# vLAR-group/OGC

Measured on AMD Instinct MI355X. Metric: point-clouds/sec (8192 pts) segnet fwd+bwd, higher is better.
Workload: dtype f32; 1 GPU; C4 KITTI-SF train_seg unsup: segnet_kitti fwd + OGC loss (dynamic+smooth+invariance) + bwd + Adam, 4 samples x 4 views x 8192 pts per GPU; n_point=8192, n_slot=10, parallelism=dp1, optimizer_stepped=True

## Files before the change

include/ogc_ops.h:

```cpp
#ifndef OGC_OPS_H
#define OGC_OPS_H

#ifdef __cplusplus
extern "C" {
#endif

typedef void *ogc_stream_t;
typedef unsigned short ogc_bf16_t;

enum {
    OGC_OK = 0,
    OGC_ERR_INVALID_ARG = -1,
    OGC_ERR_LAUNCH = -2,
    OGC_ERR_UNSUPPORTED = -3
};

#define OGC_VERSION 208
int ogc_version(void);
int ogc_distance_contracted(void);
int ogc_set_deterministic(int on);
int ogc_get_deterministic(void);
const char *ogc_last_error(void);

int ogc_furthest_point_sampling(int b, int n, int m, const float *xyz, float *temp,
// ... 63 lines not shown
                 ogc_stream_t stream);

int ogc_seg_eval_ignore(int B, int n, int k, const int *segm, const float *mask, const int *ignore, int ignore_npoint_thresh,
                        int *hard, int *counts, int *ignored, double *pred_iou, double *confidence, int *valid, int *n_gt,
                        float *score, int *rows, double *ri, int *status, ogc_stream_t stream);

int ogc_flow_eval(int B, int N, const float *gt_flow, const float *flow_pred, double epe_norm_thresh, double eps,
                  double *epe_sum, int *counts, ogc_stream_t stream);

#define OGC_SUP_LOSS_MAX_K 32
#define OGC_SUP_LOSS_TILE 64
long long ogc_sup_loss_ws_doubles(int B, int n, int k);
int ogc_sup_match_cost(int B, int n, int k, const float *mask, const float *gt_mask, const float *valid, int use_focal,
                       double alpha, double gamma, double *ws, float *cost_ce, float *cost_dice, ogc_stream_t stream);
int ogc_sup_mask_loss_fwd(int B, int n, int k, const float *mask, const float *gt_mask, const float *valid, const int *col4row,
                          int use_focal, double alpha, double gamma, double *ws, double *sums, float *terms,
                          ogc_stream_t stream);
int ogc_sup_mask_loss_bwd(int B, int n, int k, const float *mask, const float *gt_mask, const float *valid, const int *col4row,
                          int use_focal, double alpha, double gamma, const double *sums, double w_ce, double w_dice,
                          const float *grad_out, float *grad_mask, ogc_stream_t stream);

int ogc_group_concat(int b, int c, int n, int npoints, int nsample, const float *xyz, const float *new_xyz,
                     const float *points, const int *idx, float *out, ogc_stream_t stream);

int ogc_group_concat_grad(int b, int c, int n, int npoints, int nsample, const float *grad_out, const int *idx,
                          float *grad_points, ogc_stream_t stream);

int ogc_group_linear_fwd(int b, int m, int n, int npoints, int nsample, int groups, const float *P, const int *idx,
                         const float *rel, const float *wx, float *y, double *stats, ogc_stream_t stream);
int ogc_group_linear_fwd_direct(int b, int m, int cf, int n, int npoints, int nsample, int groups, const float *feats,
                                const int *idx, const float *rel, const float *w, float *y, double *stats, ogc_stream_t stream);
int ogc_group_linear_fwd_direct_h(int b, int m, int cf, int n, int npoints, int nsample, int groups, const float *feats,
                                  const int *idx, const float *rel, const float *w, ogc_bf16_t *y, double *stats, ogc_stream_t stream);
int ogc_group_linear_bwd(int b, int m, int n, int npoints, int nsample, const float *grad_y, const int *idx,
                         const float *rel, float *grad_p, float *dwx, ogc_stream_t stream);

int ogc_group_reverse_chunk(int n, int npoints, int nsample);
int ogc_group_reverse(int b, int n, int npoints, int nsample, const int *idx, int *rev_start, unsigned short *rev_pos,
                      unsigned short *heads, ogc_stream_t stream);
int ogc_group_points_grad_rev(int b, int c, int n, int npoints, int nsample, const float *grad_out, const int *rev_start,
                              const unsigned short *rev_pos, const unsigned short *heads, float *grad_points,
                              ogc_stream_t stream);

int ogc_group_points_grad_rev_dwx(int b, int c, int n, int npoints, int nsample, const float *grad_out, const int *rev_start,
                                  const unsigned short *rev_pos, const unsigned short *heads, const float *rel,
                                  float *grad_points, float *dwx, ogc_stream_t stream);
int ogc_three_interpolate_grad_rev(int b, int c, int n, int m, const float *grad_out, const float *weight,
                                   const int *rev_start, const unsigned short *rev_pos, const unsigned short *heads,
                                   float *grad_points, ogc_stream_t stream);
int ogc_three_interpolate_grad_rev_bs(int b, int c, int n, int m, const float *grad_out, long long grad_out_bstride,
                                      const float *weight, const int *rev_start, const unsigned short *rev_pos,
                                      const unsigned short *heads, float *grad_points, ogc_stream_t stream);

int ogc_view_means(int parts, const float *const *src, const int *rows, const long long *len, float *out, ogc_stream_t stream);
int ogc_view_means_grad(int parts, float *const *grad, const int *rows, const long long *len, const float *weight,
                        const float *g_loss, ogc_stream_t stream);
int ogc_sum_ranges(int parts, const float *const *src, const long long *first, const long long *count, long long total,
                   float *out, ogc_stream_t stream);

int ogc_rigid_moments(int vb, int n, int k, const float *pc, const float *pc2, const float *mask, double *mom, float *S,
                      float *means, ogc_stream_t stream);
int ogc_rigid_translation(int total, const float *means, const int *valid, float *R, float *t, ogc_stream_t stream);
int ogc_rigid_blend(int vb, int n, int k, int p, int backward, const float *pc, const float *pc2, const float *mask,
                    const float *R, const float *t, const float *grad_out, float *out, ogc_stream_t stream);

int ogc_mask_iou(int pb, int n, int k, const float *mask1, const float *mask2, int *counts, float *iou,
                 ogc_stream_t stream);
int ogc_matched_distance(int pb, int n, int k, int p, int backward, const float *mask1, const float *mask2,
                         const int *col12, const int *col21, const float *grad12, const float *grad21, float *out1,
                         float *out2, ogc_stream_t stream);

int ogc_lsap_maximize(int np, int k, const float *score, int *col4row, ogc_stream_t stream);

int ogc_sym_eigvals(int nb, int k, const double *A, double *w, ogc_stream_t stream);

int ogc_neighbour_consistency_fwd(int b, int n, int c, int k, int p, const float *mask, const int *idx, float *out,
                                  ogc_stream_t stream);

int ogc_reverse_neighbours(int b, int n, int k, const int *idx, int *rev_start, int *rev_src, int *rev_mult, int *ws,
                           ogc_stream_t stream);

int ogc_neighbour_consistency_bwd(int b, int n, int c, int k, int p, const float *mask, const int *idx,
                                  const int *rev_start, const int *rev_src, const int *rev_mult, const float *grad_out,
                                  float *grad_mask, ogc_stream_t stream);

int ogc_soft_nn_target(int b, int n1, int n2, int k, float temperature, const float *p1, const float *p2,
                       const float *mask1, const float *mask2, float *target, ogc_stream_t stream);

int ogc_soft_carry(int b, int n1, int n2, int c, float temperature, const float *p1, const float *p2, const float *x,
                   float *out, ogc_stream_t stream);

#define OGC_SCAN_CROP_TILE 1024
#define OGC_SCAN_CROP_CAMERA_DOUBLES 36
int ogc_scan_crop_camera(int n, int stride, const float *scan, const double *cam, float clip_distance, float depth_thresh,
                         float *out_pc, int *keep_idx, int *count, ogc_stream_t stream);
int ogc_scan_crop_front(int n, int stride, const float *scan, float *out_pc, int *keep_idx, int *count, ogc_stream_t stream);
int ogc_scan_crop_tile(void);

#define OGC_BOX_SEGM_CHUNK 128
#define OGC_BOX_SEGM_BOX_DOUBLES 18
int ogc_box_segm(int n, int k, const float *pc, int sign_x, int sign_y, int sign_z, const double *boxes, const int *ids,
                 int *segm, int *semantic_segm, ogc_stream_t stream);
int ogc_box_segm_chunk(void);

int ogc_kittisf_unproject(int height, int width, const unsigned short *disp1, const unsigned short *disp2,
                          const unsigned short *flow, const unsigned short *inst, float fb, float f, float p02, float p03,
                          float p12, float p13, float p23, float depth_thresh, const int *select_semantics, int n_select,
                          float *pc1, float *pc2, int *segm, int *keep_idx, int *count, ogc_stream_t stream);

int ogc_png_unfilter(const unsigned char *in, unsigned char *out, int height, int row_bytes, int bpp);

int ogc_attention_fwd(int b, int lq, int lk, int h, int d, float scale, const float *q, int ldq, const float *k,
                      int ldk, const float *v, int ldv, float *out, float *prob, ogc_stream_t stream);
int ogc_attention_bwd(int b, int lq, int lk, int h, int d, float scale, const float *q, int ldq, const float *k,
                      int ldk, const float *v, int ldv, const float *out, const float *prob, const float *dout,
                      float *dq, int lddq, float *dk, int lddk, float *dv, int lddv, ogc_stream_t stream);

int ogc_small_linear_fwd(int rows, int n_in, int n_out, const float *x, const float *weight, const float *bias,
                         float *y, ogc_stream_t stream);
int ogc_small_linear_bwd(int rows, int n_in, int n_out, const float *x, const float *weight, const float *grad_y,
                         float *grad_x, float *grad_weight, float *grad_bias, ogc_stream_t stream);

int ogc_conv1x1_wgrad_moments(int b, int cin, int cout, int hw, int relu, const float *y_prev, const float *pa,
                              const float *pb, const float *grad_y, float *moments, ogc_stream_t stream);
int ogc_gn_moments_combine(int b, int cin, int cout, int hw, int groups, const float *moments, const float *w,
                           const float *pa, const float *pb, const float *mean, const float *rstd, const float *gamma,
                           float *grad_w, float *coef, float *grad_gamma, float *grad_beta, ogc_stream_t stream);
int ogc_conv1x1_dgrad_adjoint(int b, int cin, int cout, int hw, int relu, const float *w, const float *grad_y,
                              const float *y_prev, const float *pa, const float *pb, const float *coef, float *grad_prev,
                              ogc_stream_t stream);

int ogc_first_conv_stats(int b, int c1, int c0, int hw, int groups, const float *x0, const float *w1, double *stats,
                         ogc_stream_t stream);
int ogc_conv1x1_gemm_affine_first(int b, int M, int K, int hw, int relu, int groups, int c0, const float *w, const float *x0,
                                  const float *w1, const float *pa, const float *pb, float *out, double *stats,
                                  ogc_stream_t stream);
int ogc_conv1x1_wgrad_moments_first(int b, int cin, int cout, int hw, int relu, int c0, const float *x0, const float *w1,
                                    const float *pa, const float *pb, const float *grad_y, float *moments,
                                    ogc_stream_t stream);
int ogc_conv1x1_dgrad_adjoint_first(int b, int cin, int cout, int hw, int relu, int c0, const float *w, const float *grad_y,
                                    const float *x0, const float *w1, const float *pa, const float *pb, const float *coef,
                                    float *grad_w1, ogc_stream_t stream);

int ogc_group_norm_maxpool_bwd_sparse(int b, int c, int p, int s, int groups, int relu, const float *x,
                                      const float *x_at_argmax, const float *gamma, const float *mean, const float *rstd, const float *out, const int *argmax,
                                      const float *grad_out, float *coef2, float *inj, float *grad_gamma,
                                      float *grad_beta, double *ws, ogc_stream_t stream);
int ogc_conv1x1_wgrad_moments_pooled(int b, int cin, int cout, int hw, int relu, int nsample, const float *y_prev,
                                     const float *pa, const float *pb, const float *y, const float *coef2,
                                     const float *inj, float *moments, ogc_stream_t stream);
int ogc_conv1x1_dgrad_adjoint_pooled(int b, int cin, int cout, int hw, int relu, int nsample, const float *w, const float *y,
                                     const float *coef2, const float *inj, const float *y_prev, const float *pa,
                                     const float *pb, const float *coef, float *grad_prev, ogc_stream_t stream);

int ogc_mlp_chain_pool_supported(int c0, int c1, int c2, int c3, int nsample);
int ogc_mlp_chain_pool(int b, int c0, int c1, int c2, int c3, int p, int nsample, const float *x, const float *wt1,
                       const float *b1, const float *wt2, const float *b2, const float *wt3, const float *b3, float *out,
                       ogc_stream_t stream);

int ogc_corr_layer_pool_supported(int cf, int c1, int c2, int c3, int nsample);
int ogc_corr_layer_pool(int b, int cf, int c1, int c2, int c3, int n1, int n2, int nsample, const float *pos1,
                        const float *pos2, const float *feat1, const float *feat2, const int *idx, const float *wt1,
                        const float *b1, const float *wt2, const float *b2, const float *wt3, const float *b3, float *out,
                        ogc_stream_t stream);

long long ogc_slot_masks_ws_floats(int b, int d, int n, int k);
int ogc_slot_masks_fwd(int b, int d, int n, int k, float temperature, const float *feats, const float *slots,
                       float *mask, ogc_stream_t stream);
int ogc_slot_masks_bwd(int b, int d, int n, int k, float temperature, const float *feats, const float *slots,
                       const float *mask, const float *grad_mask, float *grad_feats, float *grad_slots, float *ws,
                       ogc_stream_t stream);

int ogc_group_norm_stats_slots(void);
int ogc_group_norm_bwd_slots(void);
int ogc_group_norm_fwd(int b, int c, int hw, int groups, float eps, int relu, const float *x,
                       const float *gamma, const float *beta, float *y, float *mean, float *rstd,
                       double *ws, ogc_stream_t stream);
int ogc_group_norm_bwd(int b, int c, int hw, int groups, int relu, const float *x, const float *gamma,
                       const float *beta, const float *mean, const float *rstd, const float *grad_y,
                       float *grad_x, float *grad_gamma, float *grad_beta, double *ws, ogc_stream_t stream);

int ogc_group_norm_maxpool_fwd(int b, int c, int p, int s, int groups, float eps, int relu, const float *x,
                               const float *gamma, const float *beta, float *out, int *argmax, float *mean,
                               float *rstd, double *ws, ogc_stream_t stream);
int ogc_group_norm_maxpool_bwd(int b, int c, int p, int s, int groups, int relu, const float *x,
                               const float *gamma, const float *mean, const float *rstd, const float *out,
                               const int *argmax, const float *grad_out, float *grad_x, float *grad_gamma,
                               float *grad_beta, double *ws, ogc_stream_t stream);
int ogc_group_norm_maxpool_bwd_ext(int b, int c, int p, int s, int groups, int relu, const float *x,
                                   const float *x_at_argmax, const float *gamma, const float *mean, const float *rstd,
                                   const float *out, const int *argmax, const float *grad_out, float *grad_x,
                                   float *grad_gamma, float *grad_beta, double *ws, ogc_stream_t stream);

int ogc_batch_norm_fwd(int b, int c, int hw, float eps, int relu, int training, float momentum, const float *x,
                       const float *gamma, const float *beta, float *running_mean, float *running_var, float *y,
                       float *mean, float *rstd, double *ws, const double *stats, int slots, ogc_stream_t stream);
int ogc_batch_norm_bwd(int b, int c, int hw, int relu, int training, const float *x, const float *gamma,
                       const float *beta, const float *mean, const float *rstd, const float *grad_y, float *grad_x,
                       float *grad_gamma, float *grad_beta, double *ws, ogc_stream_t stream);
int ogc_batch_norm_maxpool_fwd(int b, int c, int p, int s, float eps, int relu, int training, float momentum,
                               const float *x, const float *gamma, const float *beta, float *running_mean,
                               float *running_var, float *out, int *argmax, float *mean, float *rstd, double *ws,
                               const double *stats, int slots, ogc_stream_t stream);
int ogc_batch_norm_maxpool_bwd(int b, int c, int p, int s, int relu, int training, const float *x, const float *gamma,
                               const float *mean, const float *rstd, const float *out, const int *argmax,
                               const float *grad_out, float *grad_x, float *grad_gamma, float *grad_beta, double *ws,
                               ogc_stream_t stream);

int ogc_conv1x1_wgrad(int b, int cin, int cout, int hw, const float *x, const float *dy, float *dw,
                      ogc_stream_t stream);

int ogc_conv1x1_gemm(int b, int M, int K, int hw, int transpose_a, const float *w, const float *in,
                     float *out, ogc_stream_t stream);

int ogc_conv1x1_gn_slots(void);
int ogc_conv1x1_gemm_stats_supported(int b, int M, int K, int hw, int affine);
int ogc_conv1x1_gemm_stream_supported(int b, int M, int K, int hw);
int ogc_conv1x1_gemm_any(int b, int M, int K, int hw, int transpose_a, const float *w, const float *in, float *out,
                         ogc_stream_t stream);

int ogc_set_matmul_precision(int bf16);
int ogc_conv1x1_gemm_gnstats(int b, int M, int K, int hw, int groups, const float *w, const float *in, float *out,
                             double *stats, ogc_stream_t stream);

int ogc_group_norm_coeffs(int b, int c, int hw, int groups, float eps, const float *x, const float *gamma,
                          const float *beta, const double *stats, int slots, double *ws, float *mean, float *rstd,
                          float *a, float *bb, ogc_stream_t stream);
int ogc_conv1x1_gemm_affine(int b, int M, int K, int hw, int relu, int groups, const float *w, const float *in,
                            const float *pa, const float *pb, float *out, double *stats, ogc_stream_t stream);
int ogc_conv1x1_wgrad_affine(int b, int cin, int cout, int hw, int relu, const float *x, const float *pa,
                             const float *pb, const float *dy, float *dw, ogc_stream_t stream);
int ogc_conv1x1_wgrad_affine_pooled(int b, int cin, int cout, int hw, int relu, int nsample, const float *x, const float *pa,
                                    const float *pb, const float *y, const float *coef2, const float *inj, float *dw,
                                    ogc_stream_t stream);
int ogc_conv1x1_dgrad_pooled(int b, int cin, int cout, int hw, int nsample, const float *w, const float *y, const float *coef2,
                             const float *inj, float *grad_z, ogc_stream_t stream);

int ogc_group_norm_fwd_stats(int b, int c, int hw, int groups, float eps, int relu, const float *x,
                             const float *gamma, const float *beta, float *y, float *mean, float *rstd,
                             const double *stats, int slots, ogc_stream_t stream);
int ogc_group_norm_maxpool_fwd_stats(int b, int c, int p, int s, int groups, float eps, int relu, const float *x,
                                     const float *gamma, const float *beta, float *out, int *argmax, float *mean,
                                     float *rstd, const double *stats, int slots, ogc_stream_t stream);

int ogc_conv1x1_gemm_affine_pool(int b, int M, int K, int hw, int relu, int groups, int nsample, const float *w,
                                 const float *in, const float *pa, const float *pb, const float *next_gamma,
                                 float *out, double *stats, float *yext, int *aext, ogc_stream_t stream);
int ogc_group_norm_pool_extremes(int b, int c, int p, int s, int groups, float eps, int relu, const float *yext,
                                 const int *aext, const float *gamma, const float *beta, float *out, int *argmax,
                                 float *mean, float *rstd, const double *stats, int slots, ogc_stream_t stream);

int ogc_chamfer_terms(int b, int n1, int n2, int p, const float *p1, const float *pc2, const int *idx12, const int *idx21,
                      float *dist1, float *dist2, ogc_stream_t stream);
int ogc_chamfer_terms_grad(int b, int n1, int n2, int p, const float *p1, const float *pc2, const int *idx12, const int *idx21,
                           const float *g1, const float *g2, float *grad_p1, ogc_stream_t stream);

int ogc_gather_xyz_pair(int b, int n, int m, const float *xyz, const int *idx, float *out, float *out_t, ogc_stream_t stream);
int ogc_flow_advance(int b, int n, float scale, const float *cur, const float *delta, const float *ref, float *out_delta,
                     float *out_new, float *out_new_t, float *out_flow, ogc_stream_t stream);
int ogc_linear_cn(int b, int cin, int cout, int n, const float *x, const float *weight, const float *bias, float *y,
                  ogc_stream_t stream);
int ogc_three_nn_weights(int b, int n, int mode, const float *dist2, float *weight, ogc_stream_t stream);
int ogc_soft_corr_flow(int b, int n1, int n2, int c, float support, const float *epsilon, const float *pc1, const float *pc2,
                       const float *f1, const float *f2, float *flow, ogc_stream_t stream);
int ogc_gru_reset(int b, int c, int cx, int n, int s, const float *rc, long long rc_batch_stride, const float *hx, float *out,
                  ogc_stream_t stream);
int ogc_gru_blend(int b, int c, int n, int s, const float *zc, long long zc_batch_stride, const float *qc,
                  long long qc_batch_stride, const float *h, long long h_batch_stride, float *out, ogc_stream_t stream);

int ogc_zero_arena_begin(void *base, int bytes, ogc_stream_t stream);
int ogc_zero_arena_end(void);

int ogc_group_linear_fwd_h(int b, int m, int n, int npoints, int nsample, int groups, const float *P, const int *idx,
                           const float *rel, const float *wx, ogc_bf16_t *y, double *stats, ogc_stream_t stream);
int ogc_group_linear_fwd_pt_h(int b, int m, int n, int npoints, int nsample, int groups, const float *Pt, const int *idx,
                              const float *rel, const float *wx, ogc_bf16_t *y, double *stats, ogc_stream_t stream);
int ogc_group_points_grad_rev_h(int b, int c, int n, int npoints, int nsample, const ogc_bf16_t *grad_out, const int *rev_start,
                                const unsigned short *rev_pos, const unsigned short *heads, float *grad_points,
                                ogc_stream_t stream);
int ogc_group_points_grad_rev_dwx_h(int b, int c, int n, int npoints, int nsample, const ogc_bf16_t *grad_out, const int *rev_start,
                                    const unsigned short *rev_pos, const unsigned short *heads, const float *rel,
                                    float *grad_points, float *dwx, ogc_stream_t stream);
int ogc_conv1x1_gemm_h(int b, int M, int K, int hw, int transpose_a, const float *w, const ogc_bf16_t *in, ogc_bf16_t *out,
                       ogc_stream_t stream);
int ogc_conv1x1_gemm_affine_h(int b, int M, int K, int hw, int relu, int groups, const float *w, const ogc_bf16_t *in,
                              const float *pa, const float *pb, ogc_bf16_t *out, double *stats, ogc_stream_t stream);
int ogc_conv1x1_gemm_affine_pool_h(int b, int M, int K, int hw, int relu, int groups, int nsample, const float *w,
                                   const ogc_bf16_t *in, const float *pa, const float *pb, const float *next_gamma,
                                   ogc_bf16_t *out, double *stats, float *yext, int *aext, ogc_stream_t stream);
int ogc_conv1x1_wgrad_xf_h(int b, int cin, int cout, int hw, const float *x, const ogc_bf16_t *dy, float *dw,
                           ogc_stream_t stream);
int ogc_conv1x1_wgrad_affine_h(int b, int cin, int cout, int hw, int relu, const ogc_bf16_t *x, const float *pa,
                               const float *pb, const ogc_bf16_t *dy, float *dw, ogc_stream_t stream);
int ogc_conv1x1_wgrad_affine_pooled_h(int b, int cin, int cout, int hw, int relu, int nsample, const ogc_bf16_t *x,
                                      const float *pa, const float *pb, const ogc_bf16_t *y, const float *coef2,
                                      const float *inj, float *dw, ogc_stream_t stream);
int ogc_conv1x1_dgrad_pooled_h(int b, int cin, int cout, int hw, int nsample, const float *w, const ogc_bf16_t *y,
                               const float *coef2, const float *inj, ogc_bf16_t *grad_z, ogc_stream_t stream);
int ogc_conv1x1_wgrad_moments_h(int b, int cin, int cout, int hw, int relu, const ogc_bf16_t *y_prev, const float *pa,
                                const float *pb, const ogc_bf16_t *grad_y, float *moments, ogc_stream_t stream);
int ogc_conv1x1_wgrad_moments_pooled_h(int b, int cin, int cout, int hw, int relu, int nsample, const ogc_bf16_t *y_prev,
                                       const float *pa, const float *pb, const ogc_bf16_t *y, const float *coef2,
                                       const float *inj, float *moments, ogc_stream_t stream);
int ogc_conv1x1_dgrad_adjoint_h(int b, int cin, int cout, int hw, int relu, const float *w, const ogc_bf16_t *grad_y,
                                const ogc_bf16_t *y_prev, const float *pa, const float *pb, const float *coef,
                                ogc_bf16_t *grad_prev, ogc_stream_t stream);
// ... 17 lines not shown
```

ogc_amd/_lib.py:

```python
import ctypes
import os

_HERE = os.path.dirname(os.path.abspath(__file__))
FMAD = os.environ.get("OGC_FMAD", "0") == "1"
DETERMINISTIC = os.environ.get("OGC_DETERMINISTIC", "0") == "1"
LIB_PATH = os.path.join(_HERE, "csrc", "libogc_ops_fmad.so" if FMAD else "libogc_ops.so")

_vp = ctypes.c_void_p
_int = ctypes.c_int
_flt = ctypes.c_float
_dbl = ctypes.c_double
_ll = ctypes.c_longlong

SIGNATURES = {
    "ogc_set_deterministic": [_int],
    "ogc_group_linear_fwd_direct": [_int, _int, _int, _int, _int, _int, _int, _vp, _vp, _vp, _vp, _vp, _vp, _vp],
    "ogc_get_deterministic": [],
    "ogc_furthest_point_sampling": [_int, _int, _int, _vp, _vp, _vp, _vp],
    "ogc_furthest_point_sampling_chain": [_int, _int, _int, _vp, _vp, _vp, _vp, _vp, _vp],
    "ogc_gather_points": [_int, _int, _int, _int, _vp, _vp, _vp, _vp],
    "ogc_gather_points_grad": [_int, _int, _int, _int, _vp, _vp, _vp, _vp],
    "ogc_knn": [_int, _int, _int, _int, _vp, _vp, _vp, _vp, _vp],
    "ogc_three_nn": [_int, _int, _int, _vp, _vp, _vp, _vp, _vp],
    "ogc_three_interpolate": [_int, _int, _int, _int, _vp, _vp, _vp, _vp, _vp],
    "ogc_three_interpolate_grad": [_int, _int, _int, _int, _vp, _vp, _vp, _vp, _vp],
    "ogc_group_points": [_int, _int, _int, _int, _int, _vp, _vp, _vp, _vp],
    "ogc_group_points_grad": [_int, _int, _int, _int, _int, _vp, _vp, _vp, _vp],
    "ogc_group_reverse_chunk": [_int, _int, _int],
    "ogc_group_reverse": [_int, _int, _int, _int, _vp, _vp, _vp, _vp, _vp],
    "ogc_three_interpolate_grad_rev": [_int, _int, _int, _int, _vp, _vp, _vp, _vp, _vp, _vp, _vp],
    "ogc_view_means": [_int, _vp, _vp, _vp, _vp, _vp],
    "ogc_view_means_grad": [_int, _vp, _vp, _vp, _vp, _vp, _vp],
    "ogc_sum_ranges": [_int, _vp, _vp, _vp, _ll, _vp, _vp],
    "ogc_three_interpolate_grad_rev_bs": [_int, _int, _int, _int, _vp, _ll, _vp, _vp, _vp, _vp, _vp, _vp],
    "ogc_group_points_grad_rev": [_int, _int, _int, _int, _int, _vp, _vp, _vp, _vp, _vp, _vp],
    "ogc_group_points_grad_rev_dwx": [_int, _int, _int, _int, _int, _vp, _vp, _vp, _vp, _vp, _vp, _vp, _vp],
    "ogc_ball_query": [_int, _int, _int, _flt, _int, _vp, _vp, _vp, _vp],
    "ogc_knn_clamped": [_int, _int, _int, _int, _flt, _vp, _vp, _vp, _vp, _vp],
    "ogc_cell_grid_bytes": [_int, _int],
    "ogc_cell_grid_build": [_int, _int, _flt, _vp, _vp, _vp],
    "ogc_ball_query_cells": [_int, _int, _flt, _int, _vp, _vp, _flt, _vp, _vp],
    "ogc_knn_clamped_cells": [_int, _int, _int, _flt, _vp, _vp, _flt, _vp, _vp, _vp],
    "ogc_chamfer_terms": [_int, _int, _int, _int, _vp, _vp, _vp, _vp, _vp, _vp, _vp],
    "ogc_chamfer_terms_grad": [_int, _int, _int, _int, _vp, _vp, _vp, _vp, _vp, _vp, _vp, _vp],
    "ogc_gather_xyz_pair": [_int, _int, _int, _vp, _vp, _vp, _vp, _vp],
    "ogc_flow_advance": [_int, _int, _flt, _vp, _vp, _vp, _vp, _vp, _vp, _vp, _vp],
    "ogc_linear_cn": [_int, _int, _int, _int, _vp, _vp, _vp, _vp, _vp],
    "ogc_three_nn_weights": [_int, _int, _int, _vp, _vp, _vp],
    "ogc_soft_corr_flow": [_int, _int, _int, _int, _flt, _vp, _vp, _vp, _vp, _vp, _vp, _vp],
    "ogc_gru_reset": [_int, _int, _int, _int, _int, _vp, _ll, _vp, _vp, _vp],
    "ogc_gru_blend": [_int, _int, _int, _int, _vp, _ll, _vp, _ll, _vp, _ll, _vp, _vp],
    "ogc_zero_arena_begin": [_vp, _int, _vp],
    "ogc_zero_arena_end": [],
    "ogc_adam_max_tensors": [],
    "ogc_adam_chunk": [],
    "ogc_adam_step": [_int, _int, _vp, _vp, _vp, _vp, _vp, _dbl, _dbl, _dbl, _dbl, _dbl, _vp],
    "ogc_kabsch_rotation": [_int, _vp, _vp, _vp, _vp],
    "ogc_rigid_icp": [_int, _int, _vp, _vp, _vp, _int, _dbl, _vp, _vp, _vp, _vp],
    "ogc_ground_plane_fit": [_int, _int, _vp, _int, _int, _dbl, _dbl, _int, _vp, _vp, _vp, _vp],
    "ogc_seg_eval": [_int, _int, _int, _vp, _vp, _int, _vp, _vp, _vp, _vp, _vp, _vp, _vp, _vp, _vp, _vp, _vp],
    "ogc_seg_eval_ignore": [_int, _int, _int, _vp, _vp, _vp, _int, _vp, _vp, _vp, _vp, _vp, _vp, _vp, _vp, _vp, _vp, _vp, _vp],
    "ogc_flow_eval": [_int, _int, _vp, _vp, _dbl, _dbl, _vp, _vp, _vp],
    "ogc_lsap_maximize": [_int, _int, _vp, _vp, _vp],
    "ogc_sup_loss_ws_doubles": [_int, _int, _int],
    "ogc_sup_match_cost": [_int, _int, _int, _vp, _vp, _vp, _int, _dbl, _dbl, _vp, _vp, _vp, _vp],
    "ogc_sup_mask_loss_fwd": [_int, _int, _int, _vp, _vp, _vp, _vp, _int, _dbl, _dbl, _vp, _vp, _vp, _vp],
    "ogc_sup_mask_loss_bwd": [_int, _int, _int, _vp, _vp, _vp, _vp, _int, _dbl, _dbl, _vp, _dbl, _dbl, _vp, _vp, _vp],
    "ogc_rigid_moments": [_int, _int, _int, _vp, _vp, _vp, _vp, _vp, _vp, _vp],
    "ogc_rigid_translation": [_int, _vp, _vp, _vp, _vp, _vp],
    "ogc_rigid_blend": [_int, _int, _int, _int, _int, _vp, _vp, _vp, _vp, _vp, _vp, _vp, _vp],
    "ogc_mask_iou": [_int, _int, _int, _vp, _vp, _vp, _vp, _vp],
    "ogc_matched_distance": [_int, _int, _int, _int, _int, _vp, _vp, _vp, _vp, _vp, _vp, _vp, _vp, _vp],
    "ogc_soft_nn_target": [_int, _int, _int, _int, _flt, _vp, _vp, _vp, _vp, _vp, _vp],
    "ogc_soft_carry": [_int, _int, _int, _int, _flt, _vp, _vp, _vp, _vp, _vp],
    "ogc_scan_crop_camera": [_int, _int, _vp, _vp, _flt, _flt, _vp, _vp, _vp, _vp],
    "ogc_scan_crop_front": [_int, _int, _vp, _vp, _vp, _vp, _vp],
    "ogc_scan_crop_tile": [],
    "ogc_box_segm": [_int, _int, _vp, _int, _int, _int, _vp, _vp, _vp, _vp, _vp],
    "ogc_box_segm_chunk": [],
    "ogc_kittisf_unproject": [_int, _int, _vp, _vp, _vp, _vp, _flt, _flt, _flt, _flt, _flt, _flt, _flt, _flt, _vp, _int,
                              _vp, _vp, _vp, _vp, _vp, _vp],
    "ogc_png_unfilter": [_vp, _vp, _int, _int, _int],
    "ogc_group_concat": [_int, _int, _int, _int, _int, _vp, _vp, _vp, _vp, _vp, _vp],
    "ogc_group_linear_fwd": [_int, _int, _int, _int, _int, _int, _vp, _vp, _vp, _vp, _vp, _vp, _vp],
    "ogc_group_linear_bwd": [_int, _int, _int, _int, _int, _vp, _vp, _vp, _vp, _vp, _vp],
    "ogc_group_concat_grad": [_int, _int, _int, _int, _int, _vp, _vp, _vp, _vp],
    "ogc_neighbour_consistency_fwd": [_int, _int, _int, _int, _int, _vp, _vp, _vp, _vp],
    "ogc_reverse_neighbours": [_int, _int, _int, _vp, _vp, _vp, _vp, _vp, _vp],
    "ogc_neighbour_consistency_bwd": [_int, _int, _int, _int, _int, _vp, _vp, _vp, _vp, _vp, _vp, _vp, _vp],
    "ogc_sym_eigvals": [_int, _int, _vp, _vp, _vp],
    "ogc_group_norm_fwd": [_int, _int, _int, _int, _flt, _int, _vp, _vp, _vp, _vp, _vp, _vp, _vp, _vp],
    "ogc_group_norm_bwd": [_int, _int, _int, _int, _int, _vp, _vp, _vp, _vp, _vp, _vp, _vp, _vp, _vp, _vp, _vp],
    "ogc_group_norm_maxpool_fwd": [_int, _int, _int, _int, _int, _flt, _int, _vp, _vp, _vp, _vp, _vp, _vp, _vp, _vp, _vp],
    "ogc_conv1x1_gemm": [_int, _int, _int, _int, _int, _vp, _vp, _vp, _vp],
    "ogc_attention_fwd": [_int, _int, _int, _int, _int, _flt, _vp, _int, _vp, _int, _vp, _int, _vp, _vp, _vp],
    "ogc_attention_bwd": [_int, _int, _int, _int, _int, _flt, _vp, _int, _vp, _int, _vp, _int, _vp, _vp, _vp, _vp, _int,
                          _vp, _int, _vp, _int, _vp],
    "ogc_conv1x1_gemm_affine_pool": [_int, _int, _int, _int, _int, _int, _int, _vp, _vp, _vp, _vp, _vp, _vp, _vp, _vp, _vp,
                                     _vp],
    "ogc_group_norm_pool_extremes": [_int, _int, _int, _int, _int, _flt, _int, _vp, _vp, _vp, _vp, _vp, _vp, _vp, _vp, _vp,
                                     _int, _vp],
    "ogc_small_linear_fwd": [_int, _int, _int, _vp, _vp, _vp, _vp, _vp],
    "ogc_small_linear_bwd": [_int, _int, _int, _vp, _vp, _vp, _vp, _vp, _vp, _vp],
    "ogc_conv1x1_wgrad_moments": [_int, _int, _int, _int, _int, _vp, _vp, _vp, _vp, _vp, _vp],
    "ogc_gn_moments_combine": [_int, _int, _int, _int, _int, _vp, _vp, _vp, _vp, _vp, _vp, _vp, _vp, _vp, _vp, _vp, _vp],
    "ogc_conv1x1_dgrad_adjoint": [_int, _int, _int, _int, _int, _vp, _vp, _vp, _vp, _vp, _vp, _vp, _vp],
    "ogc_first_conv_stats": [_int, _int, _int, _int, _int, _vp, _vp, _vp, _vp],
    "ogc_conv1x1_gemm_affine_first": [_int, _int, _int, _int, _int, _int, _int, _vp, _vp, _vp, _vp, _vp, _vp, _vp, _vp],
    "ogc_conv1x1_wgrad_moments_first": [_int, _int, _int, _int, _int, _int, _vp, _vp, _vp, _vp, _vp, _vp, _vp],
    "ogc_conv1x1_dgrad_adjoint_first": [_int, _int, _int, _int, _int, _int, _vp, _vp, _vp, _vp, _vp, _vp, _vp, _vp, _vp],
    "ogc_group_norm_maxpool_bwd_sparse": [_int, _int, _int, _int, _int, _int, _vp, _vp, _vp, _vp, _vp, _vp, _vp, _vp, _vp, _vp,
                                          _vp, _vp, _vp, _vp],
    "ogc_group_norm_maxpool_bwd_ext": [_int, _int, _int, _int, _int, _int, _vp, _vp, _vp, _vp, _vp, _vp, _vp, _vp, _vp, _vp,
                                       _vp, _vp, _vp],
    "ogc_conv1x1_wgrad_moments_pooled": [_int, _int, _int, _int, _int, _int, _vp, _vp, _vp, _vp, _vp, _vp, _vp, _vp],
    "ogc_conv1x1_dgrad_adjoint_pooled": [_int, _int, _int, _int, _int, _int, _vp, _vp, _vp, _vp, _vp, _vp, _vp, _vp, _vp, _vp],
    "ogc_mlp_chain_pool_supported": [_int, _int, _int, _int, _int],
    "ogc_mlp_chain_pool": [_int, _int, _int, _int, _int, _int, _int, _vp, _vp, _vp, _vp, _vp, _vp, _vp, _vp, _vp],
    "ogc_corr_layer_pool_supported": [_int, _int, _int, _int, _int],
    "ogc_corr_layer_pool": [_int, _int, _int, _int, _int, _int, _int, _int, _vp, _vp, _vp, _vp, _vp, _vp, _vp, _vp, _vp, _vp,
                            _vp, _vp, _vp],
    "ogc_slot_masks_ws_floats": [_int, _int, _int, _int],
    "ogc_slot_masks_fwd": [_int, _int, _int, _int, _flt, _vp, _vp, _vp, _vp],
    "ogc_slot_masks_bwd": [_int, _int, _int, _int, _flt, _vp, _vp, _vp, _vp, _vp, _vp, _vp, _vp],
    "ogc_conv1x1_gn_slots": [],
    "ogc_conv1x1_gemm_stats_supported": [_int, _int, _int, _int, _int],
    "ogc_conv1x1_gemm_stream_supported": [_int, _int, _int, _int],
    "ogc_conv1x1_gemm_any": [_int, _int, _int, _int, _int, _vp, _vp, _vp, _vp],
    "ogc_set_matmul_precision": [_int],
    "ogc_group_norm_stats_slots": [],
    "ogc_group_norm_bwd_slots": [],
    "ogc_group_norm_coeffs": [_int, _int, _int, _int, _flt, _vp, _vp, _vp, _vp, _int, _vp, _vp, _vp, _vp, _vp, _vp],
    "ogc_conv1x1_gemm_affine": [_int, _int, _int, _int, _int, _int, _vp, _vp, _vp, _vp, _vp, _vp, _vp],
    "ogc_conv1x1_wgrad_affine": [_int, _int, _int, _int, _int, _vp, _vp, _vp, _vp, _vp, _vp],
    "ogc_conv1x1_wgrad_affine_pooled": [_int, _int, _int, _int, _int, _int, _vp, _vp, _vp, _vp, _vp, _vp, _vp, _vp],
    "ogc_conv1x1_dgrad_pooled": [_int, _int, _int, _int, _int, _vp, _vp, _vp, _vp, _vp, _vp],
    "ogc_batch_norm_fwd": [_int, _int, _int, _flt, _int, _int, _flt, _vp, _vp, _vp, _vp, _vp, _vp, _vp, _vp, _vp, _vp,
                           _int, _vp],
    "ogc_batch_norm_bwd": [_int, _int, _int, _int, _int, _vp, _vp, _vp, _vp, _vp, _vp, _vp, _vp, _vp, _vp, _vp],
    "ogc_batch_norm_maxpool_fwd": [_int, _int, _int, _int, _flt, _int, _int, _flt, _vp, _vp, _vp, _vp, _vp, _vp, _vp,
                                   _vp, _vp, _vp, _vp, _int, _vp],
    "ogc_batch_norm_maxpool_bwd": [_int, _int, _int, _int, _int, _int, _vp, _vp, _vp, _vp, _vp, _vp, _vp, _vp, _vp,
                                   _vp, _vp, _vp],
    "ogc_conv1x1_gemm_gnstats": [_int, _int, _int, _int, _int, _vp, _vp, _vp, _vp, _vp],
    "ogc_group_norm_fwd_stats": [_int, _int, _int, _int, _flt, _int, _vp, _vp, _vp, _vp, _vp, _vp, _vp, _int, _vp],
    "ogc_group_norm_maxpool_fwd_stats": [_int, _int, _int, _int, _int, _flt, _int, _vp, _vp, _vp, _vp, _vp, _vp, _vp,
                                         _vp, _int, _vp],
    "ogc_conv1x1_wgrad": [_int, _int, _int, _int, _vp, _vp, _vp, _vp],
    "ogc_group_norm_maxpool_bwd": [_int, _int, _int, _int, _int, _int, _vp, _vp, _vp, _vp, _vp, _vp, _vp, _vp, _vp, _vp,
                                   _vp, _vp],
}

for _n in ("ogc_group_linear_fwd", "ogc_group_points_grad_rev", "ogc_conv1x1_gemm", "ogc_conv1x1_gemm_affine",
           "ogc_conv1x1_gemm_affine_pool", "ogc_conv1x1_wgrad_affine", "ogc_conv1x1_wgrad_affine_pooled",
           "ogc_conv1x1_dgrad_pooled", "ogc_conv1x1_wgrad_moments", "ogc_conv1x1_wgrad_moments_pooled",
           "ogc_conv1x1_dgrad_adjoint", "ogc_conv1x1_dgrad_adjoint_pooled", "ogc_group_norm_bwd",
           "ogc_group_norm_maxpool_bwd_sparse", "ogc_group_points_grad_rev_dwx"):
    SIGNATURES[_n + "_h"] = SIGNATURES[_n]
SIGNATURES["ogc_group_linear_fwd_direct_h"] = SIGNATURES["ogc_group_linear_fwd_direct"]
SIGNATURES["ogc_conv1x1_wgrad_xf_h"] = SIGNATURES["ogc_conv1x1_wgrad"]
SIGNATURES["ogc_group_linear_fwd_pt_h"] = SIGNATURES["ogc_group_linear_fwd"]

HEADER_VERSION = 208
_lib = None
_fns = {}


class OgcOpsError(RuntimeError):
    pass


def load():
    global _lib
    if _lib is None:
        if not os.path.exists(LIB_PATH):
            raise OgcOpsError(
                "libogc_ops.so not found at %s — build it with `python ogc_amd/csrc/build.py` "
                "(there is no CPU fallback)" % LIB_PATH)
        L = ctypes.CDLL(LIB_PATH)
        for name, argtypes in SIGNATURES.items():
            fn = getattr(L, name)
            fn.argtypes = argtypes
            fn.restype = _int
        L.ogc_version.restype = _int
        if L.ogc_version() != HEADER_VERSION:
            raise OgcOpsError("libogc_ops.so at %s is version %d, this package binds version %d of include/ogc_ops.h — rebuild it "
                              "with `python ogc_amd/csrc/build.py --force`" % (LIB_PATH, L.ogc_version(), HEADER_VERSION))
        L.ogc_distance_contracted.restype = _int
        if bool(L.ogc_distance_contracted()) != FMAD:
            raise OgcOpsError("%s evaluates distances %s, OGC_FMAD asked for the other form" %
                              (LIB_PATH, "contracted (fma)" if L.ogc_distance_contracted() else "un-contracted"))
        L.ogc_slot_masks_ws_floats.restype = ctypes.c_longlong
        L.ogc_cell_grid_bytes.restype = ctypes.c_longlong
        L.ogc_sup_loss_ws_doubles.restype = ctypes.c_longlong
        L.ogc_last_error.restype = ctypes.c_char_p
        L.ogc_set_deterministic(1 if DETERMINISTIC else 0)
        _lib = L
    return _lib


def set_deterministic(on):
    global DETERMINISTIC
    DETERMINISTIC = bool(on)
    load().ogc_set_deterministic(1 if on else 0)


CALL_COUNTS = None

ROCTX_NAMES = {
    "ogc_furthest_point_sampling": "K1 furthest_point_sampling", "ogc_furthest_point_sampling_chain": "K1 furthest_point_sampling (chain)",
    "ogc_gather_points": "K2 gather_points", "ogc_gather_points_grad": "K3 gather_points_grad",
    "ogc_knn": "K4 knn", "ogc_knn_clamped": "K4 knn (+ sqrt + radius clamp)", "ogc_knn_clamped_cells": "K4 knn (shared cell grid)",
    "ogc_three_nn": "K5 three_nn", "ogc_three_interpolate": "K6 three_interpolate",
    "ogc_three_interpolate_grad": "K7 three_interpolate_grad", "ogc_three_interpolate_grad_rev": "K7 three_interpolate_grad (gather form)",
    "ogc_three_interpolate_grad_rev_bs": "K7 three_interpolate_grad (gather form)",
    "ogc_group_points": "K8 group_points", "ogc_group_points_grad": "K9 group_points_grad",
    "ogc_group_points_grad_rev": "K9 group_points_grad (gather form)",
    "ogc_ball_query": "K10 ball_query", "ogc_ball_query_cells": "K10 ball_query (shared cell grid)",
}
_roctx = None


def _roctx_lib():
    global _roctx
    if _roctx is None:
        _roctx = False
        if os.environ.get("OGC_ROCTX", "0") == "1":
            for name in ("librocprofiler-sdk-roctx.so", "libroctx64.so"):
                try:
                    lib = ctypes.CDLL(os.path.join(os.environ.get("ROCM_PATH", "/opt/rocm"), "lib", name))
                    lib.roctxRangePushA.argtypes = [ctypes.c_char_p]
                    lib.roctxRangePushA.restype = ctypes.c_int
                    lib.roctxRangePop.restype = ctypes.c_int
                    _roctx = lib
                    break
                except (OSError, AttributeError):
                    continue
    return _roctx


def call(name, *args):
    if CALL_COUNTS is not None:
        CALL_COUNTS[name] += 1
    fn = _fns.get(name)
    if fn is None:
        fn = _fns[name] = getattr(load(), name)
    tx = _roctx_lib()
    if tx:
        tx.roctxRangePushA(ROCTX_NAMES.get(name, name).encode())
        try:
            rc = fn(*args)
        finally:
            tx.roctxRangePop()
    else:
        rc = fn(*args)
    if rc != 0:
        msg = load().ogc_last_error().decode("utf-8", "replace")
        raise OgcOpsError("%s failed (status %d): %s" % (name, rc, msg))
    return rc
```

ogc_amd/csrc/gn_fused_bwd.hip:

```cpp
#include "conv1x1_shared.h"
#include "act_io.h"
#include "first_conv.h"

namespace {

template <int COB, int CIB, bool POOLED, typename AT = float, int FIRST = 0>
__global__ __launch_bounds__(WG_WAVES *OGC_WAVE) void wgrad_moments_kernel(int cin, int cout, int hw, int chunks,
                                                                           int steps_per_wave, int relu,
                                                                           const AT *__restrict__ x,
                                                                           const AT *__restrict__ dy,
                                                                           const float *__restrict__ aff_a,
                                                                           const float *__restrict__ aff_b,
                                                                           const float2 *__restrict__ coef2,
                                                                           const float2 *__restrict__ inj,
                                                                           int s_shift,
                                                                           float *__restrict__ hm,
                                                                           FirstIn first = FirstIn()) {
    constexpr int XN = FIRST ? FIRST : CIB;
    __shared__ float red[WG_WAVES][COB * CIB * 256];
    const int lane = threadIdx.x & 63, wave = __builtin_amdgcn_readfirstlane(threadIdx.x >> 6);
    const int i = lane & 15, k = lane >> 4;
    const int img = blockIdx.x / chunks, chunk = blockIdx.x - img * chunks;
    const int co0 = blockIdx.y * (16 * COB), ci0 = blockIdx.z * (16 * CIB);
    const int steps_per_img = hw >> 4;
    const int first_step = (chunk * WG_WAVES + wave) * steps_per_wave;
    const int mine = max(0, min(steps_per_wave, steps_per_img - first_step));

    v4f acc1[COB][CIB], acc2[COB][CIB];
#pragma unroll
    for (int a = 0; a < COB; ++a)
#pragma unroll
        for (int c = 0; c < CIB; ++c) {
            acc1[a][c] = (v4f){0.f, 0.f, 0.f, 0.f};
            acc2[a][c] = (v4f){0.f, 0.f, 0.f, 0.f};
        }
    int yrow[COB], xrow[XN], jrow[COB];
    float ca[CIB], cb[CIB], pc2[COB], pc3[COB];
    float w1r[FIRST ? CIB : 1][FIRST ? FIRST : 1];
    const int centres = hw >> s_shift, smask = (1 << s_shift) - 1;
#pragma unroll
    for (int a = 0; a < COB; ++a) {
        const int row = min(co0 + a * 16 + i, cout - 1);
        yrow[a] = row * hw;
        if (POOLED) {
            const float2 cc = coef2[(size_t)img * cout + row];
            pc2[a] = cc.x;
            pc3[a] = cc.y;
            jrow[a] = row * centres;
        }
    }
    const float2 *jb_ = POOLED ? inj + (size_t)img * cout * centres : nullptr;
#pragma unroll
    for (int c = 0; c < CIB; ++c) {
        const int ch = min(ci0 + c * 16 + i, cin - 1);
        if constexpr (FIRST == 0) xrow[c] = ch * hw;
        ca[c] = aff_a[(size_t)img * cin + ch];
        cb[c] = aff_b[(size_t)img * cin + ch];
        if constexpr (FIRST > 0) {
#pragma unroll
            for (int e = 0; e < FIRST; ++e) w1r[c][e] = e < first.c0 ? first.w1[ch * first.c0 + min(e, first.c0 - 1)] : 0.f;
        }
    }
    if constexpr (FIRST > 0) {
#pragma unroll
        for (int e = 0; e < FIRST; ++e) xrow[e] = min(e, first.c0 - 1) * hw;
    }
    const AT *yb_ = dy + (size_t)img * cout * hw + 4 * k;
    const AT *xb_ = FIRST ? reinterpret_cast<const AT *>(first.x0) + (size_t)img * first.c0 * hw + 4 * k
                          : x + (size_t)img * cin * hw + 4 * k;
    int cur = min(first_step, steps_per_img - 1);
    const int stop = min(first_step + mine, steps_per_img) - 1;
    auto load = [&](float4(&yv)[COB], float4(&xv)[XN], float2(&jv)[COB], int &jpos) {
        const int pb = cur * 16;
#pragma unroll
        for (int a = 0; a < COB; ++a) yv[a] = ogc_ld4(yb_ + yrow[a] + pb);
#pragma unroll
        for (int c = 0; c < XN; ++c) xv[c] = ogc_ld4(xb_ + xrow[c] + pb);
        if (POOLED) {
#pragma unroll
            for (int a = 0; a < COB; ++a) jv[a] = jb_[jrow[a] + (pb >> s_shift)];
            jpos = (pb & smask) + 4 * k;
        }
        cur = min(cur + 1, max(stop, 0));
    };
    auto fma16 = [&](float4(&yv)[COB], const float4(&xraw)[XN], const float2(&jv)[COB], int jpos) {
        if (POOLED) {
#pragma unroll
            for (int a = 0; a < COB; ++a) ogc_pooled_grad(yv[a], pc2[a], pc3[a], jv[a], jpos);
        }
        float4 x0v[FIRST ? FIRST : 1];
        if constexpr (FIRST > 0) {
#pragma unroll
            for (int e = 0; e < FIRST; ++e) x0v[e] = xraw[e];
            ogc_first_mask<FIRST>(x0v, first.c0, true);
        }
        float4 m1[CIB], m2[CIB];
#pragma unroll
        for (int c = 0; c < CIB; ++c) {
            float4 v;
            if constexpr (FIRST > 0) v = ogc_first_row<FIRST>(x0v, w1r[c]);
            else v = xraw[c];
            const bool bx = relu ? fmaf(ca[c], v.x, cb[c]) > 0.f : true;
            const bool by = relu ? fmaf(ca[c], v.y, cb[c]) > 0.f : true;
            const bool bz = relu ? fmaf(ca[c], v.z, cb[c]) > 0.f : true;
            const bool bw = relu ? fmaf(ca[c], v.w, cb[c]) > 0.f : true;
            m1[c] = make_float4(bx ? 1.f : 0.f, by ? 1.f : 0.f, bz ? 1.f : 0.f, bw ? 1.f : 0.f);
            m2[c] = make_float4(bx ? v.x : 0.f, by ? v.y : 0.f, bz ? v.z : 0.f, bw ? v.w : 0.f);
        }
#pragma unroll
        for (int a = 0; a < COB; ++a)
#pragma unroll
            for (int c = 0; c < CIB; ++c) {
                acc1[a][c] = __builtin_amdgcn_mfma_f32_16x16x4f32(yv[a].x, m1[c].x, acc1[a][c], 0, 0, 0);
                acc2[a][c] = __builtin_amdgcn_mfma_f32_16x16x4f32(yv[a].x, m2[c].x, acc2[a][c], 0, 0, 0);
                acc1[a][c] = __builtin_amdgcn_mfma_f32_16x16x4f32(yv[a].y, m1[c].y, acc1[a][c], 0, 0, 0);
                acc2[a][c] = __builtin_amdgcn_mfma_f32_16x16x4f32(yv[a].y, m2[c].y, acc2[a][c], 0, 0, 0);
                acc1[a][c] = __builtin_amdgcn_mfma_f32_16x16x4f32(yv[a].z, m1[c].z, acc1[a][c], 0, 0, 0);
                acc2[a][c] = __builtin_amdgcn_mfma_f32_16x16x4f32(yv[a].z, m2[c].z, acc2[a][c], 0, 0, 0);
                acc1[a][c] = __builtin_amdgcn_mfma_f32_16x16x4f32(yv[a].w, m1[c].w, acc1[a][c], 0, 0, 0);
                acc2[a][c] = __builtin_amdgcn_mfma_f32_16x16x4f32(yv[a].w, m2[c].w, acc2[a][c], 0, 0, 0);
            }
    };

    float4 ya[COB], xa[XN], yb[COB], xb[XN];
    float2 ja[COB], jb[COB];
    int pa_ = 0, pb_ = 0;
    load(ya, xa, ja, pa_);
    int s = 0;
    for (; s + 1 < mine; s += 2) {
        load(yb, xb, jb, pb_);
        fma16(ya, xa, ja, pa_);
        load(ya, xa, ja, pa_);
        fma16(yb, xb, jb, pb_);
    }
    if (s < mine) fma16(ya, xa, ja, pa_);

    float *dst = hm + (size_t)img * 2 * cout * cin;
#pragma unroll
    for (int which = 0; which < 2; ++which) {
        if (which) __syncthreads();
#pragma unroll
        for (int a = 0; a < COB; ++a)
#pragma unroll
            for (int c = 0; c < CIB; ++c)
#pragma unroll
                for (int r = 0; r < 4; ++r)
                    red[wave][(a * CIB + c) * 256 + (k * 4 + r) * 16 + i] = which ? acc2[a][c][r] : acc1[a][c][r];
        __syncthreads();
        for (int t = threadIdx.x; t < COB * CIB * 256; t += WG_WAVES * OGC_WAVE) {
            const int blk = t >> 8, a = blk / CIB, c = blk % CIB;
            const int row = co0 + a * 16 + ((t & 255) >> 4), col = ci0 + c * 16 + (t & 15);
            const float v = (red[0][t] + red[1][t]) + (red[2][t] + red[3][t]);
            if (row < cout && col < cin && v != 0.0f) unsafeAtomicAdd(dst + ((size_t)which * cout + row) * cin + col, v);
        }
    }
}

typedef short v4s16 __attribute__((ext_vector_type(4)));

template <int COB, int CIB, bool POOLED>
__global__ __launch_bounds__(WG_WAVES *OGC_WAVE) void wgrad_moments16_kernel(int cin, int cout, int hw, int chunks,
                                                                             int steps_per_wave, int relu,
                                                                             const ogc_bf16 *__restrict__ x,
                                                                             const ogc_bf16 *__restrict__ dy,
                                                                             const float *__restrict__ aff_a,
                                                                             const float *__restrict__ aff_b,
                                                                             const float2 *__restrict__ coef2,
                                                                             const float2 *__restrict__ inj,
                                                                             int s_shift,
                                                                             float *__restrict__ hm) {
    __shared__ float red[WG_WAVES][COB * CIB * 256];
    const int lane = threadIdx.x & 63, wave = __builtin_amdgcn_readfirstlane(threadIdx.x >> 6);
    const int i = lane & 15, k = lane >> 4;
    const int img = blockIdx.x / chunks, chunk = blockIdx.x - img * chunks;
    const int co0 = blockIdx.y * (16 * COB), ci0 = blockIdx.z * (16 * CIB);
    const int steps_per_img = hw >> 5;
    const int first = (chunk * WG_WAVES + wave) * steps_per_wave;
    const int mine = max(0, min(steps_per_wave, steps_per_img - first));

    v4f acc1[COB][CIB], acc2[COB][CIB];
#pragma unroll
    for (int a = 0; a < COB; ++a)
#pragma unroll
        for (int c = 0; c < CIB; ++c) {
            acc1[a][c] = (v4f){0.f, 0.f, 0.f, 0.f};
            acc2[a][c] = (v4f){0.f, 0.f, 0.f, 0.f};
        }
    int yrow[COB], xrow[CIB], jrow[COB];
    float ca[CIB], cb[CIB], pc2[COB], pc3[COB];
    const int centres = hw >> s_shift, smask = (1 << s_shift) - 1;
#pragma unroll
    for (int a = 0; a < COB; ++a) {
        const int row = min(co0 + a * 16 + i, cout - 1);
        yrow[a] = row * hw;
        if (POOLED) {
            const float2 cc = coef2[(size_t)img * cout + row];
            pc2[a] = cc.x;
            pc3[a] = cc.y;
            jrow[a] = row * centres;
        }
    }
    const float2 *jb_ = POOLED ? inj + (size_t)img * cout * centres : nullptr;
#pragma unroll
    for (int c = 0; c < CIB; ++c) {
        const int ch = min(ci0 + c * 16 + i, cin - 1);
        xrow[c] = ch * hw;
        ca[c] = aff_a[(size_t)img * cin + ch];
        cb[c] = aff_b[(size_t)img * cin + ch];
    }
    const ogc_bf16 *yb_ = dy + (size_t)img * cout * hw + 8 * k;
    const ogc_bf16 *xb_ = x + (size_t)img * cin * hw + 8 * k;
    int cur = min(first, steps_per_img - 1);
    const int stop = min(first + mine, steps_per_img) - 1;
    auto load = [&](uint4(&yv)[COB], uint4(&xv)[CIB], float2(&jv)[COB], int &jpos) {
        const int pb = cur * 32;
#pragma unroll
        for (int a = 0; a < COB; ++a) yv[a] = *reinterpret_cast<const uint4 *>(yb_ + yrow[a] + pb);
#pragma unroll
        for (int c = 0; c < CIB; ++c) xv[c] = *reinterpret_cast<const uint4 *>(xb_ + xrow[c] + pb);
        if (POOLED) {
#pragma unroll
            for (int a = 0; a < COB; ++a) jv[a] = jb_[jrow[a] + ((pb + 8 * k) >> s_shift)];
            jpos = (pb + 8 * k) & smask;
        }
        cur = min(cur + 1, max(stop, 0));
    };
    auto fma32 = [&](const uint4(&yraw)[COB], const uint4(&xraw)[CIB], const float2(&jv)[COB], int jpos) {
        v4s16 y0[COB], y1[COB];
#pragma unroll
        for (int a = 0; a < COB; ++a) {
            if (POOLED) {
                float f[8];
                ogc_unpack8(yraw[a], f);
                ogc_pooled_grad(f, pc2[a], pc3[a], jv[a], jpos);
                y0[a] = ogc_pack_bf16_rr(f[0], f[1], f[2], f[3]);
                y1[a] = ogc_pack_bf16_rr(f[4], f[5], f[6], f[7]);
            } else {
                y0[a] = __builtin_bit_cast(v4s16, make_uint2(yraw[a].x, yraw[a].y));
                y1[a] = __builtin_bit_cast(v4s16, make_uint2(yraw[a].z, yraw[a].w));
            }
        }
        v4s16 m1a[CIB], m1b[CIB], m2a[CIB], m2b[CIB];
#pragma unroll
        for (int c = 0; c < CIB; ++c) {
            float f[8];
            ogc_unpack8(xraw[c], f);
            unsigned keep[4];
#pragma unroll
            for (int e = 0; e < 4; ++e) {
                const bool lo = relu ? fmaf(ca[c], f[2 * e], cb[c]) > 0.f : true;
                const bool hi = relu ? fmaf(ca[c], f[2 * e + 1], cb[c]) > 0.f : true;
                keep[e] = (lo ? 0x0000FFFFu : 0u) | (hi ? 0xFFFF0000u : 0u);
            }
            const unsigned xs[4] = {xraw[c].x, xraw[c].y, xraw[c].z, xraw[c].w};
            m1a[c] = __builtin_bit_cast(v4s16, make_uint2(keep[0] & 0x3F803F80u, keep[1] & 0x3F803F80u));
            m1b[c] = __builtin_bit_cast(v4s16, make_uint2(keep[2] & 0x3F803F80u, keep[3] & 0x3F803F80u));
            m2a[c] = __builtin_bit_cast(v4s16, make_uint2(keep[0] & xs[0], keep[1] & xs[1]));
            m2b[c] = __builtin_bit_cast(v4s16, make_uint2(keep[2] & xs[2], keep[3] & xs[3]));
        }
#pragma unroll
        for (int a = 0; a < COB; ++a)
#pragma unroll
            for (int c = 0; c < CIB; ++c) {
                acc1[a][c] = ogc_mfma_bf16_k32(y0[a], y1[a], m1a[c], m1b[c], acc1[a][c]);
                acc2[a][c] = ogc_mfma_bf16_k32(y0[a], y1[a], m2a[c], m2b[c], acc2[a][c]);
            }
    };

    uint4 ya[COB], xa[CIB], yb[COB], xb[CIB];
    float2 ja[COB], jb[COB];
    int pa_ = 0, pb_ = 0;
    load(ya, xa, ja, pa_);
    int s = 0;
    for (; s + 1 < mine; s += 2) {
        load(yb, xb, jb, pb_);
        fma32(ya, xa, ja, pa_);
        load(ya, xa, ja, pa_);
        fma32(yb, xb, jb, pb_);
    }
    if (s < mine) fma32(ya, xa, ja, pa_);

    float *dst = hm + (size_t)img * 2 * cout * cin;
#pragma unroll
    for (int which = 0; which < 2; ++which) {
        if (which) __syncthreads();
#pragma unroll
        for (int a = 0; a < COB; ++a)
#pragma unroll
            for (int c = 0; c < CIB; ++c)
#pragma unroll
                for (int r = 0; r < 4; ++r)
                    red[wave][(a * CIB + c) * 256 + (k * 4 + r) * 16 + i] = which ? acc2[a][c][r] : acc1[a][c][r];
        __syncthreads();
        for (int t = threadIdx.x; t < COB * CIB * 256; t += WG_WAVES * OGC_WAVE) {
            const int blk = t >> 8, a = blk / CIB, c = blk % CIB;
            const int row = co0 + a * 16 + ((t & 255) >> 4), col = ci0 + c * 16 + (t & 15);
            const float v = (red[0][t] + red[1][t]) + (red[2][t] + red[3][t]);
            if (row < cout && col < cin && v != 0.0f) unsafeAtomicAdd(dst + ((size_t)which * cout + row) * cin + col, v);
        }
    }
}


template <int COB, int CIB, typename AT, int FIRST = 0>
void moments_launch(int b, int cin, int cout, int hw, int relu, const AT *x, const AT *dy, const float *pa,
                    const float *pb, const float *coef2, const float *inj, int s_shift, float *hm, hipStream_t s,
                    FirstIn first = FirstIn()) {
    const int steps_per_img = sizeof(AT) == 2 ? hw >> 5 : hw >> 4;
    const int tiles = ogc_divup(cout, 16 * COB) * ogc_divup(cin, 16 * CIB);
    long long waves = (2048 / tiles) / b;
    if (waves < 4) waves = 4;
    int spw = (int)((steps_per_img + waves - 1) / waves);
    if (spw < 8) spw = 8;
    spw = (spw + 1) / 2 * 2;
    const int chunks = ogc_divup(steps_per_img, spw * WG_WAVES);
    dim3 grid(b * chunks, ogc_divup(cout, 16 * COB), ogc_divup(cin, 16 * CIB));
    const float2 *c2 = reinterpret_cast<const float2 *>(coef2), *ij = reinterpret_cast<const float2 *>(inj);
    if constexpr (sizeof(AT) == 2) {
        if (inj)
            hipLaunchKernelGGL((wgrad_moments16_kernel<COB, CIB, true>), grid, dim3(WG_WAVES * OGC_WAVE), 0, s, cin, cout, hw,
                               chunks, spw, relu, x, dy, pa, pb, c2, ij, s_shift, hm);
        else
            hipLaunchKernelGGL((wgrad_moments16_kernel<COB, CIB, false>), grid, dim3(WG_WAVES * OGC_WAVE), 0, s, cin, cout, hw,
                               chunks, spw, relu, x, dy, pa, pb, c2, ij, 0, hm);
    } else if constexpr (FIRST > 0) {
        hipLaunchKernelGGL((wgrad_moments_kernel<COB, CIB, false, AT, FIRST>), grid, dim3(WG_WAVES * OGC_WAVE), 0, s, cin, cout, hw,
                           chunks, spw, relu, x, dy, pa, pb, c2, ij, 0, hm, first);
    } else {
        if (inj)
            hipLaunchKernelGGL((wgrad_moments_kernel<COB, CIB, true, AT>), grid, dim3(WG_WAVES * OGC_WAVE), 0, s, cin, cout, hw, chunks,
                               spw, relu, x, dy, pa, pb, c2, ij, s_shift, hm);
        else
            hipLaunchKernelGGL((wgrad_moments_kernel<COB, CIB, false, AT>), grid, dim3(WG_WAVES * OGC_WAVE), 0, s, cin, cout, hw, chunks,
                               spw, relu, x, dy, pa, pb, c2, ij, 0, hm);
    }
}

__global__ __launch_bounds__(256) void moments_combine_kernel(int b, int cin, int cout, int hw, int groups,
                                                              const float *__restrict__ hm, const float *__restrict__ w,
                                                              const float *__restrict__ pa, const float *__restrict__ pb,
                                                              const float *__restrict__ mean, const float *__restrict__ rstd,
                                                              const float *__restrict__ gamma, float *__restrict__ dw,
                                                              float *__restrict__ coef,
                                                              float *__restrict__ dgamma, float *__restrict__ dbeta) {
    __shared__ double s1[32], s2[32];
    const int cpg = cin / groups;
    if ((int)blockIdx.x < b) {
        const int img = blockIdx.x;
        __shared__ double tt1[512], tt2[512];
        for (int t = threadIdx.x; t < 512; t += blockDim.x) { tt1[t] = 0.0; tt2[t] = 0.0; }
        if (threadIdx.x < 32) { s1[threadIdx.x] = 0.0; s2[threadIdx.x] = 0.0; }
        __syncthreads();
        const float *h1 = hm + (size_t)img * 2 * cout * cin, *h2 = h1 + (size_t)cout * cin;
        for (int it = threadIdx.x; it < cin * 8; it += blockDim.x) {
            const int ml = it / cin, k = it - ml * cin;
            double t1 = 0.0, t2 = 0.0;
            for (int m = ml; m < cout; m += 8) {
                const double wv = w[(size_t)m * cin + k];
                t1 += wv * h1[(size_t)m * cin + k];
                t2 += wv * h2[(size_t)m * cin + k];
            }
            atomicAdd(&tt1[k], t1);
            atomicAdd(&tt2[k], t2);
        }
        __syncthreads();
        for (int k = threadIdx.x; k < cin; k += blockDim.x) {
            const int g = k / cpg;
            const double mu = mean[img * groups + g], r = rstd[img * groups + g], gm = gamma[k];
            atomicAdd(&s1[g], gm * tt1[k]);
            atomicAdd(&s2[g], gm * (tt2[k] - mu * tt1[k]) * r);
        }
        __syncthreads();
        const double n = (double)cpg * (double)hw;
        for (int k = threadIdx.x; k < cin; k += blockDim.x) {
            const int g = k / cpg;
            const double mu = mean[img * groups + g], r = rstd[img * groups + g];
            const double c2 = -r * r * s2[g] / n;
            const double c3 = -r * s1[g] / n - c2 * mu;
            float *o = coef + ((size_t)img * cin + k) * 3;
            o[0] = (float)((double)gamma[k] * r);
            o[1] = (float)c2;
            o[2] = (float)c3;
        }
        for (int k = threadIdx.x; k < cin; k += blockDim.x) {
            const int g = k / cpg;
            const double mu = mean[img * groups + g], r = rstd[img * groups + g];
            unsafeAtomicAdd(dgamma + k, (float)((tt2[k] - mu * tt1[k]) * r));
            unsafeAtomicAdd(dbeta + k, (float)tt1[k]);
        }
    } else {
        const long long e = ((long long)blockIdx.x - b) * blockDim.x + threadIdx.x;
        if (e < (long long)cout * cin) {
            const int k = (int)(e % cin);
            float acc = 0.f;
            for (int img = 0; img < b; ++img) {
                const float *h1 = hm + (size_t)img * 2 * cout * cin, *h2 = h1 + (size_t)cout * cin;
                acc += pa[(size_t)img * cin + k] * h2[e] + pb[(size_t)img * cin + k] * h1[e];
            }
            dw[e] = acc;
        }
    }
}

template <int KQ, bool POOLED, typename AT = float, bool BF = false, int FIRST = 0>
__global__ __launch_bounds__(WG_WAVES *OGC_WAVE) void dgrad_adjoint_kernel(int M, int K, int hw, int relu,
                                                                           const float *__restrict__ w,
                                                                           const AT *__restrict__ gy,
                                                                           const AT *__restrict__ yprev,
                                                                           const float *__restrict__ pa,
                                                                           const float *__restrict__ pb,
                                                                           const float *__restrict__ coef,
                                                                           const float2 *__restrict__ coef2,
                                                                           const float2 *__restrict__ inj,
                                                                           int s_shift,
                                                                           AT *__restrict__ out,
                                                                           FirstIn first = FirstIn()) {
    extern __shared__ __attribute__((aligned(16))) float a_lds[];
    __shared__ __attribute__((aligned(16))) float s_w1[FIRST ? FC_MAX_ROWS * FC_MAX_C0 : 4];
    __shared__ float s_dw[FIRST ? FC_MAX_ROWS * FC_MAX_C0 : 4];
    const int lane = threadIdx.x & 63, wave = threadIdx.x >> 6;
    const int j = lane & 15, kk = lane >> 4;
    const int b = blockIdx.y;
    const int Kq = (K + 3) >> 2;
    const AT *inb = gy + (size_t)b * K * hw;
    AT *outb = out + (size_t)b * M * hw;
    const AT *yb = yprev + (size_t)b * M * hw;
    const int a_ld = ogc_a_ld(Kq);
    float *cf = a_lds + (size_t)64 * a_ld;
    if constexpr (FIRST > 0) {
        static_assert(!POOLED && !BF && sizeof(AT) == 4, "first-layer form: dense, fp32");
        ogc_first_stage_w1<WG_WAVES * OGC_WAVE>(s_w1, first.w1, M, first.c0);
        for (int t = threadIdx.x; t < FC_MAX_ROWS * FC_MAX_C0; t += WG_WAVES * OGC_WAVE) s_dw[t] = 0.f;
    }
    const int run = FIRST ? first.run : 1;
    for (int it = 0; it < run; ++it) {
    const int p0 = ((blockIdx.x * run + it) * WG_WAVES + wave) * 64;
    const bool live = p0 < hw;
    float4 x0v[FIRST ? FIRST : 1];
    if constexpr (FIRST > 0) {
        ogc_first_load_raw<FIRST>(x0v, first.x0 + (size_t)b * first.c0 * hw + (live ? p0 + 4 * j : 0), first.c0, hw);
        ogc_first_mask<FIRST>(x0v, first.c0, live);
    }

    float4 xin[KQ];
#pragma unroll
    for (int q = 0; q < KQ; ++q) {
        const int row = q * 4 + kk;
        xin[q] = (live && q < Kq && row < K) ? ogc_ld4(inb + (size_t)row * hw + p0 + 4 * j) : make_float4(0.f, 0.f, 0.f, 0.f);
    }
    if (POOLED) {
        const int centres = hw >> s_shift, cpw = 64 >> s_shift;
        float4 *tab = reinterpret_cast<float4 *>(cf + 64 * 5) + (size_t)wave * K * cpw;
        for (int e = lane; e < K * cpw; e += OGC_WAVE) {
            const int row = e / cpw, centre = (p0 >> s_shift) + (e - row * cpw);
            const float2 cc = coef2[(size_t)b * K + row];
            const float2 jj = (live && centre < centres) ? inj[((size_t)b * K + row) * centres + centre]
                                                         : make_float2(0.f, __int_as_float(-1));
            tab[e] = make_float4(cc.x, cc.y, jj.x, jj.y);
        }
        __syncthreads();
        const int mine = (4 * j) >> s_shift, jpos = (p0 + 4 * j) & ((1 << s_shift) - 1);
#pragma unroll
        for (int q = 0; q < KQ; ++q) {
            const int row = q * 4 + kk;
            if (q < Kq && row < K) {
                const float4 t = tab[row * cpw + mine];
                const int rel = __float_as_int(t.w) - jpos;
                xin[q].x = fmaf(t.x, xin[q].x, t.y) + (rel == 0 ? t.z : 0.f);
                xin[q].y = fmaf(t.x, xin[q].y, t.y) + (rel == 1 ? t.z : 0.f);
                xin[q].z = fmaf(t.x, xin[q].z, t.y) + (rel == 2 ? t.z : 0.f);
                xin[q].w = fmaf(t.x, xin[q].w, t.y) + (rel == 3 ? t.z : 0.f);
            }
        }
    }
    typedef short v4s __attribute__((ext_vector_type(4)));
    constexpr int GQ = (KQ + 3) / 4;
    v4s xb[BF ? GQ : 1][4];
    if constexpr (BF) {
#pragma unroll
        for (int g = 0; g < GQ; ++g) {
            float4 r[4];
#pragma unroll
            for (int i = 0; i < 4; ++i) r[i] = 4 * g + i < KQ ? xin[4 * g + i] : make_float4(0.f, 0.f, 0.f, 0.f);
            xb[g][0] = ogc_pack_bf16_rr(r[0].x, r[1].x, r[2].x, r[3].x);
            xb[g][1] = ogc_pack_bf16_rr(r[0].y, r[1].y, r[2].y, r[3].y);
            xb[g][2] = ogc_pack_bf16_rr(r[0].z, r[1].z, r[2].z, r[3].z);
            xb[g][3] = ogc_pack_bf16_rr(r[0].w, r[1].w, r[2].w, r[3].w);
        }
    }
    for (int m0 = 0; m0 < M; m0 += 64) {
        if (FIRST == 0 || it == 0) {
        __syncthreads();
        if constexpr (BF) {
            ogc_stage_weight_tile_bf16<true, WG_WAVES, GQ>(a_lds, w, m0, M, K, Kq);
        } else {
            ogc_stage_weight_tile<true, WG_WAVES>(a_lds, w, m0, M, K, Kq);
        }
        for (int t = threadIdx.x; t < 64; t += WG_WAVES * OGC_WAVE) {
            const int m = m0 + t;
            const bool in = m < M;
            cf[t * 5 + 0] = in ? pa[(size_t)b * M + m] : 0.f;
            cf[t * 5 + 1] = in ? pb[(size_t)b * M + m] : 0.f;
            cf[t * 5 + 2] = in ? coef[((size_t)b * M + m) * 3] : 0.f;
            cf[t * 5 + 3] = in ? coef[((size_t)b * M + m) * 3 + 1] : 0.f;
            cf[t * 5 + 4] = in ? coef[((size_t)b * M + m) * 3 + 2] : 0.f;
        }
        __syncthreads();
        }
        const int nblk = min(4, (M - m0 + 15) >> 4);
#pragma unroll
        for (int a = 0; a < 4; ++a) {
            if (a < nblk) {
                float4 yv[4];
#pragma unroll
                for (int r = 0; r < 4; ++r) {
                    const int m = m0 + a * 16 + kk * 4 + r;
                    if constexpr (FIRST > 0) {
                        float w1r[FIRST];
                        ogc_first_w1_row<FIRST>(w1r, s_w1, m);
                        yv[r] = ogc_first_row<FIRST>(x0v, w1r);
                    } else {
                        yv[r] = (live && m < M) ? ogc_ld4(yb + (size_t)m * hw + p0 + 4 * j) : make_float4(0.f, 0.f, 0.f, 0.f);
                    }
                }
                v4f acc[4];
#pragma unroll
                for (int c = 0; c < 4; ++c) acc[c] = (v4f){0.f, 0.f, 0.f, 0.f};
                if constexpr (BF) {
                    const v4s *a_bf = reinterpret_cast<const v4s *>(a_lds);
#pragma unroll
                    for (int g = 0; g + 1 < GQ; g += 2) {
                        if (4 * (g + 1) < Kq) {
                            const v4s av0 = a_bf[(g * 64 + a * 16 + j) * 4 + kk], av1 = a_bf[((g + 1) * 64 + a * 16 + j) * 4 + kk];
#pragma unroll
                            for (int c = 0; c < 4; ++c) acc[c] = ogc_mfma_bf16_k32(av0, av1, xb[g][c], xb[g + 1][c], acc[c]);
                        } else if (4 * g < Kq) {
                            const v4s av = a_bf[(g * 64 + a * 16 + j) * 4 + kk];
#pragma unroll
                            for (int c = 0; c < 4; ++c) acc[c] = __builtin_amdgcn_mfma_f32_16x16x16bf16_1k(av, xb[g][c], acc[c], 0, 0, 0);
                        }
                    }
                    if constexpr (GQ % 2 == 1) {
                        constexpr int g = GQ - 1;
                        if (4 * g < Kq) {
                            const v4s av = a_bf[(g * 64 + a * 16 + j) * 4 + kk];
#pragma unroll
                            for (int c = 0; c < 4; ++c) acc[c] = __builtin_amdgcn_mfma_f32_16x16x16bf16_1k(av, xb[g][c], acc[c], 0, 0, 0);
                        }
                    }
                } else {
#pragma unroll
                for (int q = 0; q < KQ; ++q) {
                    if (q < Kq) {
                        const float av = a_lds[(a * 16 + j) * a_ld + q * 4 + kk];
                        acc[0] = __builtin_amdgcn_mfma_f32_16x16x4f32(av, xin[q].x, acc[0], 0, 0, 0);
                        acc[1] = __builtin_amdgcn_mfma_f32_16x16x4f32(av, xin[q].y, acc[1], 0, 0, 0);
                        acc[2] = __builtin_amdgcn_mfma_f32_16x16x4f32(av, xin[q].z, acc[2], 0, 0, 0);
                        acc[3] = __builtin_amdgcn_mfma_f32_16x16x4f32(av, xin[q].w, acc[3], 0, 0, 0);
                    }
                }
                }
                if (live) {
#pragma unroll
                    for (int r = 0; r < 4; ++r) {
                        const int mi = a * 16 + kk * 4 + r, m = m0 + mi;
                        if (m < M) {
                            const float fa = cf[mi * 5], fb = cf[mi * 5 + 1], al = cf[mi * 5 + 2], c2 = cf[mi * 5 + 3], c3 = cf[mi * 5 + 4];
                            const float4 y = yv[r];
                            float4 g = make_float4(acc[0][r], acc[1][r], acc[2][r], acc[3][r]);
                            if (relu) {
                                g.x = fmaf(fa, y.x, fb) > 0.f ? g.x : 0.f; g.y = fmaf(fa, y.y, fb) > 0.f ? g.y : 0.f;
                                g.z = fmaf(fa, y.z, fb) > 0.f ? g.z : 0.f; g.w = fmaf(fa, y.w, fb) > 0.f ? g.w : 0.f;
                            }
                            float4 o;
                            o.x = fmaf(al, g.x, fmaf(c2, y.x, c3)); o.y = fmaf(al, g.y, fmaf(c2, y.y, c3));
                            o.z = fmaf(al, g.z, fmaf(c2, y.z, c3)); o.w = fmaf(al, g.w, fmaf(c2, y.w, c3));
                            if constexpr (FIRST > 0) {
                                float mine = 0.f;
#pragma unroll
                                for (int c = 0; c < FIRST; ++c) {
                                    float d = fmaf(o.w, x0v[c].w, fmaf(o.z, x0v[c].z, fmaf(o.y, x0v[c].y, o.x * x0v[c].x)));
                                    d += ogc_dpp_f32<0xB1>(d);
                                    d += ogc_dpp_f32<0x4E>(d);
                                    d += ogc_dpp_f32<0x141>(d);
                                    d += ogc_dpp_f32<0x140>(d);
                                    mine = j == c ? d : mine;
                                }
                                if (j < first.c0) atomicAdd(&s_dw[m * FC_MAX_C0 + j], mine);
                            } else {
                                ogc_st4(outb + (size_t)m * hw + p0 + 4 * j, o);
                            }
                        }
                    }
                }
            }
        }
    }
    }
    if constexpr (FIRST > 0) {
        __syncthreads();
        for (int t = threadIdx.x; t < M * first.c0; t += WG_WAVES * OGC_WAVE) {
            const float v = s_dw[(t / first.c0) * FC_MAX_C0 + t % first.c0];
            if (v != 0.0f) unsafeAtomicAdd(first.dw1 + t, v);
        }
    }
}

}

namespace {
int nsample_shift(int nsample) { return nsample == 16 ? 4 : nsample == 32 ? 5 : nsample == 64 ? 6 : -1; }

template <typename AT>
int wgrad_moments_impl(const char *name, int b, int cin, int cout, int hw, int relu, const AT *y_prev, const float *pa,
                       const float *pb, const AT *grad_y, const float *coef2, const float *inj, int s_shift,
                       float *moments, ogc_stream_t stream) {
    OGC_REQUIRE(b >= 0 && cin >= 1 && cout >= 1 && hw >= 1, "%s: bad shape", name);
    OGC_REQUIRE(y_prev && pa && pb && grad_y && moments, "%s: null pointer", name);
    if ((hw & (sizeof(AT) == 2 ? 31 : 15)) != 0 || (((uintptr_t)y_prev | (uintptr_t)grad_y) & 15) != 0) {
        ogc_set_error("%s: hw=%d must be a multiple of 16 (32 for 16-bit tensors) and the tensors 16-byte aligned", name, hw);
        return OGC_ERR_UNSUPPORTED;
    }
    if (sizeof(AT) == 2 && !ogc_g_matmul_bf16) {
        ogc_set_error("%s: 16-bit activations need ogc_set_matmul_precision(1)", name);
        return OGC_ERR_UNSUPPORTED;
    }
    OGC_REQUIRE((long long)cin * hw < (1ll << 31) && (long long)cout * hw < (1ll << 31) && b <= 32768,
                "%s: one sample exceeds 32-bit indexing", name);
    hipStream_t s = (hipStream_t)stream;
    if (b == 0) return OGC_OK;
    if (ogc_zero_async(moments, sizeof(float) * 2 * (size_t)b * cin * cout, s) != hipSuccess) {
        ogc_set_error("%s: memset failed", name);
        return OGC_ERR_LAUNCH;
    }
#define OGC_ML(A, C) moments_launch<A, C, AT>(b, cin, cout, hw, relu, y_prev, grad_y, pa, pb, coef2, inj, s_shift, moments, s)
    if (cout <= 16 && cin <= 16) OGC_ML(1, 1);
    else if (cout <= 32 && cin <= 16) OGC_ML(2, 1);
    else if (cout <= 32 && cin <= 32) OGC_ML(2, 2);
    else if (cin <= 16) OGC_ML(4, 1);
    else if (cin <= 32) OGC_ML(4, 2);
    else if (cout <= 32) OGC_ML(2, 4);
    else if (inj && sizeof(AT) == 4) OGC_ML(4, 2);
    else OGC_ML(4, 4);
#undef OGC_ML
    OGC_CHECK_LAUNCH(name);
    return OGC_OK;
}
}

extern "C" int ogc_conv1x1_wgrad_moments(int b, int cin, int cout, int hw, int relu, const float *y_prev, const float *pa,
                                         const float *pb, const float *grad_y, float *moments, ogc_stream_t stream) {
    return wgrad_moments_impl<float>("ogc_conv1x1_wgrad_moments", b, cin, cout, hw, relu, y_prev, pa, pb, grad_y, nullptr, nullptr, 0,
                                     moments, stream);
}

extern "C" int ogc_conv1x1_wgrad_moments_h(int b, int cin, int cout, int hw, int relu, const ogc_bf16_t *y_prev, const float *pa,
                                           const float *pb, const ogc_bf16_t *grad_y, float *moments, ogc_stream_t stream) {
    return wgrad_moments_impl<ogc_bf16>("ogc_conv1x1_wgrad_moments_h", b, cin, cout, hw, relu, y_prev, pa, pb, grad_y, nullptr,
                                        nullptr, 0, moments, stream);
}

namespace {
template <typename AT>
int wgrad_moments_pooled_impl(const char *name, int b, int cin, int cout, int hw, int relu, int nsample, const AT *y_prev,
                              const float *pa, const float *pb, const AT *y, const float *coef2, const float *inj,
                              float *moments, ogc_stream_t stream) {
    const int sh = nsample_shift(nsample);
    if (sh < 0 || hw % nsample != 0 || (((uintptr_t)coef2 | (uintptr_t)inj) & 7) != 0) {
        ogc_set_error("%s: nsample=%d must be 16, 32 or 64 and divide hw=%d", name, nsample, hw);
        return OGC_ERR_UNSUPPORTED;
    }
    OGC_REQUIRE(b == 0 || (coef2 && inj), "%s: null pointer", name);
    return wgrad_moments_impl<AT>(name, b, cin, cout, hw, relu, y_prev, pa, pb, y, coef2, inj, sh, moments, stream);
}
}

extern "C" int ogc_conv1x1_wgrad_moments_pooled(int b, int cin, int cout, int hw, int relu, int nsample, const float *y_prev,
                                                const float *pa, const float *pb, const float *y, const float *coef2,
                                                const float *inj, float *moments, ogc_stream_t stream) {
    return wgrad_moments_pooled_impl<float>("ogc_conv1x1_wgrad_moments_pooled", b, cin, cout, hw, relu, nsample, y_prev, pa, pb, y,
                                            coef2, inj, moments, stream);
}

extern "C" int ogc_conv1x1_wgrad_moments_pooled_h(int b, int cin, int cout, int hw, int relu, int nsample,
                                                  const ogc_bf16_t *y_prev, const float *pa, const float *pb, const ogc_bf16_t *y,
                                                  const float *coef2, const float *inj, float *moments, ogc_stream_t stream) {
    return wgrad_moments_pooled_impl<ogc_bf16>("ogc_conv1x1_wgrad_moments_pooled_h", b, cin, cout, hw, relu, nsample, y_prev, pa,
                                               pb, y, coef2, inj, moments, stream);
}

extern "C" int ogc_gn_moments_combine(int b, int cin, int cout, int hw, int groups, const float *moments, const float *w,
                                      const float *pa, const float *pb, const float *mean, const float *rstd,
                                      const float *gamma, float *grad_w, float *coef, float *grad_gamma,
                                      float *grad_beta, ogc_stream_t stream) {
    OGC_REQUIRE(b >= 1 && cin >= 1 && cin <= 512 && cout >= 1 && hw >= 1 && groups >= 1 && groups <= 32 && cin % groups == 0,
                "ogc_gn_moments_combine: bad shape (cin <= 512, groups <= 32 dividing cin)");
    OGC_REQUIRE(moments && w && pa && pb && mean && rstd && gamma && grad_w && coef && grad_gamma && grad_beta,
                "ogc_gn_moments_combine: null pointer");
    OGC_REQUIRE(grad_beta == grad_gamma + cin, "ogc_gn_moments_combine: grad_beta must follow grad_gamma (one 2 x cin buffer)");
    if (ogc_zero_async(grad_gamma, sizeof(float) * 2 * (size_t)cin, (hipStream_t)stream) != hipSuccess) {
        ogc_set_error("ogc_gn_moments_combine: memset failed");
        return OGC_ERR_LAUNCH;
    }
    hipLaunchKernelGGL(moments_combine_kernel, dim3(b + ogc_divup((long long)cout * cin, 256)), dim3(256), 0,
                       (hipStream_t)stream, b, cin, cout, hw, groups, moments, w, pa, pb, mean, rstd, gamma, grad_w, coef,
                       grad_gamma, grad_beta);
    OGC_CHECK_LAUNCH("ogc_gn_moments_combine");
    return OGC_OK;
}

namespace {
template <typename AT>
int dgrad_adjoint_impl(const char *name, int b, int cin, int cout, int hw, int relu, const float *w, const AT *grad_y,
                       const AT *y_prev, const float *pa, const float *pb, const float *coef, const float *coef2,
                       const float *inj, int s_shift, AT *grad_prev, ogc_stream_t stream) {
    OGC_REQUIRE(b >= 0 && cin >= 1 && cout >= 1 && hw >= 1, "%s: bad shape", name);
    OGC_REQUIRE(w && grad_y && y_prev && pa && pb && coef && grad_prev, "%s: null pointer", name);
    if ((hw & 63) != 0 || cout > 160 || (((uintptr_t)grad_y | (uintptr_t)y_prev | (uintptr_t)grad_prev) & ogc_act_mask<AT>()) != 0) {
        ogc_set_error("%s: needs hw %% 64 == 0, cout <= 160 and 16-byte aligned tensors (hw=%d, cout=%d)", name, hw, cout);
        return OGC_ERR_UNSUPPORTED;
    }
    OGC_REQUIRE((long long)cin * hw < (1ll << 31) && (long long)cout * hw < (1ll << 31) && b <= 65535,
                "%s: one sample exceeds 32-bit indexing", name);
    if (b == 0) return OGC_OK;
    const int M = cin, K = cout, Kq = (K + 3) / 4;
    const size_t lds = ((size_t)64 * ogc_a_ld(Kq) + 64 * 5) * sizeof(float) +
                       (inj ? (size_t)WG_WAVES * K * (64 >> s_shift) * sizeof(float4) : 0);
    if (sizeof(AT) == 2 && !ogc_g_matmul_bf16) {
        ogc_set_error("%s: 16-bit activations need ogc_set_matmul_precision(1)", name);
        return OGC_ERR_UNSUPPORTED;
    }
    if (lds > 64 * 1024) {
        ogc_set_error("%s: the weight tile and the pooled table need %zu bytes of LDS (> 64 KiB) at cout=%d, nsample=%d", name,
                      lds, cout, 64 >> (6 - s_shift));
        return OGC_ERR_UNSUPPORTED;
    }
    dim3 grid(ogc_divup(hw, 64 * WG_WAVES), b);
    hipStream_t s = (hipStream_t)stream;
    if constexpr (sizeof(AT) == 2) {
        if (!inj && ogc_gemm16_adjoint_launch(b, M, K, hw, relu, w, grad_y, y_prev, pa, pb, coef, grad_prev, s)) {
            OGC_CHECK_LAUNCH(name);
            return OGC_OK;
        }
    }
    const float2 *c2 = reinterpret_cast<const float2 *>(coef2), *ij = reinterpret_cast<const float2 *>(inj);
#define OGC_DGA(KQV)                                                                                                        \
    do {                                                                                                                    \
        if (inj)                                                                                                            \
            hipLaunchKernelGGL((dgrad_adjoint_kernel<KQV, true, AT, sizeof(AT) == 2>), grid, dim3(WG_WAVES * OGC_WAVE), lds, s, M, K, hw, relu, w,  \
                               grad_y, y_prev, pa, pb, coef, c2, ij, s_shift, grad_prev);                                  \
        else                                                                                                                \
            hipLaunchKernelGGL((dgrad_adjoint_kernel<KQV, false, AT, sizeof(AT) == 2>), grid, dim3(WG_WAVES * OGC_WAVE), lds, s, M, K, hw, relu, w, \
                               grad_y, y_prev, pa, pb, coef, c2, ij, 0, grad_prev);                                        \
    } while (0)
    if (Kq <= 8) OGC_DGA(8);
    else if (Kq <= 16) OGC_DGA(16);
    else if (Kq <= 25) OGC_DGA(25);
    else if (Kq <= 33) OGC_DGA(33);
    else OGC_DGA(40);
#undef OGC_DGA
    OGC_CHECK_LAUNCH(name);
    return OGC_OK;
}
}

extern "C" int ogc_conv1x1_dgrad_adjoint(int b, int cin, int cout, int hw, int relu, const float *w, const float *grad_y,
                                         const float *y_prev, const float *pa, const float *pb, const float *coef,
                                         float *grad_prev, ogc_stream_t stream) {
    return dgrad_adjoint_impl<float>("ogc_conv1x1_dgrad_adjoint", b, cin, cout, hw, relu, w, grad_y, y_prev, pa, pb, coef, nullptr,
                                     nullptr, 0, grad_prev, stream);
}

extern "C" int ogc_conv1x1_dgrad_adjoint_h(int b, int cin, int cout, int hw, int relu, const float *w, const ogc_bf16_t *grad_y,
                                           const ogc_bf16_t *y_prev, const float *pa, const float *pb, const float *coef,
                                           ogc_bf16_t *grad_prev, ogc_stream_t stream) {
    return dgrad_adjoint_impl<ogc_bf16>("ogc_conv1x1_dgrad_adjoint_h", b, cin, cout, hw, relu, w, grad_y, y_prev, pa, pb, coef,
                                        nullptr, nullptr, 0, grad_prev, stream);
}

namespace {
template <typename AT>
int dgrad_adjoint_pooled_impl(const char *name, int b, int cin, int cout, int hw, int relu, int nsample, const float *w,
                              const AT *y, const float *coef2, const float *inj, const AT *y_prev, const float *pa,
                              const float *pb, const float *coef, AT *grad_prev, ogc_stream_t stream) {
    const int sh = nsample_shift(nsample);
    if (sh < 0 || hw % nsample != 0 || (((uintptr_t)coef2 | (uintptr_t)inj) & 7) != 0) {
        ogc_set_error("%s: nsample=%d must be 16, 32 or 64 and divide hw=%d", name, nsample, hw);
        return OGC_ERR_UNSUPPORTED;
    }
    OGC_REQUIRE(b == 0 || (coef2 && inj), "%s: null pointer", name);
    return dgrad_adjoint_impl<AT>(name, b, cin, cout, hw, relu, w, y, y_prev, pa, pb, coef, coef2, inj, sh, grad_prev, stream);
}
}

extern "C" int ogc_conv1x1_dgrad_adjoint_pooled(int b, int cin, int cout, int hw, int relu, int nsample, const float *w,
                                                const float *y, const float *coef2, const float *inj, const float *y_prev,
                                                const float *pa, const float *pb, const float *coef, float *grad_prev,
                                                ogc_stream_t stream) {
    return dgrad_adjoint_pooled_impl<float>("ogc_conv1x1_dgrad_adjoint_pooled", b, cin, cout, hw, relu, nsample, w, y, coef2, inj,
                                            y_prev, pa, pb, coef, grad_prev, stream);
}

extern "C" int ogc_conv1x1_dgrad_adjoint_pooled_h(int b, int cin, int cout, int hw, int relu, int nsample, const float *w,
                                                  const ogc_bf16_t *y, const float *coef2, const float *inj,
                                                  const ogc_bf16_t *y_prev, const float *pa, const float *pb, const float *coef,
                                                  ogc_bf16_t *grad_prev, ogc_stream_t stream) {
    return dgrad_adjoint_pooled_impl<ogc_bf16>("ogc_conv1x1_dgrad_adjoint_pooled_h", b, cin, cout, hw, relu, nsample, w, y, coef2,
                                               inj, y_prev, pa, pb, coef, grad_prev, stream);
}

extern "C" int ogc_conv1x1_wgrad_moments_first(int b, int cin, int cout, int hw, int relu, int c0, const float *x0, const float *w1,
                                               const float *pa, const float *pb, const float *grad_y, float *moments,
                                               ogc_stream_t stream) {
    const char *name = "ogc_conv1x1_wgrad_moments_first";
    const int rc = ogc_first_check(name, b, cin, c0, hw, x0, w1);
    if (rc != OGC_OK) return rc;
    OGC_REQUIRE(cout >= 1 && pa && pb && grad_y && moments, "%s: bad shape or null pointer", name);
    if (((uintptr_t)grad_y & 15) != 0) {
        ogc_set_error("%s: grad_y must be 16-byte aligned", name);
        return OGC_ERR_UNSUPPORTED;
    }
    OGC_REQUIRE((long long)cout * hw < (1ll << 31), "%s: one sample exceeds 32-bit indexing", name);
    hipStream_t s = (hipStream_t)stream;
    if (b == 0) return OGC_OK;
    if (ogc_zero_async(moments, sizeof(float) * 2 * (size_t)b * cin * cout, s) != hipSuccess) {
        ogc_set_error("%s: memset failed", name);
        return OGC_ERR_LAUNCH;
    }
    FirstIn first;
    first.x0 = x0; first.w1 = w1; first.c0 = c0;
    const int cp = ogc_first_cp(c0);
#define OGC_MLF(A, C)                                                                                                                    \
    do {                                                                                                                                 \
        if (cp == 3) moments_launch<A, C, float, 3>(b, cin, cout, hw, relu, nullptr, grad_y, pa, pb, nullptr, nullptr, 0, moments, s, first); \
        else if (cp == 6) moments_launch<A, C, float, 6>(b, cin, cout, hw, relu, nullptr, grad_y, pa, pb, nullptr, nullptr, 0, moments, s, first); \
        else moments_launch<A, C, float, 8>(b, cin, cout, hw, relu, nullptr, grad_y, pa, pb, nullptr, nullptr, 0, moments, s, first); \
    } while (0)
    if (cout <= 16 && cin <= 16) OGC_MLF(1, 1);
    else if (cout <= 32 && cin <= 16) OGC_MLF(2, 1);
    else if (cout <= 32) OGC_MLF(2, 2);
    else if (cin <= 16) OGC_MLF(4, 1);
    else OGC_MLF(4, 2);
#undef OGC_MLF
    OGC_CHECK_LAUNCH(name);
    return OGC_OK;
}

extern "C" int ogc_conv1x1_dgrad_adjoint_first(int b, int cin, int cout, int hw, int relu, int c0, const float *w,
                                               const float *grad_y, const float *x0, const float *w1, const float *pa,
                                               const float *pb, const float *coef, float *grad_w1, ogc_stream_t stream) {
    const char *name = "ogc_conv1x1_dgrad_adjoint_first";
    const int rc = ogc_first_check(name, b, cin, c0, hw, x0, w1);
    if (rc != OGC_OK) return rc;
    OGC_REQUIRE(cout >= 1 && w && grad_y && pa && pb && coef && grad_w1, "%s: bad shape or null pointer", name);
    if (cout > 64 || ((uintptr_t)grad_y & 15) != 0) {
        ogc_set_error("%s: needs cout <= 64 and a 16-byte aligned grad_y (cout=%d)", name, cout);
        return OGC_ERR_UNSUPPORTED;
    }
    OGC_REQUIRE((long long)cout * hw < (1ll << 31) && b <= 65535, "%s: one sample exceeds 32-bit indexing", name);
    hipStream_t s = (hipStream_t)stream;
    if (ogc_zero_async(grad_w1, sizeof(float) * (size_t)cin * c0, s) != hipSuccess) {
        ogc_set_error("%s: memset failed", name);
        return OGC_ERR_LAUNCH;
    }
    if (b == 0) return OGC_OK;
    const int M = cin, K = cout, Kq = (K + 3) / 4;
    const size_t lds = ((size_t)64 * ogc_a_ld(Kq) + 64 * 5) * sizeof(float);
    const int tiles = ogc_divup(hw, 64 * WG_WAVES);
    int chunks = 768 / b;
    if (chunks < 1) chunks = 1;
    if (chunks > tiles) chunks = tiles;
    FirstIn first;
    first.x0 = x0; first.w1 = w1; first.c0 = c0; first.dw1 = grad_w1;
    first.run = ogc_divup(tiles, chunks);
    dim3 grid(ogc_divup(tiles, first.run), b);
    const int cp = ogc_first_cp(c0);
#define OGC_DGAF(KQV, CPV)                                                                                                  \
    hipLaunchKernelGGL((dgrad_adjoint_kernel<KQV, false, float, false, CPV>), grid, dim3(WG_WAVES * OGC_WAVE), lds, s, M, K, hw, \
                       relu, w, grad_y, (const float *)nullptr, pa, pb, coef, (const float2 *)nullptr, (const float2 *)nullptr, 0, \
                       (float *)nullptr, first)
    if (Kq <= 8) {
        if (cp == 3) OGC_DGAF(8, 3); else if (cp == 6) OGC_DGAF(8, 6); else OGC_DGAF(8, 8);
    } else {
        if (cp == 3) OGC_DGAF(16, 3); else if (cp == 6) OGC_DGAF(16, 6); else OGC_DGAF(16, 8);
    }
#undef OGC_DGAF
    OGC_CHECK_LAUNCH(name);
    return OGC_OK;
}
```

ogc_amd/fused.py:

```python
import weakref

import torch
import torch.nn.functional as F
from torch.autograd import Function

from .pointnet2 import pointnet2 as _api



import collections as _collections
import functools as _functools

from .utils.zero_arena import zeroed_empty

GATE_MISSES = _collections.Counter()


def deterministic():
    from . import _lib
    return _lib.DETERMINISTIC

ACT16 = __import__("os").environ.get("OGC_ACT16", "1") != "0"


# ... 626 lines not shown
    with torch.no_grad():
        counts = zeroed_empty(PB * K * K, torch.int32, dev)
        iou = torch.empty(PB, K, K, dtype=torch.float32, device=dev)
        nat.mask_iou_wrapper(PB, N, K, mask1.detach(), mask2.detach(), counts, iou)
        both = torch.stack([iou, iou.transpose(1, 2)]).contiguous()
        cols = torch.empty(2 * PB, K, dtype=torch.int32, device=dev)
        nat.lsap_maximize_wrapper(2 * PB, K, both, cols)
    return _MatchedDistance.apply(mask1, mask2, cols[:PB], cols[PB:], int(loss_norm))


FUSED_GN_BACKWARD_MAX_WIDTH = 64
FUSED_GN_BACKWARD = True
ACT16_MOMENT_WIDTH = int(__import__("os").environ.get("OGC_ACT16_MOMENT_WIDTH", "64"))


def _moment_width(t):
    return ACT16_MOMENT_WIDTH if t.dtype is torch.bfloat16 else FUSED_GN_BACKWARD_MAX_WIDTH


def _pool_moment_cout(t):
    return ACT16_MOMENT_WIDTH if t.dtype is torch.bfloat16 else max(FUSED_GN_BACKWARD_MAX_WIDTH, SPARSE_POOL_MAX_COUT)


def _norm_act_conv_forward(y_prev, stats_prev, gn_weight, gn_bias, conv_weight, gn_groups, eps, relu, next_groups, pool,
                           next_gamma):
    nat = _api._native
    B, cin = y_prev.shape[0], y_prev.shape[1]
    cout = conv_weight.shape[0]
    hw = y_prev.numel() // (B * cin)
    dev = y_prev.device
    mean = torch.empty(B * gn_groups, dtype=torch.float32, device=dev)
    rstd = torch.empty_like(mean)
    a = torch.empty(B * cin, dtype=torch.float32, device=dev)
    bb = torch.empty_like(a)
    gamma, beta = gn_weight.contiguous(), gn_bias.contiguous()
    if stats_prev is not None:
        nat.group_norm_coeffs_wrapper(B, cin, hw, gn_groups, eps, None, gamma, beta, stats_prev,
                                      stats_prev.numel() // (2 * B * gn_groups), None, mean, rstd, a, bb)
    else:
        ws = nat.group_norm_ws(B, cin, gn_groups, False, dev)
        nat.group_norm_coeffs_wrapper(B, cin, hw, gn_groups, eps, y_prev, gamma, beta, None, 0, ws, mean, rstd, a, bb)
    y = torch.empty((B, cout) + tuple(y_prev.shape[2:]), dtype=y_prev.dtype, device=dev)
    w = conv_weight.contiguous()
    stats = extremes = None
    if (next_groups > 0 and next_groups <= 32 and cout % next_groups == 0 and (cout // next_groups) % 4 == 0
            and (cin <= 100 or _stats_ok(nat, B, cout, cin, hw, True))):
        stats = zeroed_empty(nat.conv1x1_gn_slots() * B * next_groups * 2, torch.float64, dev)
        if (pool and next_gamma is not None and (cin <= 100 or POOL_EXTREMES_WIDE)
                and getattr(nat, "conv1x1_gemm_affine_pool_wrapper", None) is not None):
            centres = hw // pool
            yext = torch.empty(B, cout, centres, dtype=torch.float32, device=dev)
            aext = torch.empty(B, cout, centres, dtype=torch.int32, device=dev)
            nat.conv1x1_gemm_affine_pool_wrapper(B, cout, cin, hw, relu, next_groups, pool, w, y_prev, a, bb,
                                                 next_gamma.contiguous(), y, stats, yext, aext)
            extremes = (yext, aext)
        else:
            nat.conv1x1_gemm_affine_wrapper(B, cout, cin, hw, relu, next_groups, w, y_prev, a, bb, y, stats)
    else:
        nat.conv1x1_gemm_affine_wrapper(B, cout, cin, hw, relu, 0, w, y_prev, a, bb, y, None)
    return y, stats, extremes, mean, rstd, a, bb


class _NormActConv(Function):

    @staticmethod
    def forward(ctx, y_prev, stats_prev, gn_weight, gn_bias, conv_weight, gn_groups, eps, relu, next_groups, pool=0,
                next_gamma=None):
        ctx.set_materialize_grads(False)
        y_prev = y_prev.contiguous()
        y, stats, extremes, mean, rstd, a, bb = _norm_act_conv_forward(y_prev, stats_prev, gn_weight, gn_bias, conv_weight,
                                                                       gn_groups, eps, relu, next_groups, pool, next_gamma)
        hw = y_prev.numel() // (y_prev.shape[0] * y_prev.shape[1])
        ctx.save_for_backward(y_prev, gn_weight, gn_bias, conv_weight, mean, rstd, a, bb)
        ctx.cfg = (gn_groups, relu, hw)
        if extremes is not None:
            ctx.mark_non_differentiable(stats, *extremes)
            return (y, stats) + extremes
        if stats is not None:
            ctx.mark_non_differentiable(stats)
        return y, stats

    @staticmethod
    def backward(ctx, grad_y, _grad_stats=None, *_grad_extremes):
        if grad_y is None:
            return (None,) * 11
        nat = _api._native
        y_prev, gn_weight, gn_bias, conv_weight, mean, rstd, a, bb = ctx.saved_tensors
        gn_groups, relu, hw = ctx.cfg
        B, cin = y_prev.shape[0], y_prev.shape[1]
        cout = conv_weight.shape[0]
        grad_y = grad_y.contiguous()
        w = conv_weight.contiguous()
        grad_w = zeroed_empty((cout, cin), torch.float32, y_prev.device)
        if (FUSED_GN_BACKWARD and getattr(nat, "conv1x1_dgrad_adjoint_wrapper", None) is not None and hw % 64 == 0
                and cout <= _moment_width(y_prev) and cin <= _moment_width(y_prev) and gn_groups <= 32
                and cin % gn_groups == 0):
            dev = y_prev.device
            moments = zeroed_empty((B, 2, cout, cin), torch.float32, dev)
            nat.conv1x1_wgrad_moments_wrapper(B, cin, cout, hw, relu, y_prev, a, bb, grad_y, moments)
            coef = torch.empty(B, cin, 3, dtype=torch.float32, device=dev)
            ggb = zeroed_empty((2, cin), torch.float32, dev)
            gw, gb = ggb[0], ggb[1]
            nat.gn_moments_combine_wrapper(B, cin, cout, hw, gn_groups, moments, w.view(cout, cin), a, bb, mean, rstd,
                                           gn_weight.contiguous(), grad_w, coef, gw, gb)
            grad_prev = torch.empty_like(y_prev)
            nat.conv1x1_dgrad_adjoint_wrapper(B, cin, cout, hw, relu, w.view(cout, cin), grad_y, y_prev, a, bb, coef, grad_prev)
            return grad_prev, None, gw, gb, grad_w.view_as(conv_weight), None, None, None, None, None, None
        nat.conv1x1_wgrad_affine_wrapper(B, cin, cout, hw, relu, y_prev, a, bb, grad_y, grad_w)
        if y_prev.dtype is torch.bfloat16 or (_gemm_ok(cout, hw) and _plain_gemm_mine(cout, (B, cin, hw))):
            grad_z = torch.empty_like(y_prev)
            nat.conv1x1_gemm_wrapper(B, cin, cout, hw, 1, w, grad_y, grad_z)
        else:
            grad_z = _product(w.view(cout, cin), grad_y.reshape(B, cout, hw), True).view_as(y_prev)
        grad_prev = torch.empty_like(y_prev)
        gw, gb = torch.empty_like(gn_weight), torch.empty_like(gn_bias)
        ws = nat.group_norm_ws(B, cin, gn_groups, True, y_prev.device)
        nat.group_norm_bwd_wrapper(B, cin, hw, gn_groups, relu, y_prev, gn_weight.contiguous(),
                                   gn_bias.contiguous(), mean, rstd, grad_z, grad_prev, gw, gb, ws)
        return grad_prev, None, gw, gb, grad_w.view_as(conv_weight), None, None, None, None, None, None


@_gate
def norm_act_conv_available(y_prev, gn, conv):
    if deterministic():
        return False
    if not (y_prev.is_cuda and _is_act(y_prev) and gn.affine and conv.bias is None and conv.groups == 1
            and all(k == 1 for k in conv.kernel_size) and all(v == 1 for v in conv.stride)
            and all(v == 0 for v in conv.padding)
            and getattr(_api._native, "conv1x1_gemm_affine_wrapper", None) is not None):
        return False
    hw = y_prev.numel() // max(y_prev.shape[0] * y_prev.shape[1], 1)
    if y_prev.dtype is torch.bfloat16 and _api._native.get_matmul_precision() != "bf16":
        return False
    return _gemm_ok(y_prev.shape[1], hw)


def act16_middle_ok(y_prev, gn, conv):
    return norm_act_conv_available(y_prev, gn, conv) and conv.weight.shape[0] <= 160


def norm_act_conv(y_prev, stats_prev, gn, relu, conv, next_gn=None, pool=0):
    next_groups = next_gn.num_groups if (next_gn is not None and next_gn.affine) else 0
    res = _NormActConv.apply(y_prev, stats_prev, gn.weight, gn.bias, conv.weight, gn.num_groups, gn.eps, bool(relu),
                             next_groups, int(pool) if (pool in (16, 32, 64) and next_groups) else 0,
                             next_gn.weight if next_groups else None)
    if pool:
        return res[0], res[1], (tuple(res[2:]) if len(res) > 2 else None)
    return res[0], res[1]


FIRST_PAIR_FUSED = True
FIRST_PAIR_MAX_C0 = 8


class _FirstPairConv(Function):

    @staticmethod
    def forward(ctx, x0, w1, gn_weight, gn_bias, w2, gn_groups, eps, relu, next_groups):
        ctx.set_materialize_grads(False)
        nat = _api._native
        B, c0 = x0.shape[0], x0.shape[1]
        c1, c2 = w1.shape[0], w2.shape[0]
        hw = x0.numel() // (B * c0)
        dev = x0.device
        slots = nat.conv1x1_gn_slots()
        w1c, w2c = w1.contiguous(), w2.contiguous()
        stats1 = zeroed_empty(slots * B * gn_groups * 2, torch.float64, dev)
        nat.first_conv_stats_wrapper(B, c1, c0, hw, gn_groups, x0, w1c, stats1)
        mean = torch.empty(B * gn_groups, dtype=torch.float32, device=dev)
        rstd = torch.empty_like(mean)
        a = torch.empty(B * c1, dtype=torch.float32, device=dev)
        bb = torch.empty_like(a)
        nat.group_norm_coeffs_wrapper(B, c1, hw, gn_groups, eps, None, gn_weight.contiguous(), gn_bias.contiguous(), stats1,
                                      slots, None, mean, rstd, a, bb)
        y2 = torch.empty((B, c2) + tuple(x0.shape[2:]), dtype=torch.float32, device=dev)
        stats2 = zeroed_empty(slots * B * next_groups * 2, torch.float64, dev)
        nat.conv1x1_gemm_affine_first_wrapper(B, c2, c1, hw, relu, next_groups, c0, w2c, x0, w1c, a, bb, y2, stats2)
        ctx.save_for_backward(x0, w1, gn_weight, w2, mean, rstd, a, bb)
        ctx.cfg = (gn_groups, relu, hw)
        ctx.mark_non_differentiable(stats2)
        return y2, stats2

    @staticmethod
    def backward(ctx, grad_y, _grad_stats=None):
        if grad_y is None:
            return (None,) * 9
        nat = _api._native
        x0, w1, gn_weight, w2, mean, rstd, a, bb = ctx.saved_tensors
        gn_groups, relu, hw = ctx.cfg
        B, c0 = x0.shape[0], x0.shape[1]
        c1, c2 = w1.shape[0], w2.shape[0]
        dev = x0.device
        grad_y = grad_y.contiguous()
        w1c, w2c = w1.contiguous().view(c1, c0), w2.contiguous().view(c2, c1)
        moments = zeroed_empty((B, 2, c2, c1), torch.float32, dev)
        nat.conv1x1_wgrad_moments_first_wrapper(B, c1, c2, hw, relu, c0, x0, w1c, a, bb, grad_y, moments)
        grad_w2 = zeroed_empty((c2, c1), torch.float32, dev)
        coef = torch.empty(B, c1, 3, dtype=torch.float32, device=dev)
        ggb = zeroed_empty((2, c1), torch.float32, dev)
        nat.gn_moments_combine_wrapper(B, c1, c2, hw, gn_groups, moments, w2c, a, bb, mean, rstd, gn_weight.contiguous(),
                                       grad_w2, coef, ggb[0], ggb[1])
        grad_w1 = zeroed_empty((c1, c0), torch.float32, dev)
        nat.conv1x1_dgrad_adjoint_first_wrapper(B, c1, c2, hw, relu, c0, w2c, grad_y, x0, w1c, a, bb, coef, grad_w1)
        return None, grad_w1.view_as(w1), ggb[0], ggb[1], grad_w2.view_as(w2), None, None, None, None


def _plain_conv(conv):
    return (conv.bias is None and conv.groups == 1 and all(k == 1 for k in conv.kernel_size)
            and all(v == 1 for v in conv.stride) and all(v == 0 for v in conv.padding))


def first_pair_available(x, conv, gn, conv2, gn2):
    if not FIRST_PAIR_FUSED or deterministic():
        return False
    nat = _api._native
    if (getattr(nat, "conv1x1_dgrad_adjoint_first_wrapper", None) is None or not FUSED_GN_BACKWARD
            or nat.get_matmul_precision() != "fp32"):
        return False
    if not (x is not None and x.is_cuda and x.dtype == torch.float32 and x.is_contiguous() and x.dim() >= 3
            and not x.requires_grad and 1 <= x.shape[1] <= FIRST_PAIR_MAX_C0 and x.shape[0] >= 1):
        return False
    if not (_plain_conv(conv) and _plain_conv(conv2) and gn.affine and gn2.affine):
        return False
    c0, c1, c2 = x.shape[1], conv.weight.shape[0], conv2.weight.shape[0]
    hw = x.numel() // (x.shape[0] * c0)
    g1, g2 = gn.num_groups, gn2.num_groups
    return (conv.weight.shape[1] == c0 and conv2.weight.shape[1] == c1 and hw % 64 == 0
            and c1 <= FUSED_GN_BACKWARD_MAX_WIDTH and c2 <= FUSED_GN_BACKWARD_MAX_WIDTH
            and g1 <= 32 and c1 % g1 == 0 and (c1 // g1) % 4 == 0 and g2 <= 32 and c2 % g2 == 0 and (c2 // g2) % 4 == 0
            and max(c1, c2) * hw < 2 ** 31 and x.shape[0] <= 32768)


def first_pair_conv(x, conv, gn, relu, conv2, gn2):
    return _FirstPairConv.apply(x, conv.weight, gn.weight, gn.bias, conv2.weight, gn.num_groups, gn.eps, bool(relu),
                                gn2.num_groups)


SPARSE_POOL_BACKWARD = True
SPARSE_POOL_MAX_COUT = 64
WIDE_POOL_BACKWARD = _os.environ.get("OGC_WIDE_POOL", "1") != "0"

class _NormActConvPool(Function):

    @staticmethod
    def forward(ctx, y_prev, stats_prev, gn_weight, gn_bias, conv_weight, gn_groups, eps, relu, gn2_weight, gn2_bias,
                groups2, eps2, relu2):
        nat = _api._native
        y_prev = y_prev.contiguous()
        B, cin, P, S = y_prev.shape
        cout = conv_weight.shape[0]
        y, stats, extremes, mean, rstd, a, bb = _norm_act_conv_forward(y_prev, stats_prev, gn_weight, gn_bias, conv_weight,
                                                                       gn_groups, eps, relu, groups2, S, gn2_weight)
        dev = y_prev.device
        out = torch.empty(B, cout, P, dtype=torch.float32, device=dev)
        arg = torch.empty(B, cout, P, dtype=torch.int32, device=dev)
        mean2 = torch.empty(B * groups2, dtype=torch.float32, device=dev)
        rstd2 = torch.empty_like(mean2)
        g2, b2 = gn2_weight.contiguous(), gn2_bias.contiguous()
        nat.group_norm_pool_extremes_wrapper(B, cout, P, S, groups2, eps2, relu2, extremes[0], extremes[1], g2, b2, out, arg,
                                             mean2, rstd2, stats, stats.numel() // (2 * B * groups2))
        ctx.save_for_backward(y_prev, gn_weight, gn_bias, conv_weight, mean, rstd, a, bb, y, gn2_weight, mean2, rstd2, out, arg,
                              extremes[0])
        ctx.cfg = (gn_groups, relu, groups2, relu2)
        return out

    @staticmethod
    def backward(ctx, grad_out):
        nat = _api._native
        (y_prev, gn_weight, gn_bias, conv_weight, mean, rstd, a, bb, y, gn2_weight, mean2, rstd2, out, arg,
         yext) = ctx.saved_tensors
        gn_groups, relu, groups2, relu2 = ctx.cfg
        B, cin, P, S = y_prev.shape
        cout, hw, dev = conv_weight.shape[0], P * S, y_prev.device
        coef2 = torch.empty(B, cout, 2, dtype=torch.float32, device=dev)
        inj = torch.empty(B, cout, P, 2, dtype=torch.float32, device=dev)
        gw2, gb2 = torch.empty_like(gn2_weight), torch.empty_like(gn2_weight)
        ws = nat.group_norm_ws(B, cout, groups2, True, dev)
        nat.group_norm_maxpool_bwd_sparse_wrapper(B, cout, P, S, groups2, relu2, y, gn2_weight.contiguous(), mean2,
                                                  rstd2, out, arg, grad_out.contiguous(), coef2, inj, gw2, gb2, ws,
                                                  yext if POOL_SUMS_FROM_EXTREMES else None)
        w = conv_weight.contiguous().view(cout, cin)
        if cin > _moment_width(y_prev) or cout > _pool_moment_cout(y_prev):
            grad_w = zeroed_empty((cout, cin), torch.float32, dev)
            nat.conv1x1_wgrad_affine_pooled_wrapper(B, cin, cout, hw, relu, S, y_prev, a, bb, y, coef2, inj, grad_w)
            grad_z = torch.empty_like(y_prev)
            nat.conv1x1_dgrad_pooled_wrapper(B, cin, cout, hw, S, w, y, coef2, inj, grad_z)
            grad_prev = torch.empty_like(y_prev)
            gw, gb = torch.empty_like(gn_weight), torch.empty_like(gn_bias)
            ws = nat.group_norm_ws(B, cin, gn_groups, True, dev)
            nat.group_norm_bwd_wrapper(B, cin, hw, gn_groups, relu, y_prev, gn_weight.contiguous(), gn_bias.contiguous(), mean,
                                       rstd, grad_z, grad_prev, gw, gb, ws)
            return (grad_prev, None, gw, gb, grad_w.view_as(conv_weight), None, None, None, gw2, gb2, None, None, None)
        moments = zeroed_empty((B, 2, cout, cin), torch.float32, dev)
        nat.conv1x1_wgrad_moments_pooled_wrapper(B, cin, cout, hw, relu, S, y_prev, a, bb, y, coef2, inj, moments)
        coef = torch.empty(B, cin, 3, dtype=torch.float32, device=dev)
        ggb = zeroed_empty((2, cin), torch.float32, dev)
        gw, gb = ggb[0], ggb[1]
        grad_w = torch.empty(cout, cin, dtype=torch.float32, device=dev)
        nat.gn_moments_combine_wrapper(B, cin, cout, hw, gn_groups, moments, w, a, bb, mean, rstd,
                                       gn_weight.contiguous(), grad_w, coef, gw, gb)
        grad_prev = torch.empty_like(y_prev)
        nat.conv1x1_dgrad_adjoint_pooled_wrapper(B, cin, cout, hw, relu, S, w, y, coef2, inj, y_prev, a, bb, coef, grad_prev)
        return (grad_prev, None, gw, gb, grad_w.view_as(conv_weight), None, None, None, gw2, gb2, None, None, None)


@_gate
def norm_act_conv_pool_available(y_prev, gn, conv, next_gn):
    nat = _api._native
    if not (SPARSE_POOL_BACKWARD and FUSED_GN_BACKWARD and y_prev.dim() == 4 and y_prev.shape[-1] in (16, 32, 64)
            and next_gn is not None and next_gn.affine and norm_act_conv_available(y_prev, gn, conv)
            and getattr(nat, "conv1x1_dgrad_adjoint_pooled_wrapper", None) is not None
            and getattr(nat, "conv1x1_gemm_affine_pool_wrapper", None) is not None):
        return False
    cin, cout, g, g2 = y_prev.shape[1], conv.weight.shape[0], gn.num_groups, next_gn.num_groups
    if cin > _moment_width(y_prev) or cout > _pool_moment_cout(y_prev):
        B, hw = y_prev.shape[0], y_prev.shape[2] * y_prev.shape[3]
        return (WIDE_POOL_BACKWARD and getattr(nat, "conv1x1_dgrad_pooled_wrapper", None) is not None
                and hw % 64 == 0 and B * (hw // 64) >= 1024 and B <= 65535
                and g <= 32 and cin % g == 0 and g2 <= 32 and cout % g2 == 0 and (cout // g2) % 4 == 0
                and (cin <= 100 or (POOL_EXTREMES_WIDE and _stats_ok(nat, B, cout, cin, hw, True))))
    kq = (cout + 3) // 4
    lds = (64 * 4 * (kq | 1) + 320) * 4 + 4 * cout * (64 // y_prev.shape[-1]) * 16
    return (lds <= 65536 and (y_prev.shape[2] * y_prev.shape[3]) % 64 == 0 and cin <= _moment_width(y_prev)
            and cout <= _pool_moment_cout(y_prev) and g <= 32 and cin % g == 0
            and g2 <= 32 and cout % g2 == 0 and (cout // g2) % 4 == 0)


def norm_act_conv_pool(y_prev, stats_prev, gn, relu, conv, next_gn, next_relu):
    return _NormActConvPool.apply(y_prev, stats_prev, gn.weight, gn.bias, conv.weight, gn.num_groups, gn.eps, bool(relu),
                                  next_gn.weight, next_gn.bias, next_gn.num_groups, next_gn.eps, bool(next_relu))


class _SelfAttentionCore(Function):

    @staticmethod
    def forward(ctx, qkv, n_head):
        nat = _api._native
        qkv = qkv.contiguous()
        B, L, E3 = qkv.shape
        E = E3 // 3
        out = torch.empty(B, L, E, dtype=torch.float32, device=qkv.device)
        prob = torch.empty(B, n_head, L, L, dtype=torch.float32, device=qkv.device)
        scale = (E // n_head) ** -0.5
        nat.attention_fwd_wrapper(n_head, scale, qkv[:, :, :E], qkv[:, :, E:2 * E], qkv[:, :, 2 * E:], out, prob)
        ctx.save_for_backward(qkv, out, prob)
        ctx.cfg = (n_head, scale)
        return out

    @staticmethod
    def backward(ctx, grad_out):
        qkv, out, prob = ctx.saved_tensors
        n_head, scale = ctx.cfg
        E = qkv.shape[2] // 3
        grad = torch.empty_like(qkv)
        _api._native.attention_bwd_wrapper(n_head, scale, qkv[:, :, :E], qkv[:, :, E:2 * E], qkv[:, :, 2 * E:], out, prob,
                                           grad_out.contiguous(), grad[:, :, :E], grad[:, :, E:2 * E], grad[:, :, 2 * E:])
        return grad, None


class _CrossAttentionCore(Function):

    @staticmethod
    def forward(ctx, q, kv, n_head):
        nat = _api._native
        q, kv = q.contiguous(), kv.contiguous()
        B, Lq, E = q.shape
        Lk = kv.shape[1]
        out = torch.empty(B, Lq, E, dtype=torch.float32, device=q.device)
        prob = torch.empty(B, n_head, Lq, Lk, dtype=torch.float32, device=q.device)
        scale = (E // n_head) ** -0.5
        nat.attention_fwd_wrapper(n_head, scale, q, kv[:, :, :E], kv[:, :, E:], out, prob)
        ctx.save_for_backward(q, kv, out, prob)
        ctx.cfg = (n_head, scale)
        return out

    @staticmethod
    def backward(ctx, grad_out):
        q, kv, out, prob = ctx.saved_tensors
        n_head, scale = ctx.cfg
        E = q.shape[2]
        gq, gkv = torch.empty_like(q), torch.empty_like(kv)
        _api._native.attention_bwd_wrapper(n_head, scale, q, kv[:, :, :E], kv[:, :, E:], out, prob, grad_out.contiguous(),
                                           gq, gkv[:, :, :E], gkv[:, :, E:])
        return gq, gkv, None


class _SlotMasks(Function):

    @staticmethod
    def forward(ctx, feats, slots, temperature):
        feats, slots = feats.contiguous(), slots.contiguous()
        B, D, N = feats.shape
        mask = torch.empty(B, N, slots.shape[2], dtype=torch.float32, device=feats.device)
        _api._native.slot_masks_fwd_wrapper(temperature, feats, slots, mask)
        ctx.save_for_backward(feats, slots, mask)
        ctx.temperature = temperature
        return mask

    @staticmethod
    def backward(ctx, grad_mask):
        feats, slots, mask = ctx.saved_tensors
        gf, gs = torch.empty_like(feats), torch.empty_like(slots)
        _api._native.slot_masks_bwd_wrapper(ctx.temperature, feats, slots, mask, grad_mask.contiguous(), gf, gs)
        return gf, gs, None


@_gate
def slot_masks_available(feats, slots):
    return (getattr(_api._native, "slot_masks_fwd_wrapper", None) is not None and feats.dim() == 3 and slots.dim() == 3
            and feats.shape[1] == slots.shape[1] <= 256 and 0 < slots.shape[2] <= 32 and feats.shape[2] > 0
            and all(t.is_cuda and t.dtype == torch.float32 for t in (feats, slots)))


def slot_masks(feats, slots, temperature=0.05):
    return _SlotMasks.apply(feats, slots, float(temperature))


@_gate
def attention_core_available(embed_dim, n_head, lq, lk, *tensors):
    nat = _api._native
    return (getattr(nat, "attention_fwd_wrapper", None) is not None and embed_dim % n_head == 0
            and embed_dim // n_head in (16, 32) and 4 * (lq * lk + 2 * lq * (embed_dim // n_head) + lq + 4) <= 64 * 1024
            and all(t.is_cuda and t.dtype == torch.float32 for t in tensors))


class _SmallLinear(Function):

    @staticmethod
    def forward(ctx, x, weight, bias):
        x2 = x.reshape(-1, x.shape[-1]).contiguous()
        weight = weight.contiguous()
        y = torch.empty(x2.shape[0], weight.shape[0], dtype=torch.float32, device=x.device)
        _api._native.small_linear_fwd_wrapper(x2, weight, None if bias is None else bias.contiguous(), y)
        ctx.save_for_backward(x2, weight)
        ctx.shape = x.shape
        ctx.has_bias = bias is not None
        return y.view(*x.shape[:-1], weight.shape[0])

    @staticmethod
    def backward(ctx, gy):
        x2, weight = ctx.saved_tensors
        gy2 = gy.reshape(-1, gy.shape[-1]).contiguous()
        gx = torch.empty_like(x2) if ctx.needs_input_grad[0] else None
        gw = torch.empty_like(weight) if ctx.needs_input_grad[1] else None
        gb = torch.empty(weight.shape[0], dtype=torch.float32, device=gy.device) \
            if (ctx.has_bias and ctx.needs_input_grad[2]) else None
        if gx is not None or gw is not None or gb is not None:
            _api._native.small_linear_bwd_wrapper(x2, weight, gy2, gx, gw, gb)
        return (None if gx is None else gx.view(ctx.shape)), gw, gb


_SMALL_LINEAR_ROWS = 1024


def small_linear(x, weight, bias=None):
    if (x.is_cuda and x.dtype == torch.float32 and weight.dtype == torch.float32 and x.dim() >= 2
            and 0 < x.numel() // x.shape[-1] <= _SMALL_LINEAR_ROWS
            and getattr(_api._native, "small_linear_fwd_wrapper", None) is not None):
        return _SmallLinear.apply(x, weight, bias)
    return F.linear(x, weight, bias)


class _ManyRowsLinear(Function):

    @staticmethod
    def forward(ctx, x, weight, bias):
        ctx.save_for_backward(x, weight)
        return F.linear(x, weight, bias)

    @staticmethod
    def backward(ctx, gy):
        x, weight = ctx.saved_tensors
        gx = gw = gb = None
        if ctx.needs_input_grad[0]:
            gx = gy.matmul(weight)
        if ctx.needs_input_grad[1]:
            gw = torch.bmm(gy.transpose(1, 2), x).sum(0)
        if ctx.needs_input_grad[2]:
            gb = gy.sum(1).sum(0)
        return gx, gw, gb


def many_rows_linear(x, weight, bias):
# ... 159 lines not shown
```

ogc_amd/pointnet2_cuda.py:

```python
import torch

from . import _lib


def _check(t, dtype, name):
    try:
        if t.is_cuda and t.dtype is dtype and t.is_contiguous():
            return t.data_ptr()
    except AttributeError:
        pass
    if not isinstance(t, torch.Tensor):
        raise TypeError("%s must be a torch.Tensor" % name)
    if t.device.type != "cuda":
        raise RuntimeError("%s must be a CUDA tensor (HIP device); ogc_amd has no CPU path" % name)
    if not t.is_contiguous():
        raise RuntimeError("%s must be contiguous" % name)
    if t.dtype != dtype:
        raise RuntimeError("%s must be %s, got %s" % (name, dtype, t.dtype))
    return t.data_ptr()


def _f(t, name):
    return _check(t, torch.float32, name)

# ... 524 lines not shown

def _opt(t, dtype, name):
    return 0 if t is None else _check(t, dtype, name)


def batch_norm_fwd_wrapper(b, c, hw, eps, relu, training, momentum, x, gamma, beta, running_mean, running_var, y, mean,
                           rstd, ws, stats, slots):
    _run("ogc_batch_norm_fwd", x, b, c, hw, float(eps), int(relu), int(training), float(momentum), _f(x, "x"),
         _f(gamma, "gamma"), _f(beta, "beta"), _opt(running_mean, torch.float32, "running_mean"),
         _opt(running_var, torch.float32, "running_var"), _f(y, "y"), _opt(mean, torch.float32, "mean"),
         _opt(rstd, torch.float32, "rstd"), _opt(ws, torch.float64, "ws"), _opt(stats, torch.float64, "stats"), int(slots))


def batch_norm_bwd_wrapper(b, c, hw, relu, training, x, gamma, beta, mean, rstd, grad_y, grad_x, grad_gamma, grad_beta,
                           ws):
    _run("ogc_batch_norm_bwd", x, b, c, hw, int(relu), int(training), _f(x, "x"), _f(gamma, "gamma"), _f(beta, "beta"),
         _f(mean, "mean"), _f(rstd, "rstd"), _f(grad_y, "grad_y"), _f(grad_x, "grad_x"), _f(grad_gamma, "grad_gamma"),
         _f(grad_beta, "grad_beta"), _check(ws, torch.float64, "ws"))


def batch_norm_maxpool_fwd_wrapper(b, c, p, s, eps, relu, training, momentum, x, gamma, beta, running_mean, running_var,
                                   out, argmax, mean, rstd, ws, stats, slots):
    _run("ogc_batch_norm_maxpool_fwd", x, b, c, p, s, float(eps), int(relu), int(training), float(momentum), _f(x, "x"),
         _f(gamma, "gamma"), _f(beta, "beta"), _opt(running_mean, torch.float32, "running_mean"),
         _opt(running_var, torch.float32, "running_var"), _f(out, "out"), _i(argmax, "argmax"),
         _opt(mean, torch.float32, "mean"), _opt(rstd, torch.float32, "rstd"), _opt(ws, torch.float64, "ws"),
         _opt(stats, torch.float64, "stats"), int(slots))


def batch_norm_maxpool_bwd_wrapper(b, c, p, s, relu, training, x, gamma, mean, rstd, out, argmax, grad_out, grad_x,
                                   grad_gamma, grad_beta, ws):
    _run("ogc_batch_norm_maxpool_bwd", x, b, c, p, s, int(relu), int(training), _f(x, "x"), _f(gamma, "gamma"),
         _f(mean, "mean"), _f(rstd, "rstd"), _f(out, "out"), _i(argmax, "argmax"), _f(grad_out, "grad_out"),
         _f(grad_x, "grad_x"), _f(grad_gamma, "grad_gamma"), _f(grad_beta, "grad_beta"), _check(ws, torch.float64, "ws"))


def group_norm_coeffs_wrapper(b, c, hw, groups, eps, x, gamma, beta, stats, slots, ws, mean, rstd, a, bb):
    _run("ogc_group_norm_coeffs", gamma, b, c, hw, groups, float(eps), _opt(x, torch.float32, "x"), _f(gamma, "gamma"),
         _f(beta, "beta"), _opt(stats, torch.float64, "stats"), int(slots), _opt(ws, torch.float64, "ws"),
         _f(mean, "mean"), _f(rstd, "rstd"), _f(a, "a"), _f(bb, "bb"))


def conv1x1_gemm_affine_wrapper(b, M, K, hw, relu, groups, w, inp, pa, pb, out, stats):
    h, (ip, op) = _acts((inp, out), ("in", "out"))
    _run("ogc_conv1x1_gemm_affine" + h, inp, b, M, K, hw, int(relu), int(groups), _f(w, "w"), ip, _f(pa, "pa"),
         _f(pb, "pb"), op, _opt(stats, torch.float64, "stats"))


def conv1x1_gemm_affine_pool_wrapper(b, M, K, hw, relu, groups, nsample, w, inp, pa, pb, next_gamma, out, stats, yext,
                                     aext):
    h, (ip, op) = _acts((inp, out), ("in", "out"))
    _run("ogc_conv1x1_gemm_affine_pool" + h, inp, b, M, K, hw, int(relu), int(groups), int(nsample), _f(w, "w"),
         ip, _f(pa, "pa"), _f(pb, "pb"), _f(next_gamma, "next_gamma"), op,
         _check(stats, torch.float64, "stats"), _f(yext, "yext"), _i(aext, "aext"))


def group_norm_pool_extremes_wrapper(b, c, p, s, groups, eps, relu, yext, aext, gamma, beta, out, argmax, mean, rstd,
                                     stats, slots):
    _run("ogc_group_norm_pool_extremes", yext, b, c, p, s, groups, float(eps), int(relu), _f(yext, "yext"),
         _i(aext, "aext"), _f(gamma, "gamma"), _f(beta, "beta"), _f(out, "out"), _i(argmax, "argmax"), _f(mean, "mean"),
         _f(rstd, "rstd"), _check(stats, torch.float64, "stats"), int(slots))


def conv1x1_wgrad_affine_wrapper(b, cin, cout, hw, relu, x, pa, pb, dy, dw):
    h, (xp, dyp) = _acts((x, dy), ("x", "dy"))
    _run("ogc_conv1x1_wgrad_affine" + h, x, b, cin, cout, hw, int(relu), xp, _f(pa, "pa"), _f(pb, "pb"), dyp, _f(dw, "dw"))


def _rows(t, name):
    if not isinstance(t, torch.Tensor) or t.device.type != "cuda" or t.dtype != torch.float32 or t.dim() != 3:
        raise RuntimeError("%s must be a 3-D float32 CUDA tensor" % name)
    ld = t.stride(1)
    if t.stride(2) != 1 or ld < t.shape[2] or (t.shape[0] > 1 and t.stride(0) != t.shape[1] * ld):
        raise RuntimeError("%s must be a column slice of a contiguous (b, l, W) tensor" % name)
    return t.data_ptr(), ld


def attention_fwd_wrapper(h, scale, q, k, v, out, prob):
    b, lq, e = q.shape
    lk = k.shape[1]
    (qp, ldq), (kp, ldk), (vp, ldv) = _rows(q, "q"), _rows(k, "k"), _rows(v, "v")
    _run("ogc_attention_fwd", q, b, lq, lk, h, e // h, float(scale), qp, ldq, kp, ldk, vp, ldv, _f(out, "out"),
         _f(prob, "prob"))


def attention_bwd_wrapper(h, scale, q, k, v, out, prob, dout, dq, dk, dv):
    b, lq, e = q.shape
    lk = k.shape[1]
    (qp, ldq), (kp, ldk), (vp, ldv) = _rows(q, "q"), _rows(k, "k"), _rows(v, "v")
    (dqp, lddq), (dkp, lddk), (dvp, lddv) = _rows(dq, "dq"), _rows(dk, "dk"), _rows(dv, "dv")
    _run("ogc_attention_bwd", q, b, lq, lk, h, e // h, float(scale), qp, ldq, kp, ldk, vp, ldv, _f(out, "out"),
         _f(prob, "prob"), _f(dout, "dout"), dqp, lddq, dkp, lddk, dvp, lddv)


def conv1x1_wgrad_moments_wrapper(b, cin, cout, hw, relu, y_prev, pa, pb, grad_y, moments):
    h, (yp, gp) = _acts((y_prev, grad_y), ("y_prev", "grad_y"))
    _run("ogc_conv1x1_wgrad_moments" + h, y_prev, b, cin, cout, hw, int(relu), yp, _f(pa, "pa"), _f(pb, "pb"), gp,
         _f(moments, "moments"))


def gn_moments_combine_wrapper(b, cin, cout, hw, groups, moments, w, pa, pb, mean, rstd, gamma, grad_w, coef, gw, gb):
    _run("ogc_gn_moments_combine", moments, b, cin, cout, hw, groups, _f(moments, "moments"), _f(w, "w"), _f(pa, "pa"),
         _f(pb, "pb"), _f(mean, "mean"), _f(rstd, "rstd"), _f(gamma, "gamma"), _f(grad_w, "grad_w"), _f(coef, "coef"),
         _f(gw, "grad_gamma"), _f(gb, "grad_beta"))


def conv1x1_dgrad_adjoint_wrapper(b, cin, cout, hw, relu, w, grad_y, y_prev, pa, pb, coef, grad_prev):
    h, (gp, yp, op) = _acts((grad_y, y_prev, grad_prev), ("grad_y", "y_prev", "grad_prev"))
    _run("ogc_conv1x1_dgrad_adjoint" + h, grad_y, b, cin, cout, hw, int(relu), _f(w, "w"), gp, yp, _f(pa, "pa"), _f(pb, "pb"),
         _f(coef, "coef"), op)


def first_conv_stats_wrapper(b, c1, c0, hw, groups, x0, w1, stats):
    _run("ogc_first_conv_stats", x0, b, c1, c0, hw, groups, _f(x0, "x0"), _f(w1, "w1"), _check(stats, torch.float64, "stats"))


def conv1x1_gemm_affine_first_wrapper(b, M, K, hw, relu, groups, c0, w, x0, w1, pa, pb, out, stats):
    _run("ogc_conv1x1_gemm_affine_first", x0, b, M, K, hw, int(relu), groups, c0, _f(w, "w"), _f(x0, "x0"), _f(w1, "w1"),
         _f(pa, "pa"), _f(pb, "pb"), _f(out, "out"), _check(stats, torch.float64, "stats"))


def conv1x1_wgrad_moments_first_wrapper(b, cin, cout, hw, relu, c0, x0, w1, pa, pb, grad_y, moments):
    _run("ogc_conv1x1_wgrad_moments_first", x0, b, cin, cout, hw, int(relu), c0, _f(x0, "x0"), _f(w1, "w1"), _f(pa, "pa"),
         _f(pb, "pb"), _f(grad_y, "grad_y"), _f(moments, "moments"))


def conv1x1_dgrad_adjoint_first_wrapper(b, cin, cout, hw, relu, c0, w, grad_y, x0, w1, pa, pb, coef, grad_w1):
    _run("ogc_conv1x1_dgrad_adjoint_first", x0, b, cin, cout, hw, int(relu), c0, _f(w, "w"), _f(grad_y, "grad_y"), _f(x0, "x0"),
         _f(w1, "w1"), _f(pa, "pa"), _f(pb, "pb"), _f(coef, "coef"), _f(grad_w1, "grad_w1"))


def group_norm_maxpool_bwd_sparse_wrapper(b, c, p, s, groups, relu, x, gamma, mean, rstd, out, argmax, grad_out, coef2, inj,
                                          grad_gamma, grad_beta, ws, x_at_argmax=None):
    h, (xp,) = _acts((x,), ("x",))
    _run("ogc_group_norm_maxpool_bwd_sparse" + h, x, b, c, p, s, groups, int(relu), xp,
         _opt(x_at_argmax, torch.float32, "x_at_argmax"), _f(gamma, "gamma"),
         _f(mean, "mean"), _f(rstd, "rstd"), _f(out, "out"), _i(argmax, "argmax"), _f(grad_out, "grad_out"),
         _f(coef2, "coef2"), _f(inj, "inj"), _f(grad_gamma, "grad_gamma"), _f(grad_beta, "grad_beta"),
         _check(ws, torch.float64, "ws"))


def conv1x1_wgrad_moments_pooled_wrapper(b, cin, cout, hw, relu, nsample, y_prev, pa, pb, y, coef2, inj, moments):
    h, (ypp, yp) = _acts((y_prev, y), ("y_prev", "y"))
    _run("ogc_conv1x1_wgrad_moments_pooled" + h, y_prev, b, cin, cout, hw, int(relu), nsample, ypp, _f(pa, "pa"),
         _f(pb, "pb"), yp, _f(coef2, "coef2"), _f(inj, "inj"), _f(moments, "moments"))


def conv1x1_dgrad_adjoint_pooled_wrapper(b, cin, cout, hw, relu, nsample, w, y, coef2, inj, y_prev, pa, pb, coef, grad_prev):
    h, (yp, ypp, op) = _acts((y, y_prev, grad_prev), ("y", "y_prev", "grad_prev"))
    _run("ogc_conv1x1_dgrad_adjoint_pooled" + h, y, b, cin, cout, hw, int(relu), nsample, _f(w, "w"), yp,
         _f(coef2, "coef2"), _f(inj, "inj"), ypp, _f(pa, "pa"), _f(pb, "pb"), _f(coef, "coef"), op)


def mlp_chain_pool_supported(c0, c1, c2, c3, nsample):
    return bool(_lib.load().ogc_mlp_chain_pool_supported(c0, c1, c2, c3, nsample))


def mlp_chain_pool_wrapper(x, wts, biases, out):
    B, c0, P, S = x.shape
    c = [w.shape[1] for w in wts] + [0]
    _run("ogc_mlp_chain_pool", x, B, c0, c[0], c[1], c[2] if len(wts) > 2 else 0, P, S, _f(x, "x"),
         _f(wts[0], "wt1"), _f(biases[0], "b1"), _f(wts[1], "wt2"), _f(biases[1], "b2"),
         _f(wts[2], "wt3") if len(wts) > 2 else None, _f(biases[2], "b3") if len(wts) > 2 else None, _f(out, "out"))


def corr_layer_pool_supported(cf, c1, c2, c3, nsample):
    return bool(_lib.load().ogc_corr_layer_pool_supported(cf, c1, c2, c3, nsample))


def corr_layer_pool_wrapper(pos1, pos2, feat1, feat2, idx, wts, biases, out):
    B, cf, n1 = feat1.shape
    _run("ogc_corr_layer_pool", feat1, B, cf, wts[0].shape[1], wts[1].shape[1], wts[2].shape[1], n1, feat2.shape[2],
         idx.shape[2], _f(pos1, "pos1"), _f(pos2, "pos2"), _f(feat1, "feat1"), _f(feat2, "feat2"), _i(idx, "idx"),
         _f(wts[0], "wt1"), _f(biases[0], "b1"), _f(wts[1], "wt2"), _f(biases[1], "b2"), _f(wts[2], "wt3"),
         _f(biases[2], "b3"), _f(out, "out"))


def small_linear_fwd_wrapper(x, weight, bias, y):
    rows, n_in = x.shape
    _run("ogc_small_linear_fwd", x, rows, n_in, weight.shape[0], _f(x, "x"), _f(weight, "weight"),
         None if bias is None else _f(bias, "bias"), _f(y, "y"))


def small_linear_bwd_wrapper(x, weight, grad_y, grad_x, grad_weight, grad_bias):
    rows, n_in = x.shape
    _run("ogc_small_linear_bwd", x, rows, n_in, weight.shape[0], _f(x, "x"), _f(weight, "weight"), _f(grad_y, "grad_y"),
         None if grad_x is None else _f(grad_x, "grad_x"), None if grad_weight is None else _f(grad_weight, "grad_weight"),
         None if grad_bias is None else _f(grad_bias, "grad_bias"))


def slot_masks_fwd_wrapper(temperature, feats, slots, mask):
    b, d, n = feats.shape
    _run("ogc_slot_masks_fwd", feats, b, d, n, slots.shape[2], float(temperature), _f(feats, "feats"),
         _f(slots, "slots"), _f(mask, "mask"))


def slot_masks_bwd_wrapper(temperature, feats, slots, mask, grad_mask, grad_feats, grad_slots):
    b, d, n = feats.shape
    k = slots.shape[2]
    ws = torch.empty(max(int(_lib.load().ogc_slot_masks_ws_floats(b, d, n, k)), 1), dtype=torch.float32,
                     device=feats.device)
    _run("ogc_slot_masks_bwd", feats, b, d, n, k, float(temperature), _f(feats, "feats"), _f(slots, "slots"),
         _f(mask, "mask"), _f(grad_mask, "grad_mask"), _f(grad_feats, "grad_feats"), _f(grad_slots, "grad_slots"),
         _f(ws, "ws"))


def group_norm_ws(b, c, groups, backward, device):
    L = _lib.load()
    n = 2 * b * c * L.ogc_group_norm_bwd_slots() if backward else 2 * b * groups * L.ogc_group_norm_stats_slots()
    return torch.empty(max(n, 1), dtype=torch.float64, device=device)


_precision = "fp32"


def set_matmul_precision(mode):
    global _precision
    if mode not in ("fp32", "bf16"):
        raise ValueError("matmul precision must be 'fp32' or 'bf16'")
    previous = "bf16" if _lib.load().ogc_set_matmul_precision(1 if mode == "bf16" else 0) else "fp32"
    _precision = mode
    return previous


def get_matmul_precision():
    return _precision


def conv1x1_gemm_stream_supported(b, m, k, hw):
    return bool(_lib.load().ogc_conv1x1_gemm_stream_supported(int(b), int(m), int(k), int(hw)))


def conv1x1_gemm_stats_supported(b, m, k, hw, affine):
    return bool(_lib.load().ogc_conv1x1_gemm_stats_supported(int(b), int(m), int(k), int(hw), 1 if affine else 0))


def conv1x1_gn_slots():
    return _lib.load().ogc_conv1x1_gn_slots()


def conv1x1_gemm_gnstats_wrapper(b, M, K, hw, groups, w, inp, out, stats):
    _run("ogc_conv1x1_gemm_gnstats", inp, b, M, K, hw, groups, _f(w, "w"), _f(inp, "in"), _f(out, "out"),
         _check(stats, torch.float64, "stats"))


def group_norm_fwd_stats_wrapper(b, c, hw, groups, eps, relu, x, gamma, beta, y, mean, rstd, stats, slots):
    _run("ogc_group_norm_fwd_stats", x, b, c, hw, groups, float(eps), int(relu), _f(x, "x"), _f(gamma, "gamma"),
         _f(beta, "beta"), _f(y, "y"), _f(mean, "mean"), _f(rstd, "rstd"), _check(stats, torch.float64, "stats"),
         int(slots))


def group_norm_maxpool_fwd_stats_wrapper(b, c, p, s, groups, eps, relu, x, gamma, beta, out, argmax, mean, rstd, stats,
                                         slots):
    _run("ogc_group_norm_maxpool_fwd_stats", x, b, c, p, s, groups, float(eps), int(relu), _f(x, "x"),
         _f(gamma, "gamma"), _f(beta, "beta"), _f(out, "out"), _i(argmax, "argmax"), _f(mean, "mean"),
         _f(rstd, "rstd"), _check(stats, torch.float64, "stats"), int(slots))


def conv1x1_gemm_wrapper(b, M, K, hw, transpose_a, w, inp, out):
    h, (ip, op) = _acts((inp, out), ("in", "out"))
    _run("ogc_conv1x1_gemm" + h, inp, b, M, K, hw, int(transpose_a), _f(w, "w"), ip, op)


def conv1x1_gemm_any_wrapper(b, M, K, hw, transpose_a, w, inp, out):
    _run("ogc_conv1x1_gemm_any", inp, b, M, K, hw, int(transpose_a), _f(w, "w"), _f(inp, "in"), _f(out, "out"))


def conv1x1_wgrad_affine_pooled_wrapper(b, cin, cout, hw, relu, nsample, x, pa, pb, y, coef2, inj, dw):
    h, (xp, yp) = _acts((x, y), ("x", "y"))
    _run("ogc_conv1x1_wgrad_affine_pooled" + h, x, b, cin, cout, hw, int(relu), nsample, xp, _f(pa, "pa"), _f(pb, "pb"),
         yp, _f(coef2, "coef2"), _f(inj, "inj"), _f(dw, "dw"))


def conv1x1_dgrad_pooled_wrapper(b, cin, cout, hw, nsample, w, y, coef2, inj, grad_z):
    h, (yp, gp) = _acts((y, grad_z), ("y", "grad_z"))
    _run("ogc_conv1x1_dgrad_pooled" + h, y, b, cin, cout, hw, nsample, _f(w, "w"), yp, _f(coef2, "coef2"), _f(inj, "inj"), gp)
```

ogc_amd/utils/nn_util.py:

```python
import numpy as np
import torch
import torch.nn as nn


class GroupNorm(nn.Sequential):

    def __init__(self, in_size, num_groups, name=""):
        super().__init__()
        gn = nn.GroupNorm(num_groups, in_size)
        nn.init.ones_(gn.weight)
        nn.init.zeros_(gn.bias)
        self.add_module(name + "gn", gn)


class _BatchNormNd(nn.Sequential):
    _cls = None

    def __init__(self, in_size, name=""):
        super().__init__()
        bn = self._cls(in_size)
        nn.init.ones_(bn.weight)
        nn.init.zeros_(bn.bias)
        self.add_module(name + "bn", bn)


class BatchNorm1d(_BatchNormNd):
    _cls = nn.BatchNorm1d


class BatchNorm2d(_BatchNormNd):
    _cls = nn.BatchNorm2d


def get_norm_layer(layer_def, dimension, **kwargs):
    if layer_def is None:
        return nn.Identity()
    spec = dict(kwargs)
    spec.update(layer_def)
    kind = spec.pop("class")
    if kind == "GroupNorm":
        return GroupNorm(**spec)
    if kind == "BatchNorm":
        return (BatchNorm1d, BatchNorm2d)[dimension - 1](**spec)
    raise KeyError(kind)


def _assemble(seq, name, main_name, main, norm, activation, preact):
    tail = []
    if norm is not None:
        tail.append((name + "normlayer", norm))
    if activation is not None:
        tail.append((name + "activation", activation))
    order = tail + [(name + main_name, main)] if preact else [(name + main_name, main)] + tail
    for key, mod in order:
        seq.add_module(key, mod)


class _ConvNd(nn.Sequential):
    _conv = None
    _dim = None

    def __init__(self, in_size, out_size, kernel_size, stride, padding, dilation, activation, bn, init, bias,
                 preact, name):
        super().__init__()
        use_bias = bias and (bn is None)
        conv = self._conv(in_size, out_size, kernel_size=kernel_size, stride=stride, padding=padding,
                          dilation=dilation, bias=use_bias)
        init(conv.weight)
        if use_bias:
            nn.init.zeros_(conv.bias)
        norm = None
        if bn is not None:
            norm = get_norm_layer(bn, self._dim, in_size=in_size if preact else out_size)
        _assemble(self, name, "conv", conv, norm, activation, preact)
        self._gn_fuse = (not preact and isinstance(norm, GroupNorm)
                         and (activation is None or type(activation) is nn.ReLU))
        self._names = (name + "conv", name + "normlayer", activation is not None)

    def forward(self, input):
        if self._gn_fuse:
            from ..fused import group_norm_act, pointwise_conv
            conv_name, norm_name, relu = self._names
            gn = getattr(self, norm_name)[0]
            y, stats = pointwise_conv(input, getattr(self, conv_name), gn)
            return group_norm_act(y, gn, relu, stats)
        from ..fused import pointwise_conv
        x = input
        for mod in self:
            x = pointwise_conv(x, mod) if isinstance(mod, (nn.Conv1d, nn.Conv2d)) else mod(x)
        return x

    def forward_maxpool(self, input):
        if self._gn_fuse:
            from ..fused import group_norm_act_maxpool, pointwise_conv
            conv_name, norm_name, relu = self._names
            gn = getattr(self, norm_name)[0]
            y, stats = pointwise_conv(input, getattr(self, conv_name), gn)
            return group_norm_act_maxpool(y, gn, relu, stats)
        return self.forward(input).max(dim=-1)[0]


class Conv1d(_ConvNd):
    _conv, _dim = nn.Conv1d, 1

    def __init__(self, in_size, out_size, kernel_size=1, stride=1, padding=0, dilation=1,
                 activation=nn.ReLU(inplace=True), bn=None, init=nn.init.kaiming_normal_, bias=True,
                 preact=False, name=""):
        super().__init__(in_size, out_size, kernel_size, stride, padding, dilation, activation, bn, init, bias,
                         preact, name)


class Conv2d(_ConvNd):
    _conv, _dim = nn.Conv2d, 2

    def __init__(self, in_size, out_size, kernel_size=(1, 1), stride=(1, 1), padding=(0, 0), dilation=(1, 1),
                 activation=nn.ReLU(inplace=True), bn=None, init=nn.init.kaiming_normal_, bias=True,
                 preact=False, name=""):
        super().__init__(in_size, out_size, kernel_size, stride, padding, dilation, activation, bn, init, bias,
                         preact, name)


class FC(nn.Sequential):

    def __init__(self, in_size, out_size, activation=nn.ReLU(inplace=True), bn=None, init=None, preact=False,
                 name=""):
        super().__init__()
        fc = nn.Linear(in_size, out_size, bias=bn is None)
        if init is not None:
            init(fc.weight)
        if bn is None:
            nn.init.zeros_(fc.bias)
        norm = None
        if bn is not None:
            norm = get_norm_layer(bn, 1, in_size=in_size if preact else out_size)
        _assemble(self, name, "fc", fc, norm, activation, preact)


class SharedMLP(nn.Sequential):

    def __init__(self, args, bn=None, activation=nn.ReLU(inplace=True), preact=False, first=False, name=""):
        super().__init__()
        for i, (c_in, c_out) in enumerate(zip(args[:-1], args[1:])):
            bare = first and preact and i == 0
            self.add_module(name + "layer%d" % i,
                            Conv2d(c_in, c_out, bn=None if bare else bn, activation=None if bare else activation,
                                   preact=preact))


def _shared_mlp_run(self, x, pool, first=None):
    from ..fused import (act16_middle_ok, group_norm_act, group_norm_act_maxpool, norm_act_conv, norm_act_conv_available,
                         norm_act_conv_pool, norm_act_conv_pool_available, pointwise_conv)
    layers = list(self.children())
    pending = None

    def flush(p, last):
        y, stats, gn, relu, extremes = p
        if y.dtype is torch.bfloat16:
            from ..fused import act16_leave
            y, extremes = act16_leave(y), None
        if last and pool:
            return group_norm_act_maxpool(y, gn, relu, stats, extremes)
        return group_norm_act(y, gn, relu, stats)

    def block(layer):
        conv_name, norm_name, relu = layer._names
        return getattr(layer, conv_name), getattr(layer, norm_name)[0], relu

    skip = False
    for li, layer in enumerate(layers):
        if skip:
            skip = False
            continue
        fusable = isinstance(layer, _ConvNd) and layer._gn_fuse
        if (fusable and li == 0 and first is None and len(layers) >= 2 + (1 if pool else 0)
                and isinstance(layers[1], _ConvNd) and layers[1]._gn_fuse):
            from ..fused import first_pair_available, first_pair_conv
            (conv, gn, relu), (conv2, gn2, relu2) = block(layer), block(layers[1])
            if first_pair_available(x, conv, gn, conv2, gn2):
                y, stats = first_pair_conv(x, conv, gn, relu, conv2, gn2)
                pending, skip = (y, stats, gn2, relu2, None), True
                continue
        if not fusable:
            if pending is not None:
                x, pending = flush(pending, False), None
            x = layer(x)
            continue
        conv_name, norm_name, relu = layer._names
        conv, gn = getattr(layer, conv_name), getattr(layer, norm_name)[0]
        extremes = None
        if pending is not None and pending[0].dtype is torch.bfloat16:
            tail = pool and li == len(layers) - 1
            ok = (norm_act_conv_pool_available(pending[0], pending[2], conv, gn) if tail else
                  (act16_middle_ok(pending[0], pending[2], conv) and li < len(layers) - 1))
            if not ok:
                from ..fused import act16_leave
                pending = (act16_leave(pending[0]),) + tuple(pending[1:4]) + (None,)
        if pending is not None and norm_act_conv_available(pending[0], pending[2], conv):
            if pool and li == len(layers) - 1 and pending[0].dim() == 4 and pending[0].shape[-1] in (16, 32, 64):
                if norm_act_conv_pool_available(pending[0], pending[2], conv, gn):
                    return norm_act_conv_pool(pending[0], pending[1], pending[2], pending[3], conv, gn, relu)
                y, stats, extremes = norm_act_conv(pending[0], pending[1], pending[2], pending[3], conv, gn,
                                                   pool=pending[0].shape[-1])
            else:
                y, stats = norm_act_conv(pending[0], pending[1], pending[2], pending[3], conv, gn)
        else:
            if pending is not None:
                x, pending = flush(pending, False), None
            y, stats = first(conv, gn) if (first is not None and li == 0) else pointwise_conv(x, conv, gn)
        pending = (y, stats, gn, relu, extremes)
    if pending is not None:
        return flush(pending, True)
    return x.max(dim=-1)[0] if pool else x


def _shared_mlp_forward(self, x):
    return _shared_mlp_run(self, x, False)


def _shared_mlp_forward_maxpool(self, x, first=None):
    return _shared_mlp_run(self, x, True, first)


def _shared_mlp_first_layer(self):
    layers = list(self.children())
    if not layers or not (isinstance(layers[0], _ConvNd) and layers[0]._gn_fuse):
        return None
    conv_name, norm_name, _ = layers[0]._names
    return getattr(layers[0], conv_name), getattr(layers[0], norm_name)[0]


SharedMLP.forward = _shared_mlp_forward
SharedMLP.forward_maxpool = _shared_mlp_forward_maxpool
SharedMLP.first_layer = _shared_mlp_first_layer


def knead_leading_dims(n_dim: int, data: torch.Tensor):
    if data is None:
        return None
    shape = list(data.size())
    return data.view(int(np.prod(shape[:n_dim])), *shape[n_dim:])


def break_leading_dim(dim_size: list, data: torch.Tensor):
    if data is None:
        return None
    return data.view(*dim_size, *list(data.size())[1:])


class Seq(nn.Sequential):

    def __init__(self, input_channels):
        super().__init__()
        self.count = 0
        self.current_channels = input_channels

    def _push(self, module, out_channels=None):
        self.add_module(str(self.count), module)
        self.count += 1
        if out_channels is not None:
            self.current_channels = out_channels
        return self

    def conv1d(self, out_size, kernel_size=1, stride=1, padding=0, dilation=1, activation=nn.ReLU(inplace=True),
               leaky=False, bn=None, init=nn.init.kaiming_normal_, bias=True, preact=False, name=""):
        if leaky:
            activation = nn.LeakyReLU(0.1, inplace=True)
        return self._push(Conv1d(self.current_channels, out_size, kernel_size=kernel_size, stride=stride,
                                 padding=padding, dilation=dilation, activation=activation, bn=bn, init=init,
                                 bias=bias, preact=preact, name=name), out_size)

    def conv2d(self, out_size, kernel_size=(1, 1), stride=(1, 1), padding=(0, 0), dilation=(1, 1),
               activation=nn.ReLU(inplace=True), bn=None, init=nn.init.kaiming_normal_, bias=True, preact=False,
               name=""):
        return self._push(Conv2d(self.current_channels, out_size, kernel_size=kernel_size, stride=stride,
                                 padding=padding, dilation=dilation, activation=activation, bn=bn, init=init,
                                 bias=bias, preact=preact, name=name), out_size)

    def fc(self, out_size, activation=nn.ReLU(inplace=True), bn=None, init=None, preact=False, name=""):
        return self._push(FC(self.current_channels, out_size, activation=activation, bn=bn, init=init,
                             preact=preact, name=name), out_size)

    def dropout(self, p=0.5):
        return self._push(nn.Dropout(p=p))

    def maxpool2d(self, kernel_size, stride=None, padding=0, dilation=1, return_indices=False, ceil_mode=False):
        return self._push(nn.MaxPool2d(kernel_size=kernel_size, stride=stride, padding=padding, dilation=dilation,
                                       return_indices=return_indices, ceil_mode=ceil_mode))
```

ogc_amd/utils/pointnet2_util.py:

```python
import torch
import torch.nn as nn

from ..pointnet2.pointnet2 import (GroupAll, QueryAndGroup, furthest_point_sample, furthest_point_sample_chain, gather_nd,
                                   knn_radius_clamp,
                                   three_interpolate, three_nn)
from .nn_util import SharedMLP


FPS_CHAIN_SHORTCUT = True


class _PointnetSAModuleBase(nn.Module):

    def __init__(self):
        super().__init__()
        self.npoint = None
        self.groupers = None
        self.mlps = None

    def plan_geometry(self, xyz, parent_ties=None):
        if self.npoint is None:
            return None
        plan = self.plan_sampling(xyz, parent_ties)
        plan["idx"] = self.plan_neighbours(xyz, plan["new_xyz"])
        plan["rev"] = self.plan_reverse(plan["idx"], xyz.shape[1])
        return plan

    def plan_reverse(self, idx, n):
        from .. import fused as _fused
        group_reverse = _fused.group_reverse
        if not torch.is_grad_enabled():
            return [None] * len(idx)
        want = lambda j: j is not None and j.is_cuda and j.shape[1] * j.shape[2] >= _fused.GROUP_GRAD_GATHER_MIN_FANIN * n
        return [group_reverse(j.int().contiguous(), n) if want(j) else None for j in idx]

    def plan_sampling(self, xyz, parent_ties=None):
        new_inds, ties = furthest_point_sample_chain(xyz, self.npoint, parent_ties if FPS_CHAIN_SHORTCUT else None)
        new_inds = new_inds.long()
        new_xyz = gather_nd(xyz, new_inds)
        return {"new_inds": new_inds, "new_xyz": new_xyz, "ties": ties}

    def plan_neighbours(self, xyz, new_xyz):
        knn, idx = {}, []
        reach = {}
        for grouper in self.groupers:
            if isinstance(grouper, QueryAndGroup):
                r = reach.get(grouper.nsample, 0.0)
                reach[grouper.nsample] = None if (r is None or grouper.radius is None) else max(r, grouper.radius)
        for grouper in self.groupers:
            if not isinstance(grouper, QueryAndGroup):
                idx.append(None)
                continue
            if grouper.nsample not in knn:
                knn[grouper.nsample] = knn_radius_clamp(grouper.nsample, reach[grouper.nsample], new_xyz, xyz)
            dist, nn_idx = knn[grouper.nsample]
            if grouper.radius is not None:
                nn_idx = torch.where(dist > grouper.radius, nn_idx[:, :, :1], nn_idx)
            idx.append(nn_idx.contiguous())
        return idx

    def forward(self, xyz, features=None, return_inds=False, geometry=None):
        if geometry is None:
            geometry = self.plan_geometry(xyz)
        elif hasattr(geometry, "get"):
            geometry = geometry.get()
        if geometry is not None and "idx" not in geometry:
            geometry = dict(geometry, idx=self.plan_neighbours(xyz, geometry["new_xyz"]))
        if geometry is not None and "rev" not in geometry:
            geometry = dict(geometry, rev=self.plan_reverse(geometry["idx"], xyz.shape[1]))
        new_xyz = geometry["new_xyz"] if geometry is not None else None
        new_inds = geometry["new_inds"] if geometry is not None else None

        from ..fused import first_level_plain, grouped_first_layer, grouped_first_layer_available
        pooled = []
        for i, (grouper, mlp) in enumerate(zip(self.groupers, self.mlps)):
            if isinstance(grouper, QueryAndGroup):
                nn_idx = geometry["idx"][i]
                head = mlp.first_layer() if (grouper.use_xyz and xyz.is_cuda and not first_level_plain(features)) else None
                if head is not None and grouped_first_layer_available(xyz, new_xyz, features, nn_idx, head[0], head[1]):
                    pooled.append(mlp.forward_maxpool(None, first=lambda conv, gn, j=nn_idx, rv=geometry["rev"][i]:
                                                      grouped_first_layer(xyz, new_xyz, features, j, conv, gn, rv,
                                                                          act16=len(mlp) >= 2)))
                    continue
                grouped = grouper(xyz, new_xyz, features, idx=nn_idx)[0]
            else:
                grouped = grouper(xyz, new_xyz, features)[0]
            pooled.append(mlp.forward_maxpool(grouped))
        new_features = torch.cat(pooled, dim=1) if len(pooled) != 1 else pooled[0]
        if return_inds:
            return new_xyz, new_features, new_inds
        return new_xyz, new_features


class PointnetSAModuleMSG(_PointnetSAModuleBase):

    def __init__(self, npoint, radii, nsamples, mlps, bn, use_xyz=True):
        super().__init__()
        assert len(radii) == len(nsamples) == len(mlps)
        self.npoint = npoint
        self.groupers = nn.ModuleList()
        self.mlps = nn.ModuleList()
        for radius, nsample, mlp_spec in zip(radii, nsamples, mlps):
            self.groupers.append(QueryAndGroup(radius, nsample, use_xyz=use_xyz) if npoint is not None
                                 else GroupAll(use_xyz))
            if use_xyz:
                mlp_spec[0] += 3
            self.mlps.append(SharedMLP(mlp_spec, bn=bn))


class PointnetSAModule(PointnetSAModuleMSG):

    def __init__(self, mlp, npoint, radius, nsample, bn, use_xyz=True):
        super().__init__(npoint=npoint, radii=[radius], nsamples=[nsample], mlps=[mlp], bn=bn, use_xyz=use_xyz)


class PointnetFPModule(nn.Module):

    def __init__(self, mlp, bn):
        super().__init__()
        self.mlp = SharedMLP(mlp, bn=bn)

    @staticmethod
    def plan_geometry(unknown, known):
        dist, idx = three_nn(unknown.contiguous(), known.contiguous())
        dist_recip = 1.0 / (dist + 1e-8)
        weight = dist_recip / dist_recip.sum(dim=2, keepdim=True)
        idx, weight = idx.contiguous(), weight.contiguous()
        rev = None
        if torch.is_grad_enabled() and idx.is_cuda and (3 * idx.shape[1]) % 16 == 0:
            from ..fused import group_reverse
            rev = group_reverse(idx.int() if idx.dtype != torch.int32 else idx, known.shape[1])
        return {"idx": idx, "weight": weight, "rev": rev}

    def forward(self, unknown, known, unknow_feats, known_feats, geometry=None):
        if known is not None:
            if geometry is None:
                geometry = self.plan_geometry(unknown, known)
            elif hasattr(geometry, "get"):
                geometry = geometry.get()
            interpolated = three_interpolate(known_feats.contiguous(), geometry["idx"], geometry["weight"],
                                             geometry.get("rev"))
        else:
            interpolated = known_feats.expand(*known_feats.size()[0:2], unknown.size(1))
        if unknow_feats is not None:
            interpolated = torch.cat([interpolated, unknow_feats], dim=1)
        return self.mlp(interpolated.unsqueeze(-1)).squeeze(-1)
```

Baseline: 1653 point-clouds/s.

## Skip duplicate-neighbour steps in pooled MLP backward via live-step lists

Adds a kernel that scans ball-query neighbour indices and builds, per centre, a compact list of 16-sample steps that hold distinct neighbours, with a multiplicity weight for the trailing padded duplicates. The pooled and first-layer weight-gradient and data-gradient backward kernels gain a list-driven variant that iterates only over live steps and scales the last lane by the folded duplicate count. This avoids redundant backward work on padded repeated neighbours. The cost is an extra planning kernel, indirection in the inner loops, and reliance on duplicates being exact repeats of the first index.

```diff
diff --git a/include/ogc_ops.h b/include/ogc_ops.h
--- a/include/ogc_ops.h
+++ b/include/ogc_ops.h
@@ -239,6 +239,23 @@
 int ogc_conv1x1_dgrad_adjoint_pooled(int b, int cin, int cout, int hw, int relu, int nsample, const float *w, const float *y,
                                      const float *coef2, const float *inj, const float *y_prev, const float *pa,
                                      const float *pb, const float *coef, float *grad_prev, ogc_stream_t stream);
+
+int ogc_live_steps(int b, int p, int nsample, const int *idx, int *live, int *n_live, ogc_stream_t stream);
+int ogc_conv1x1_wgrad_moments_pooled_live(int b, int cin, int cout, int hw, int relu, int nsample, const float *y_prev,
+                                          const float *pa, const float *pb, const float *y, const float *coef2,
+                                          const float *inj, const int *live, const int *n_live, int live_cap, float *moments,
+                                          ogc_stream_t stream);
+int ogc_conv1x1_dgrad_adjoint_pooled_live(int b, int cin, int cout, int hw, int relu, int nsample, const float *w, const float *y,
+                                          const float *coef2, const float *inj, const float *y_prev, const float *pa,
+                                          const float *pb, const float *coef, const int *live, const int *n_live, int live_cap,
+                                          float *grad_prev, ogc_stream_t stream);
+int ogc_conv1x1_wgrad_moments_first_live(int b, int cin, int cout, int hw, int relu, int c0, int nsample, const float *x0,
+                                         const float *w1, const float *pa, const float *pb, const float *grad_y,
+                                         const int *live, const int *n_live, int live_cap, float *moments, ogc_stream_t stream);
+int ogc_conv1x1_dgrad_adjoint_first_live(int b, int cin, int cout, int hw, int relu, int c0, int nsample, const float *w,
+                                         const float *grad_y, const float *x0, const float *w1, const float *pa, const float *pb,
+                                         const float *coef, const int *live, const int *n_live, int live_cap, float *grad_w1,
+                                         ogc_stream_t stream);
 
 int ogc_mlp_chain_pool_supported(int c0, int c1, int c2, int c3, int nsample);
 int ogc_mlp_chain_pool(int b, int c0, int c1, int c2, int c3, int p, int nsample, const float *x, const float *wt1,
diff --git a/ogc_amd/_lib.py b/ogc_amd/_lib.py
--- a/ogc_amd/_lib.py
+++ b/ogc_amd/_lib.py
@@ -115,8 +115,17 @@
                                        _vp, _vp, _vp],
     "ogc_conv1x1_wgrad_moments_pooled": [_int, _int, _int, _int, _int, _int, _vp, _vp, _vp, _vp, _vp, _vp, _vp, _vp],
     "ogc_conv1x1_dgrad_adjoint_pooled": [_int, _int, _int, _int, _int, _int, _vp, _vp, _vp, _vp, _vp, _vp, _vp, _vp, _vp, _vp],
+    "ogc_live_steps": [_int, _int, _int, _vp, _vp, _vp, _vp],
+    "ogc_conv1x1_wgrad_moments_pooled_live": [_int, _int, _int, _int, _int, _int, _vp, _vp, _vp, _vp, _vp, _vp, _vp, _vp, _int, _vp,
+                                              _vp],
+    "ogc_conv1x1_dgrad_adjoint_pooled_live": [_int, _int, _int, _int, _int, _int, _vp, _vp, _vp, _vp, _vp, _vp, _vp, _vp, _vp, _vp,
+                                              _int, _vp, _vp],
+    "ogc_conv1x1_wgrad_moments_first_live": [_int, _int, _int, _int, _int, _int, _int, _vp, _vp, _vp, _vp, _vp, _vp, _vp, _int, _vp,
+                                             _vp],
+    "ogc_conv1x1_dgrad_adjoint_first_live": [_int, _int, _int, _int, _int, _int, _int, _vp, _vp, _vp, _vp, _vp, _vp, _vp, _vp, _vp,
+                                             _int, _vp, _vp],
     "ogc_mlp_chain_pool_supported": [_int, _int, _int, _int, _int],
-    "ogc_mlp_chain_pool": [_int, _int, _int, _int, _int, _int, _int, _vp, _vp, _vp, _vp, _vp, _vp, _vp, _vp, _vp],
+    "ogc_mlp_chain_pool":[_int, _int, _int, _int, _int, _int, _int, _vp, _vp, _vp, _vp, _vp, _vp, _vp, _vp, _vp],
     "ogc_corr_layer_pool_supported": [_int, _int, _int, _int, _int],
     "ogc_corr_layer_pool": [_int, _int, _int, _int, _int, _int, _int, _int, _vp, _vp, _vp, _vp, _vp, _vp, _vp, _vp, _vp, _vp,
                             _vp, _vp, _vp],
diff --git a/ogc_amd/csrc/gn_fused_bwd.hip b/ogc_amd/csrc/gn_fused_bwd.hip
--- a/ogc_amd/csrc/gn_fused_bwd.hip
+++ b/ogc_amd/csrc/gn_fused_bwd.hip
@@ -4,7 +4,56 @@
 
 namespace {
 
-template <int COB, int CIB, bool POOLED, typename AT = float, int FIRST = 0>
+constexpr int LIVE_SHIFT = 28;
+constexpr int LIVE_MASK = (1 << LIVE_SHIFT) - 1;
+struct LiveIn {
+    const int *steps = nullptr;
+    const int *n = nullptr;
+    int cap = 0;
+};
+
+constexpr int LIVE_MAX_P = 32768;
+__global__ __launch_bounds__(1024) void live_steps_kernel(int p, int s, const int *__restrict__ idx, int *__restrict__ steps,
+                                                          int *__restrict__ n_live) {
+    __shared__ int part[1024];
+    __shared__ unsigned char cnt[LIVE_MAX_P];
+    const int t = threadIdx.x, b = blockIdx.x, T = s >> 4;
+    const int lane = t & 63, wave = t >> 6;
+    const int *ib = idx + (size_t)b * p * s;
+    int *out = steps + (size_t)b * p * T;
+    const int row0 = lane & ~(s - 1);
+    const unsigned long long row_mask = (s == 64 ? ~0ull : (1ull << s) - 1ull) << row0;
+    const int total = p * s;
+    for (int e0 = wave * 64; e0 < total; e0 += 1024) {
+        const bool in = e0 + lane < total;
+        const int v = in ? ib[e0 + lane] : 0;
+        const int first = __shfl(v, row0);
+        const unsigned long long differs = __builtin_amdgcn_ballot_w64(in && v != first) & row_mask;
+        const int hi = differs ? 63 - __clzll(differs) - row0 : 0;
+        if (in && lane == row0) cnt[(e0 + lane) / s] = (unsigned char)(min((hi + 1) >> 4, T - 1) + 1);
+    }
+    __syncthreads();
+    const int per = (p + 1023) / 1024;
+    const int c0 = min(t * per, p), c1 = min(c0 + per, p);
+    int sum = 0;
+    for (int c = c0; c < c1; ++c) sum += cnt[c];
+    part[t] = sum;
+    __syncthreads();
+    for (int off = 1; off < 1024; off <<= 1) {
+        const int v = t >= off ? part[t - off] : 0;
+        __syncthreads();
+        part[t] += v;
+        __syncthreads();
+    }
+    int at = t > 0 ? part[t - 1] : 0;
+    for (int c = c0; c < c1; ++c) {
+        const int sl = cnt[c] - 1;
+        for (int st = 0; st <= sl; ++st) out[at++] = (c * T + st) | (st == sl ? (T - 1 - sl) << LIVE_SHIFT : 0);
+    }
+    if (t == 1023) n_live[b] = part[1023];
+}
+
+template <int COB, int CIB, bool POOLED, typename AT = float, int FIRST = 0, bool LIST = false>
 __global__ __launch_bounds__(WG_WAVES *OGC_WAVE) void wgrad_moments_kernel(int cin, int cout, int hw, int chunks,
                                                                            int steps_per_wave, int relu,
                                                                            const AT *__restrict__ x,
@@ -15,14 +64,22 @@
                                                                            const float2 *__restrict__ inj,
                                                                            int s_shift,
                                                                            float *__restrict__ hm,
-                                                                           FirstIn first = FirstIn()) {
+                                                                           FirstIn first = FirstIn(), LiveIn ls = LiveIn()) {
     constexpr int XN = FIRST ? FIRST : CIB;
     __shared__ float red[WG_WAVES][COB * CIB * 256];
     const int lane = threadIdx.x & 63, wave = __builtin_amdgcn_readfirstlane(threadIdx.x >> 6);
     const int i = lane & 15, k = lane >> 4;
     const int img = blockIdx.x / chunks, chunk = blockIdx.x - img * chunks;
     const int co0 = blockIdx.y * (16 * COB), ci0 = blockIdx.z * (16 * CIB);
-    const int steps_per_img = hw >> 4;
+    int steps_per_img = hw >> 4;
+    const int *lv_ = nullptr;
+    if constexpr (LIST) {
+        steps_per_img = min(ls.n[img], ls.cap);
+        lv_ = ls.steps + (size_t)img * ls.cap;
+        const int waves = chunks * WG_WAVES;
+        steps_per_wave = ((steps_per_img + waves - 1) / waves + 1) & ~1;
+        if (chunk * WG_WAVES * steps_per_wave >= steps_per_img) return;
+    }
     const int first_step = (chunk * WG_WAVES + wave) * steps_per_wave;
     const int mine = max(0, min(steps_per_wave, steps_per_img - first_step));
 
@@ -70,8 +127,10 @@
                           : x + (size_t)img * cin * hw + 4 * k;
     int cur = min(first_step, steps_per_img - 1);
     const int stop = min(first_step + mine, steps_per_img) - 1;
-    auto load = [&](float4(&yv)[COB], float4(&xv)[XN], float2(&jv)[COB], int &jpos) {
-        const int pb = cur * 16;
+    int ent = LIST ? lv_[cur] : 0;
+    auto load = [&](float4(&yv)[COB], float4(&xv)[XN], float2(&jv)[COB], int &jpos, int &went) {
+        const int pb = LIST ? min(ent & LIVE_MASK, (hw >> 4) - 1) * 16 : cur * 16;
+        if constexpr (LIST) went = ent;
 #pragma unroll
         for (int a = 0; a < COB; ++a) yv[a] = ogc_ld4(yb_ + yrow[a] + pb);
 #pragma unroll
@@ -82,11 +141,17 @@
             jpos = (pb & smask) + 4 * k;
         }
         cur = min(cur + 1, max(stop, 0));
+        if constexpr (LIST) ent = lv_[cur];
     };
-    auto fma16 = [&](float4(&yv)[COB], const float4(&xraw)[XN], const float2(&jv)[COB], int jpos) {
+    auto fma16 = [&](float4(&yv)[COB], const float4(&xraw)[XN], const float2(&jv)[COB], int jpos, int went) {
         if (POOLED) {
 #pragma unroll
             for (int a = 0; a < COB; ++a) ogc_pooled_grad(yv[a], pc2[a], pc3[a], jv[a], jpos);
+        }
+        if constexpr (LIST) {
+            const float wl = k == 3 ? (float)(1 + 16 * (went >> LIVE_SHIFT)) : 1.f;
+#pragma unroll
+            for (int a = 0; a < COB; ++a) yv[a].w *= wl;
         }
         float4 x0v[FIRST ? FIRST : 1];
         if constexpr (FIRST > 0) {
@@ -125,15 +190,16 @@
     float4 ya[COB], xa[XN], yb[COB], xb[XN];
     float2 ja[COB], jb[COB];
     int pa_ = 0, pb_ = 0;
-    load(ya, xa, ja, pa_);
+    int wa_ = 0, wb_ = 0;
+    load(ya, xa, ja, pa_, wa_);
     int s = 0;
     for (; s + 1 < mine; s += 2) {
-        load(yb, xb, jb, pb_);
-        fma16(ya, xa, ja, pa_);
-        load(ya, xa, ja, pa_);
-        fma16(yb, xb, jb, pb_);
-    }
-    if (s < mine) fma16(ya, xa, ja, pa_);
+        load(yb, xb, jb, pb_, wb_);
+        fma16(ya, xa, ja, pa_, wa_);
+        load(ya, xa, ja, pa_, wa_);
+        fma16(yb, xb, jb, pb_, wb_);
+    }
+    if (s < mine) fma16(ya, xa, ja, pa_, wa_);
 
     float *dst = hm + (size_t)img * 2 * cout * cin;
 #pragma unroll
@@ -305,7 +371,7 @@
 template <int COB, int CIB, typename AT, int FIRST = 0>
 void moments_launch(int b, int cin, int cout, int hw, int relu, const AT *x, const AT *dy, const float *pa,
                     const float *pb, const float *coef2, const float *inj, int s_shift, float *hm, hipStream_t s,
-                    FirstIn first = FirstIn()) {
+                    FirstIn first = FirstIn(), LiveIn ls = LiveIn()) {
     const int steps_per_img = sizeof(AT) == 2 ? hw >> 5 : hw >> 4;
     const int tiles = ogc_divup(cout, 16 * COB) * ogc_divup(cin, 16 * CIB);
     long long waves = (2048 / tiles) / b;
@@ -324,10 +390,17 @@
             hipLaunchKernelGGL((wgrad_moments16_kernel<COB, CIB, false>), grid, dim3(WG_WAVES * OGC_WAVE), 0, s, cin, cout, hw,
                                chunks, spw, relu, x, dy, pa, pb, c2, ij, 0, hm);
     } else if constexpr (FIRST > 0) {
-        hipLaunchKernelGGL((wgrad_moments_kernel<COB, CIB, false, AT, FIRST>), grid, dim3(WG_WAVES * OGC_WAVE), 0, s, cin, cout, hw,
-                           chunks, spw, relu, x, dy, pa, pb, c2, ij, 0, hm, first);
+        if (ls.steps)
+            hipLaunchKernelGGL((wgrad_moments_kernel<COB, CIB, false, AT, FIRST, true>), grid, dim3(WG_WAVES * OGC_WAVE), 0, s, cin, cout,
+                               hw, chunks, spw, relu, x, dy, pa, pb, c2, ij, 0, hm, first, ls);
+        else
+            hipLaunchKernelGGL((wgrad_moments_kernel<COB, CIB, false, AT, FIRST>), grid, dim3(WG_WAVES * OGC_WAVE), 0, s, cin, cout, hw,
+                               chunks, spw, relu, x, dy, pa, pb, c2, ij, 0, hm, first, ls);
     } else {
-        if (inj)
+        if (inj && ls.steps)
+            hipLaunchKernelGGL((wgrad_moments_kernel<COB, CIB, true, AT, 0, true>), grid, dim3(WG_WAVES * OGC_WAVE), 0, s, cin, cout, hw,
+                               chunks, spw, relu, x, dy, pa, pb, c2, ij, s_shift, hm, first, ls);
+        else if (inj)
             hipLaunchKernelGGL((wgrad_moments_kernel<COB, CIB, true, AT>), grid, dim3(WG_WAVES * OGC_WAVE), 0, s, cin, cout, hw, chunks,
                                spw, relu, x, dy, pa, pb, c2, ij, s_shift, hm);
         else
@@ -402,7 +475,7 @@
     }
 }
 
-template <int KQ, bool POOLED, typename AT = float, bool BF = false, int FIRST = 0>
+template <int KQ, bool POOLED, typename AT = float, bool BF = false, int FIRST = 0, bool LIST = false>
 __global__ __launch_bounds__(WG_WAVES *OGC_WAVE) void dgrad_adjoint_kernel(int M, int K, int hw, int relu,
                                                                            const float *__restrict__ w,
                                                                            const AT *__restrict__ gy,
@@ -414,7 +487,7 @@
                                                                            const float2 *__restrict__ inj,
                                                                            int s_shift,
                                                                            AT *__restrict__ out,
-                                                                           FirstIn first = FirstIn()) {
+                                                                           FirstIn first = FirstIn(), LiveIn ls = LiveIn()) {
     extern __shared__ __attribute__((aligned(16))) float a_lds[];
     __shared__ __attribute__((aligned(16))) float s_w1[FIRST ? FC_MAX_ROWS * FC_MAX_C0 : 4];
     __shared__ float s_dw[FIRST ? FC_MAX_ROWS * FC_MAX_C0 : 4];
@@ -427,39 +500,67 @@
     const AT *yb = yprev + (size_t)b * M * hw;
     const int a_ld = ogc_a_ld(Kq);
     float *cf = a_lds + (size_t)64 * a_ld;
+    int run = FIRST ? first.run : 1;
+    int n_lv = 0;
+    const int *lv_ = nullptr;
+    if constexpr (LIST) {
+        static_assert((POOLED || FIRST > 0) && !BF && sizeof(AT) == 4, "list form: pooled or first-layer, fp32");
+        n_lv = min(ls.n[b], ls.cap);
+        lv_ = ls.steps + (size_t)b * ls.cap;
+        const int tiles = (n_lv + 4 * WG_WAVES - 1) / (4 * WG_WAVES);
+        if (FIRST) run = (tiles + (int)gridDim.x - 1) / (int)gridDim.x;
+        if ((int)blockIdx.x * run >= tiles) return;
+    }
     if constexpr (FIRST > 0) {
         static_assert(!POOLED && !BF && sizeof(AT) == 4, "first-layer form: dense, fp32");
         ogc_first_stage_w1<WG_WAVES * OGC_WAVE>(s_w1, first.w1, M, first.c0);
         for (int t = threadIdx.x; t < FC_MAX_ROWS * FC_MAX_C0; t += WG_WAVES * OGC_WAVE) s_dw[t] = 0.f;
     }
-    const int run = FIRST ? first.run : 1;
     for (int it = 0; it < run; ++it) {
-    const int p0 = ((blockIdx.x * run + it) * WG_WAVES + wave) * 64;
-    const bool live = p0 < hw;
+    const int tw = (blockIdx.x * run + it) * WG_WAVES + wave;
+    const int p0 = tw * 64;
+    const bool live = LIST ? 4 * tw < n_lv : p0 < hw;
+    int pos = p0 + 4 * j;
+    bool mine_ok = true;
+    float wl = 1.f;
+    if constexpr (LIST) {
+        const int q = 4 * tw + (j >> 2);
+        mine_ok = q < n_lv;
+        const int ent = lv_[min(q, n_lv - 1)];
+        pos = min(ent & LIVE_MASK, (hw >> 4) - 1) * 16 + 4 * (j & 3);
+        wl = (j & 3) == 3 ? (float)(1 + 16 * (ent >> LIVE_SHIFT)) : 1.f;
+    }
+    const bool lane_live = live && mine_ok;
     float4 x0v[FIRST ? FIRST : 1];
     if constexpr (FIRST > 0) {
-        ogc_first_load_raw<FIRST>(x0v, first.x0 + (size_t)b * first.c0 * hw + (live ? p0 + 4 * j : 0), first.c0, hw);
-        ogc_first_mask<FIRST>(x0v, first.c0, live);
+        ogc_first_load_raw<FIRST>(x0v, first.x0 + (size_t)b * first.c0 * hw + (live ? pos : 0), first.c0, hw);
+        ogc_first_mask<FIRST>(x0v, first.c0, lane_live);
     }
 
     float4 xin[KQ];
 #pragma unroll
     for (int q = 0; q < KQ; ++q) {
         const int row = q * 4 + kk;
-        xin[q] = (live && q < Kq && row < K) ? ogc_ld4(inb + (size_t)row * hw + p0 + 4 * j) : make_float4(0.f, 0.f, 0.f, 0.f);
+        xin[q] = (lane_live && q < Kq && row < K) ? ogc_ld4(inb + (size_t)row * hw + pos) : make_float4(0.f, 0.f, 0.f, 0.f);
     }
     if (POOLED) {
-        const int centres = hw >> s_shift, cpw = 64 >> s_shift;
+        const int centres = hw >> s_shift, cpw = LIST ? 4 : 64 >> s_shift;
         float4 *tab = reinterpret_cast<float4 *>(cf + 64 * 5) + (size_t)wave * K * cpw;
         for (int e = lane; e < K * cpw; e += OGC_WAVE) {
-            const int row = e / cpw, centre = (p0 >> s_shift) + (e - row * cpw);
+            const int row = e / cpw;
+            int centre = (p0 >> s_shift) + (e - row * cpw);
+            if constexpr (LIST) {
+                const int q = 4 * tw + (e - row * cpw);
+                const int step = min(lv_[min(q, n_lv - 1)] & LIVE_MASK, (hw >> 4) - 1);
+                centre = q < n_lv ? (step * 16) >> s_shift : centres;
+            }
             const float2 cc = coef2[(size_t)b * K + row];
             const float2 jj = (live && centre < centres) ? inj[((size_t)b * K + row) * centres + centre]
                                                          : make_float2(0.f, __int_as_float(-1));
             tab[e] = make_float4(cc.x, cc.y, jj.x, jj.y);
         }
         __syncthreads();
-        const int mine = (4 * j) >> s_shift, jpos = (p0 + 4 * j) & ((1 << s_shift) - 1);
+        const int mine = LIST ? j >> 2 : (4 * j) >> s_shift, jpos = pos & ((1 << s_shift) - 1);
 #pragma unroll
         for (int q = 0; q < KQ; ++q) {
             const int row = q * 4 + kk;
@@ -520,7 +621,7 @@
                         ogc_first_w1_row<FIRST>(w1r, s_w1, m);
                         yv[r] = ogc_first_row<FIRST>(x0v, w1r);
                     } else {
-                        yv[r] = (live && m < M) ? ogc_ld4(yb + (size_t)m * hw + p0 + 4 * j) : make_float4(0.f, 0.f, 0.f, 0.f);
+                        yv[r] = (live && m < M) ? ogc_ld4(yb + (size_t)m * hw + pos) : make_float4(0.f, 0.f, 0.f, 0.f);
                     }
                 }
                 v4f acc[4];
@@ -577,6 +678,7 @@
                             o.z = fmaf(al, g.z, fmaf(c2, y.z, c3)); o.w = fmaf(al, g.w, fmaf(c2, y.w, c3));
                             if constexpr (FIRST > 0) {
                                 float mine = 0.f;
+                                if constexpr (LIST) o.w *= wl;
 #pragma unroll
                                 for (int c = 0; c < FIRST; ++c) {
                                     float d = fmaf(o.w, x0v[c].w, fmaf(o.z, x0v[c].z, fmaf(o.y, x0v[c].y, o.x * x0v[c].x)));
@@ -588,7 +690,7 @@
                                 }
                                 if (j < first.c0) atomicAdd(&s_dw[m * FC_MAX_C0 + j], mine);
                             } else {
-                                ogc_st4(outb + (size_t)m * hw + p0 + 4 * j, o);
+                                if (mine_ok) ogc_st4(outb + (size_t)m * hw + pos, o);
                             }
                         }
                     }
@@ -611,10 +713,22 @@
 namespace {
 int nsample_shift(int nsample) { return nsample == 16 ? 4 : nsample == 32 ? 5 : nsample == 64 ? 6 : -1; }
 
+int live_check(const char *name, const int *live, const int *n_live, int live_cap, int hw, int nsample, LiveIn &ls) {
+    OGC_REQUIRE(live && n_live, "%s: null live-step list", name);
+    if (nsample != 32 && nsample != 64) {
+        ogc_set_error("%s: the list form needs nsample 32 or 64 (nsample=%d)", name, nsample);
+        return OGC_ERR_UNSUPPORTED;
+    }
+    OGC_REQUIRE(hw >= 16 && hw % nsample == 0 && (hw >> 4) <= LIVE_MASK && live_cap >= (hw >> 4),
+                "%s: the live-step list holds %d entries per sample, hw=%d needs room for %d", name, live_cap, hw, hw >> 4);
+    ls.steps = live; ls.n = n_live; ls.cap = live_cap;
+    return OGC_OK;
+}
+
 template <typename AT>
 int wgrad_moments_impl(const char *name, int b, int cin, int cout, int hw, int relu, const AT *y_prev, const float *pa,
                        const float *pb, const AT *grad_y, const float *coef2, const float *inj, int s_shift,
-                       float *moments, ogc_stream_t stream) {
+                       float *moments, ogc_stream_t stream, LiveIn ls = LiveIn()) {
     OGC_REQUIRE(b >= 0 && cin >= 1 && cout >= 1 && hw >= 1, "%s: bad shape", name);
     OGC_REQUIRE(y_prev && pa && pb && grad_y && moments, "%s: null pointer", name);
     if ((hw & (sizeof(AT) == 2 ? 31 : 15)) != 0 || (((uintptr_t)y_prev | (uintptr_t)grad_y) & 15) != 0) {
@@ -633,7 +747,7 @@
         ogc_set_error("%s: memset failed", name);
         return OGC_ERR_LAUNCH;
     }
-#define OGC_ML(A, C) moments_launch<A, C, AT>(b, cin, cout, hw, relu, y_prev, grad_y, pa, pb, coef2, inj, s_shift, moments, s)
+#define OGC_ML(A, C) moments_launch<A, C, AT>(b, cin, cout, hw, relu, y_prev, grad_y, pa, pb, coef2, inj, s_shift, moments, s, FirstIn(), ls)
     if (cout <= 16 && cin <= 16) OGC_ML(1, 1);
     else if (cout <= 32 && cin <= 16) OGC_ML(2, 1);
     else if (cout <= 32 && cin <= 32) OGC_ML(2, 2);
@@ -664,14 +778,14 @@
 template <typename AT>
 int wgrad_moments_pooled_impl(const char *name, int b, int cin, int cout, int hw, int relu, int nsample, const AT *y_prev,
                               const float *pa, const float *pb, const AT *y, const float *coef2, const float *inj,
-                              float *moments, ogc_stream_t stream) {
+                              float *moments, ogc_stream_t stream, LiveIn ls = LiveIn()) {
     const int sh = nsample_shift(nsample);
     if (sh < 0 || hw % nsample != 0 || (((uintptr_t)coef2 | (uintptr_t)inj) & 7) != 0) {
         ogc_set_error("%s: nsample=%d must be 16, 32 or 64 and divide hw=%d", name, nsample, hw);
         return OGC_ERR_UNSUPPORTED;
     }
     OGC_REQUIRE(b == 0 || (coef2 && inj), "%s: null pointer", name);
-    return wgrad_moments_impl<AT>(name, b, cin, cout, hw, relu, y_prev, pa, pb, y, coef2, inj, sh, moments, stream);
+    return wgrad_moments_impl<AT>(name, b, cin, cout, hw, relu, y_prev, pa, pb, y, coef2, inj, sh, moments, stream, ls);
 }
 }
 
@@ -680,6 +794,17 @@
                                                 const float *inj, float *moments, ogc_stream_t stream) {
     return wgrad_moments_pooled_impl<float>("ogc_conv1x1_wgrad_moments_pooled", b, cin, cout, hw, relu, nsample, y_prev, pa, pb, y,
                                             coef2, inj, moments, stream);
+}
+
+extern "C" int ogc_conv1x1_wgrad_moments_pooled_live(int b, int cin, int cout, int hw, int relu, int nsample, const float *y_prev,
+                                                     const float *pa, const float *pb, const float *y, const float *coef2,
+                                                     const float *inj, const int *live, const int *n_live, int live_cap,
+                                                     float *moments, ogc_stream_t stream) {
+    const char *name = "ogc_conv1x1_wgrad_moments_pooled_live";
+    LiveIn ls;
+    const int rc = live_check(name, live, n_live, live_cap, hw, nsample, ls);
+    if (rc != OGC_OK) return rc;
+    return wgrad_moments_pooled_impl<float>(name, b, cin, cout, hw, relu, nsample, y_prev, pa, pb, y, coef2, inj, moments, stream, ls);
 }
 
 extern "C" int ogc_conv1x1_wgrad_moments_pooled_h(int b, int cin, int cout, int hw, int relu, int nsample,
@@ -713,7 +838,7 @@
 template <typename AT>
 int dgrad_adjoint_impl(const char *name, int b, int cin, int cout, int hw, int relu, const float *w, const AT *grad_y,
                        const AT *y_prev, const float *pa, const float *pb, const float *coef, const float *coef2,
-                       const float *inj, int s_shift, AT *grad_prev, ogc_stream_t stream) {
+                       const float *inj, int s_shift, AT *grad_prev, ogc_stream_t stream, LiveIn ls = LiveIn()) {
     OGC_REQUIRE(b >= 0 && cin >= 1 && cout >= 1 && hw >= 1, "%s: bad shape", name);
     OGC_REQUIRE(w && grad_y && y_prev && pa && pb && coef && grad_prev, "%s: null pointer", name);
     if ((hw & 63) != 0 || cout > 160 || (((uintptr_t)grad_y | (uintptr_t)y_prev | (uintptr_t)grad_prev) & ogc_act_mask<AT>()) != 0) {
@@ -725,7 +850,7 @@
     if (b == 0) return OGC_OK;
     const int M = cin, K = cout, Kq = (K + 3) / 4;
     const size_t lds = ((size_t)64 * ogc_a_ld(Kq) + 64 * 5) * sizeof(float) +
-                       (inj ? (size_t)WG_WAVES * K * (64 >> s_shift) * sizeof(float4) : 0);
+                       (inj ? (size_t)WG_WAVES * K * (ls.steps ? 4 : 64 >> s_shift) * sizeof(float4) : 0);
     if (sizeof(AT) == 2 && !ogc_g_matmul_bf16) {
         ogc_set_error("%s: 16-bit activations need ogc_set_matmul_precision(1)", name);
         return OGC_ERR_UNSUPPORTED;
@@ -746,6 +871,13 @@
     const float2 *c2 = reinterpret_cast<const float2 *>(coef2), *ij = reinterpret_cast<const float2 *>(inj);
 #define OGC_DGA(KQV)                                                                                                        \
     do {                                                                                                                    \
+        if constexpr (sizeof(AT) == 4) {                                                                                    \
+            if (inj && ls.steps) {                 \
+                hipLaunchKernelGGL((dgrad_adjoint_kernel<KQV, true, AT, false, 0, true>), grid, dim3(WG_WAVES * OGC_WAVE), lds, s, M, K, \
+                                   hw, relu, w, grad_y, y_prev, pa, pb, coef, c2, ij, s_shift, grad_prev, FirstIn(), ls);  \
+                break;                                                                                                      \
+            }                                                                                                               \
+        }                                                                                                                   \
         if (inj)                                                                                                            \
             hipLaunchKernelGGL((dgrad_adjoint_kernel<KQV, true, AT, sizeof(AT) == 2>), grid, dim3(WG_WAVES * OGC_WAVE), lds, s, M, K, hw, relu, w,  \
                                grad_y, y_prev, pa, pb, coef, c2, ij, s_shift, grad_prev);                                  \
@@ -782,14 +914,14 @@
 template <typename AT>
 int dgrad_adjoint_pooled_impl(const char *name, int b, int cin, int cout, int hw, int relu, int nsample, const float *w,
                               const AT *y, const float *coef2, const float *inj, const AT *y_prev, const float *pa,
-                              const float *pb, const float *coef, AT *grad_prev, ogc_stream_t stream) {
+                              const float *pb, const float *coef, AT *grad_prev, ogc_stream_t stream, LiveIn ls = LiveIn()) {
     const int sh = nsample_shift(nsample);
     if (sh < 0 || hw % nsample != 0 || (((uintptr_t)coef2 | (uintptr_t)inj) & 7) != 0) {
         ogc_set_error("%s: nsample=%d must be 16, 32 or 64 and divide hw=%d", name, nsample, hw);
         return OGC_ERR_UNSUPPORTED;
     }
     OGC_REQUIRE(b == 0 || (coef2 && inj), "%s: null pointer", name);
-    return dgrad_adjoint_impl<AT>(name, b, cin, cout, hw, relu, w, y, y_prev, pa, pb, coef, coef2, inj, sh, grad_prev, stream);
+    return dgrad_adjoint_impl<AT>(name, b, cin, cout, hw, relu, w, y, y_prev, pa, pb, coef, coef2, inj, sh, grad_prev, stream, ls);
 }
 }
 
@@ -801,6 +933,18 @@
                                             y_prev, pa, pb, coef, grad_prev, stream);
 }
 
+extern "C" int ogc_conv1x1_dgrad_adjoint_pooled_live(int b, int cin, int cout, int hw, int relu, int nsample, const float *w,
+                                                     const float *y, const float *coef2, const float *inj, const float *y_prev,
+                                                     const float *pa, const float *pb, const float *coef, const int *live,
+                                                     const int *n_live, int live_cap, float *grad_prev, ogc_stream_t stream) {
+    const char *name = "ogc_conv1x1_dgrad_adjoint_pooled_live";
+    LiveIn ls;
+    const int rc = live_check(name, live, n_live, live_cap, hw, nsample, ls);
+    if (rc != OGC_OK) return rc;
+    return dgrad_adjoint_pooled_impl<float>(name, b, cin, cout, hw, relu, nsample, w, y, coef2, inj, y_prev, pa, pb, coef, grad_prev,
+                                            stream, ls);
+}
+
 extern "C" int ogc_conv1x1_dgrad_adjoint_pooled_h(int b, int cin, int cout, int hw, int relu, int nsample, const float *w,
                                                   const ogc_bf16_t *y, const float *coef2, const float *inj,
                                                   const ogc_bf16_t *y_prev, const float *pa, const float *pb, const float *coef,
@@ -809,10 +953,10 @@
                                                inj, y_prev, pa, pb, coef, grad_prev, stream);
 }
 
-extern "C" int ogc_conv1x1_wgrad_moments_first(int b, int cin, int cout, int hw, int relu, int c0, const float *x0, const float *w1,
-                                               const float *pa, const float *pb, const float *grad_y, float *moments,
-                                               ogc_stream_t stream) {
-    const char *name = "ogc_conv1x1_wgrad_moments_first";
+namespace {
+int wgrad_moments_first_impl(const char *name, int b, int cin, int cout, int hw, int relu, int c0, const float *x0, const float *w1,
+                             const float *pa, const float *pb, const float *grad_y, float *moments, ogc_stream_t stream,
+                             LiveIn ls = LiveIn()) {
     const int rc = ogc_first_check(name, b, cin, c0, hw, x0, w1);
     if (rc != OGC_OK) return rc;
     OGC_REQUIRE(cout >= 1 && pa && pb && grad_y && moments, "%s: bad shape or null pointer", name);
@@ -832,9 +976,9 @@
     const int cp = ogc_first_cp(c0);
 #define OGC_MLF(A, C)                                                                                                                    \
     do {                                                                                                                                 \
-        if (cp == 3) moments_launch<A, C, float, 3>(b, cin, cout, hw, relu, nullptr, grad_y, pa, pb, nullptr, nullptr, 0, moments, s, first); \
-        else if (cp == 6) moments_launch<A, C, float, 6>(b, cin, cout, hw, relu, nullptr, grad_y, pa, pb, nullptr, nullptr, 0, moments, s, first); \
-        else moments_launch<A, C, float, 8>(b, cin, cout, hw, relu, nullptr, grad_y, pa, pb, nullptr, nullptr, 0, moments, s, first); \
+        if (cp == 3) moments_launch<A, C, float, 3>(b, cin, cout, hw, relu, nullptr, grad_y, pa, pb, nullptr, nullptr, 0, moments, s, first, ls); \
+        else if (cp == 6) moments_launch<A, C, float, 6>(b, cin, cout, hw, relu, nullptr, grad_y, pa, pb, nullptr, nullptr, 0, moments, s, first, ls); \
+        else moments_launch<A, C, float, 8>(b, cin, cout, hw, relu, nullptr, grad_y, pa, pb, nullptr, nullptr, 0, moments, s, first, ls); \
     } while (0)
     if (cout <= 16 && cin <= 16) OGC_MLF(1, 1);
     else if (cout <= 32 && cin <= 16) OGC_MLF(2, 1);
@@ -846,10 +990,9 @@
     return OGC_OK;
 }
 
-extern "C" int ogc_conv1x1_dgrad_adjoint_first(int b, int cin, int cout, int hw, int relu, int c0, const float *w,
-                                               const float *grad_y, const float *x0, const float *w1, const float *pa,
-                                               const float *pb, const float *coef, float *grad_w1, ogc_stream_t stream) {
-    const char *name = "ogc_conv1x1_dgrad_adjoint_first";
+int dgrad_adjoint_first_impl(const char *name, int b, int cin, int cout, int hw, int relu, int c0, const float *w,
+                             const float *grad_y, const float *x0, const float *w1, const float *pa, const float *pb,
+                             const float *coef, float *grad_w1, ogc_stream_t stream, LiveIn ls = LiveIn()) {
     const int rc = ogc_first_check(name, b, cin, c0, hw, x0, w1);
     if (rc != OGC_OK) return rc;
     OGC_REQUIRE(cout >= 1 && w && grad_y && pa && pb && coef && grad_w1, "%s: bad shape or null pointer", name);
@@ -876,9 +1019,16 @@
     dim3 grid(ogc_divup(tiles, first.run), b);
     const int cp = ogc_first_cp(c0);
 #define OGC_DGAF(KQV, CPV)                                                                                                  \
-    hipLaunchKernelGGL((dgrad_adjoint_kernel<KQV, false, float, false, CPV>), grid, dim3(WG_WAVES * OGC_WAVE), lds, s, M, K, hw, \
-                       relu, w, grad_y, (const float *)nullptr, pa, pb, coef, (const float2 *)nullptr, (const float2 *)nullptr, 0, \
-                       (float *)nullptr, first)
+    do {                                                                                                                    \
+        if (ls.steps)                                                                                                       \
+            hipLaunchKernelGGL((dgrad_adjoint_kernel<KQV, false, float, false, CPV, true>), grid, dim3(WG_WAVES * OGC_WAVE), lds, s, M, \
+                               K, hw, relu, w, grad_y, (const float *)nullptr, pa, pb, coef, (const float2 *)nullptr,       \
+                               (const float2 *)nullptr, 0, (float *)nullptr, first, ls);                                    \
+        else                                                                                                                \
+            hipLaunchKernelGGL((dgrad_adjoint_kernel<KQV, false, float, false, CPV>), grid, dim3(WG_WAVES * OGC_WAVE), lds, s, M, K, \
+                               hw, relu, w, grad_y, (const float *)nullptr, pa, pb, coef, (const float2 *)nullptr,          \
+                               (const float2 *)nullptr, 0, (float *)nullptr, first, ls);                                    \
+    } while (0)
     if (Kq <= 8) {
         if (cp == 3) OGC_DGAF(8, 3); else if (cp == 6) OGC_DGAF(8, 6); else OGC_DGAF(8, 8);
     } else {
@@ -888,3 +1038,57 @@
     OGC_CHECK_LAUNCH(name);
     return OGC_OK;
 }
+}
+
+extern "C" int ogc_conv1x1_wgrad_moments_first(int b, int cin, int cout, int hw, int relu, int c0, const float *x0, const float *w1,
+                                               const float *pa, const float *pb, const float *grad_y, float *moments,
+                                               ogc_stream_t stream) {
+    return wgrad_moments_first_impl("ogc_conv1x1_wgrad_moments_first", b, cin, cout, hw, relu, c0, x0, w1, pa, pb, grad_y, moments,
+                                    stream);
+}
+
+extern "C" int ogc_conv1x1_dgrad_adjoint_first(int b, int cin, int cout, int hw, int relu, int c0, const float *w,
+                                               const float *grad_y, const float *x0, const float *w1, const float *pa,
+                                               const float *pb, const float *coef, float *grad_w1, ogc_stream_t stream) {
+    return dgrad_adjoint_first_impl("ogc_conv1x1_dgrad_adjoint_first", b, cin, cout, hw, relu, c0, w, grad_y, x0, w1, pa, pb, coef,
+                                    grad_w1, stream);
+}
+
+extern "C" int ogc_conv1x1_wgrad_moments_first_live(int b, int cin, int cout, int hw, int relu, int c0, int nsample, const float *x0,
+                                                    const float *w1, const float *pa, const float *pb, const float *grad_y,
+                                                    const int *live, const int *n_live, int live_cap, float *moments,
+                                                    ogc_stream_t stream) {
+    const char *name = "ogc_conv1x1_wgrad_moments_first_live";
+    LiveIn ls;
+    const int rc = live_check(name, live, n_live, live_cap, hw, nsample, ls);
+    if (rc != OGC_OK) return rc;
+    return wgrad_moments_first_impl(name, b, cin, cout, hw, relu, c0, x0, w1, pa, pb, grad_y, moments, stream, ls);
+}
+
+extern "C" int ogc_conv1x1_dgrad_adjoint_first_live(int b, int cin, int cout, int hw, int relu, int c0, int nsample, const float *w,
+                                                    const float *grad_y, const float *x0, const float *w1, const float *pa,
+                                                    const float *pb, const float *coef, const int *live, const int *n_live,
+                                                    int live_cap, float *grad_w1, ogc_stream_t stream) {
+    const char *name = "ogc_conv1x1_dgrad_adjoint_first_live";
+    LiveIn ls;
+    const int rc = live_check(name, live, n_live, live_cap, hw, nsample, ls);
+    if (rc != OGC_OK) return rc;
+    return dgrad_adjoint_first_impl(name, b, cin, cout, hw, relu, c0, w, grad_y, x0, w1, pa, pb, coef, grad_w1, stream, ls);
+}
+
+extern "C" int ogc_live_steps(int b, int p, int s, const int *idx, int *live, int *n_live, ogc_stream_t stream) {
+    OGC_REQUIRE(b >= 0 && p >= 1, "ogc_live_steps: bad shape");
+    if (s != 16 && s != 32 && s != 64) {
+        ogc_set_error("ogc_live_steps: nsample=%d must be 16, 32 or 64", s);
+        return OGC_ERR_UNSUPPORTED;
+    }
+    OGC_REQUIRE(idx && live && n_live, "ogc_live_steps: null pointer");
+    if (p > LIVE_MAX_P) {
+        ogc_set_error("ogc_live_steps: p=%d centres per sample, at most %d", p, LIVE_MAX_P);
+        return OGC_ERR_UNSUPPORTED;
+    }
+    if (b == 0) return OGC_OK;
+    hipLaunchKernelGGL(live_steps_kernel, dim3(b), dim3(1024), 0, (hipStream_t)stream, p, s, idx, live, n_live);
+    OGC_CHECK_LAUNCH("ogc_live_steps");
+    return OGC_OK;
+}
diff --git a/ogc_amd/fused.py b/ogc_amd/fused.py
--- a/ogc_amd/fused.py
+++ b/ogc_amd/fused.py
@@ -802,12 +802,39 @@
 FIRST_PAIR_FUSED = True
 FIRST_PAIR_MAX_C0 = 8
 
+SKIP_REPEAT_STEPS = True
+
+
+def live_steps(idx):
+    nat = _api._native
+    if not (SKIP_REPEAT_STEPS and torch.is_grad_enabled() and idx is not None and idx.is_cuda and idx.dim() == 3
+            and idx.shape[2] in (32, 64) and idx.shape[1] <= 32768 and not deterministic() and getattr(nat, "live_steps_wrapper", None) is not None
+            and nat.get_matmul_precision() == "fp32"):
+        return None
+    return nat.live_steps_wrapper((idx if idx.dtype is torch.int32 else idx.int()).contiguous())
+
+
+class LiveLink:
+    __slots__ = ("live", "n_live", "pair", "tail")
+
+    def __init__(self, live):
+        self.live, self.n_live = live
+        self.pair = self.tail = False
+
+    def fits(self, B, P, S):
+        return (SKIP_REPEAT_STEPS and S in (32, 64) and tuple(self.live.shape) == (B, P * S // 16)
+                and tuple(self.n_live.shape) == (B,) and not deterministic()
+                and getattr(_api._native, "conv1x1_dgrad_adjoint_first_live_wrapper", None) is not None)
+
 
 class _FirstPairConv(Function):
 
     @staticmethod
-    def forward(ctx, x0, w1, gn_weight, gn_bias, w2, gn_groups, eps, relu, next_groups):
+    def forward(ctx, x0, w1, gn_weight, gn_bias, w2, gn_groups, eps, relu, next_groups, link=None):
         ctx.set_materialize_grads(False)
+        ctx.link = None
+        if link is not None and x0.dim() == 4 and link.fits(x0.shape[0], x0.shape[2], x0.shape[3]):
+            ctx.link, link.pair = link, True
         nat = _api._native
         B, c0 = x0.shape[0], x0.shape[1]
         c1, c2 = w1.shape[0], w2.shape[0]
@@ -834,8 +861,9 @@
     @staticmethod
     def backward(ctx, grad_y, _grad_stats=None):
         if grad_y is None:
-            return (None,) * 9
-        nat = _api._native
+            return (None,) * 10
+        nat = _api._native
+        link = ctx.link if (ctx.link is not None and ctx.link.tail) else None
         x0, w1, gn_weight, w2, mean, rstd, a, bb = ctx.saved_tensors
         gn_groups, relu, hw = ctx.cfg
         B, c0 = x0.shape[0], x0.shape[1]
@@ -844,15 +872,23 @@
         grad_y = grad_y.contiguous()
         w1c, w2c = w1.contiguous().view(c1, c0), w2.contiguous().view(c2, c1)
         moments = zeroed_empty((B, 2, c2, c1), torch.float32, dev)
-        nat.conv1x1_wgrad_moments_first_wrapper(B, c1, c2, hw, relu, c0, x0, w1c, a, bb, grad_y, moments)
+        if link is not None:
+            nat.conv1x1_wgrad_moments_first_live_wrapper(B, c1, c2, hw, relu, c0, x0.shape[3], x0, w1c, a, bb, grad_y, link.live,
+                                                         link.n_live, moments)
+        else:
+            nat.conv1x1_wgrad_moments_first_wrapper(B, c1, c2, hw, relu, c0, x0, w1c, a, bb, grad_y, moments)
         grad_w2 = zeroed_empty((c2, c1), torch.float32, dev)
         coef = torch.empty(B, c1, 3, dtype=torch.float32, device=dev)
         ggb = zeroed_empty((2, c1), torch.float32, dev)
         nat.gn_moments_combine_wrapper(B, c1, c2, hw, gn_groups, moments, w2c, a, bb, mean, rstd, gn_weight.contiguous(),
                                        grad_w2, coef, ggb[0], ggb[1])
         grad_w1 = zeroed_empty((c1, c0), torch.float32, dev)
-        nat.conv1x1_dgrad_adjoint_first_wrapper(B, c1, c2, hw, relu, c0, w2c, grad_y, x0, w1c, a, bb, coef, grad_w1)
-        return None, grad_w1.view_as(w1), ggb[0], ggb[1], grad_w2.view_as(w2), None, None, None, None
+        if link is not None:
+            nat.conv1x1_dgrad_adjoint_first_live_wrapper(B, c1, c2, hw, relu, c0, x0.shape[3], w2c, grad_y, x0, w1c, a, bb, coef,
+                                                         link.live, link.n_live, grad_w1)
+        else:
+            nat.conv1x1_dgrad_adjoint_first_wrapper(B, c1, c2, hw, relu, c0, w2c, grad_y, x0, w1c, a, bb, coef, grad_w1)
+        return None, grad_w1.view_as(w1), ggb[0], ggb[1], grad_w2.view_as(w2), None, None, None, None, None
 
 
 def _plain_conv(conv):
@@ -881,9 +917,9 @@
             and max(c1, c2) * hw < 2 ** 31 and x.shape[0] <= 32768)
 
 
-def first_pair_conv(x, conv, gn, relu, conv2, gn2):
+def first_pair_conv(x, conv, gn, relu, conv2, gn2, link=None):
     return _FirstPairConv.apply(x, conv.weight, gn.weight, gn.bias, conv2.weight, gn.num_groups, gn.eps, bool(relu),
-                                gn2.num_groups)
+                                gn2.num_groups, link)
 
 
 SPARSE_POOL_BACKWARD = True
@@ -894,11 +930,15 @@
 
     @staticmethod
     def forward(ctx, y_prev, stats_prev, gn_weight, gn_bias, conv_weight, gn_groups, eps, relu, gn2_weight, gn2_bias,
-                groups2, eps2, relu2):
+                groups2, eps2, relu2, link=None):
         nat = _api._native
         y_prev = y_prev.contiguous()
         B, cin, P, S = y_prev.shape
         cout = conv_weight.shape[0]
+        ctx.link = None
+        if (link is not None and link.pair and y_prev.dtype is torch.float32 and link.fits(B, P, S)
+                and cin <= _moment_width(y_prev) and cout <= _pool_moment_cout(y_prev)):
+            ctx.link, link.tail = link, True
         y, stats, extremes, mean, rstd, a, bb = _norm_act_conv_forward(y_prev, stats_prev, gn_weight, gn_bias, conv_weight,
                                                                        gn_groups, eps, relu, groups2, S, gn2_weight)
         dev = y_prev.device
@@ -940,9 +980,14 @@
             ws = nat.group_norm_ws(B, cin, gn_groups, True, dev)
             nat.group_norm_bwd_wrapper(B, cin, hw, gn_groups, relu, y_prev, gn_weight.contiguous(), gn_bias.contiguous(), mean,
                                        rstd, grad_z, grad_prev, gw, gb, ws)
-            return (grad_prev, None, gw, gb, grad_w.view_as(conv_weight), None, None, None, gw2, gb2, None, None, None)
+            return (grad_prev, None, gw, gb, grad_w.view_as(conv_weight), None, None, None, gw2, gb2, None, None, None, None)
+        link = ctx.link
         moments = zeroed_empty((B, 2, cout, cin), torch.float32, dev)
-        nat.conv1x1_wgrad_moments_pooled_wrapper(B, cin, cout, hw, relu, S, y_prev, a, bb, y, coef2, inj, moments)
+        if link is not None:
+            nat.conv1x1_wgrad_moments_pooled_live_wrapper(B, cin, cout, hw, relu, S, y_prev, a, bb, y, coef2, inj, link.live,
+                                                          link.n_live, moments)
+        else:
+            nat.conv1x1_wgrad_moments_pooled_wrapper(B, cin, cout, hw, relu, S, y_prev, a, bb, y, coef2, inj, moments)
         coef = torch.empty(B, cin, 3, dtype=torch.float32, device=dev)
         ggb = zeroed_empty((2, cin), torch.float32, dev)
         gw, gb = ggb[0], ggb[1]
@@ -950,8 +995,12 @@
         nat.gn_moments_combine_wrapper(B, cin, cout, hw, gn_groups, moments, w, a, bb, mean, rstd,
                                        gn_weight.contiguous(), grad_w, coef, gw, gb)
         grad_prev = torch.empty_like(y_prev)
-        nat.conv1x1_dgrad_adjoint_pooled_wrapper(B, cin, cout, hw, relu, S, w, y, coef2, inj, y_prev, a, bb, coef, grad_prev)
-        return (grad_prev, None, gw, gb, grad_w.view_as(conv_weight), None, None, None, gw2, gb2, None, None, None)
+        if link is not None:
+            nat.conv1x1_dgrad_adjoint_pooled_live_wrapper(B, cin, cout, hw, relu, S, w, y, coef2, inj, y_prev, a, bb, coef,
+                                                          link.live, link.n_live, grad_prev)
+        else:
+            nat.conv1x1_dgrad_adjoint_pooled_wrapper(B, cin, cout, hw, relu, S, w, y, coef2, inj, y_prev, a, bb, coef, grad_prev)
+        return (grad_prev, None, gw, gb, grad_w.view_as(conv_weight), None, None, None, gw2, gb2, None, None, None, None)
 
 
 @_gate
@@ -976,9 +1025,9 @@
             and g2 <= 32 and cout % g2 == 0 and (cout // g2) % 4 == 0)
 
 
-def norm_act_conv_pool(y_prev, stats_prev, gn, relu, conv, next_gn, next_relu):
+def norm_act_conv_pool(y_prev, stats_prev, gn, relu, conv, next_gn, next_relu, link=None):
     return _NormActConvPool.apply(y_prev, stats_prev, gn.weight, gn.bias, conv.weight, gn.num_groups, gn.eps, bool(relu),
-                                  next_gn.weight, next_gn.bias, next_gn.num_groups, next_gn.eps, bool(next_relu))
+                                  next_gn.weight, next_gn.bias, next_gn.num_groups, next_gn.eps, bool(next_relu), link)
 
 
 class _SelfAttentionCore(Function):
diff --git a/ogc_amd/pointnet2_cuda.py b/ogc_amd/pointnet2_cuda.py
--- a/ogc_amd/pointnet2_cuda.py
+++ b/ogc_amd/pointnet2_cuda.py
@@ -700,6 +700,45 @@
          _f(coef2, "coef2"), _f(inj, "inj"), ypp, _f(pa, "pa"), _f(pb, "pb"), _f(coef, "coef"), op)
 
 
+def live_steps_wrapper(idx):
+    B, P, S = idx.shape
+    live = torch.empty(B, P * max(S // 16, 1), dtype=torch.int32, device=idx.device)
+    n_live = torch.empty(B, dtype=torch.int32, device=idx.device)
+    _run("ogc_live_steps", idx, B, P, S, _i(idx, "idx"), _i(live, "live"), _i(n_live, "n_live"))
+    return live, n_live
+
+
+def _live_args(live, n_live):
+    return (_opt(live, torch.int32, "live"), _opt(n_live, torch.int32, "n_live"),
+            0 if live is None else live.numel() // max(live.shape[0], 1))
+
+
+def conv1x1_wgrad_moments_pooled_live_wrapper(b, cin, cout, hw, relu, nsample, y_prev, pa, pb, y, coef2, inj, live, n_live,
+                                              moments):
+    _run("ogc_conv1x1_wgrad_moments_pooled_live", y_prev, b, cin, cout, hw, int(relu), nsample, _f(y_prev, "y_prev"),
+         _f(pa, "pa"), _f(pb, "pb"), _f(y, "y"), _f(coef2, "coef2"), _f(inj, "inj"), *_live_args(live, n_live),
+         _f(moments, "moments"))
+
+
+def conv1x1_dgrad_adjoint_pooled_live_wrapper(b, cin, cout, hw, relu, nsample, w, y, coef2, inj, y_prev, pa, pb, coef, live,
+                                              n_live, grad_prev):
+    _run("ogc_conv1x1_dgrad_adjoint_pooled_live", y, b, cin, cout, hw, int(relu), nsample, _f(w, "w"), _f(y, "y"),
+         _f(coef2, "coef2"), _f(inj, "inj"), _f(y_prev, "y_prev"), _f(pa, "pa"), _f(pb, "pb"), _f(coef, "coef"),
+         *_live_args(live, n_live), _f(grad_prev, "grad_prev"))
+
+
+def conv1x1_wgrad_moments_first_live_wrapper(b, cin, cout, hw, relu, c0, nsample, x0, w1, pa, pb, grad_y, live, n_live, moments):
+    _run("ogc_conv1x1_wgrad_moments_first_live", x0, b, cin, cout, hw, int(relu), c0, nsample, _f(x0, "x0"), _f(w1, "w1"),
+         _f(pa, "pa"), _f(pb, "pb"), _f(grad_y, "grad_y"), *_live_args(live, n_live), _f(moments, "moments"))
+
+
+def conv1x1_dgrad_adjoint_first_live_wrapper(b, cin, cout, hw, relu, c0, nsample, w, grad_y, x0, w1, pa, pb, coef, live, n_live,
+                                             grad_w1):
+    _run("ogc_conv1x1_dgrad_adjoint_first_live", x0, b, cin, cout, hw, int(relu), c0, nsample, _f(w, "w"), _f(grad_y, "grad_y"),
+         _f(x0, "x0"), _f(w1, "w1"), _f(pa, "pa"), _f(pb, "pb"), _f(coef, "coef"), *_live_args(live, n_live),
+         _f(grad_w1, "grad_w1"))
+
+
 def mlp_chain_pool_supported(c0, c1, c2, c3, nsample):
     return bool(_lib.load().ogc_mlp_chain_pool_supported(c0, c1, c2, c3, nsample))
 
diff --git a/ogc_amd/utils/nn_util.py b/ogc_amd/utils/nn_util.py
--- a/ogc_amd/utils/nn_util.py
+++ b/ogc_amd/utils/nn_util.py
@@ -147,10 +147,11 @@
                                    preact=preact))
 
 
-def _shared_mlp_run(self, x, pool, first=None):
+def _shared_mlp_run(self, x, pool, first=None, live=None):
     from ..fused import (act16_middle_ok, group_norm_act, group_norm_act_maxpool, norm_act_conv, norm_act_conv_available,
                          norm_act_conv_pool, norm_act_conv_pool_available, pointwise_conv)
     layers = list(self.children())
+    link = None
     pending = None
 
     def flush(p, last):
@@ -177,7 +178,10 @@
             from ..fused import first_pair_available, first_pair_conv
             (conv, gn, relu), (conv2, gn2, relu2) = block(layer), block(layers[1])
             if first_pair_available(x, conv, gn, conv2, gn2):
-                y, stats = first_pair_conv(x, conv, gn, relu, conv2, gn2)
+                if live is not None and pool and len(layers) == 3:
+                    from ..fused import LiveLink
+                    link = LiveLink(live)
+                y, stats = first_pair_conv(x, conv, gn, relu, conv2, gn2, link)
                 pending, skip = (y, stats, gn2, relu2, None), True
                 continue
         if not fusable:
@@ -198,7 +202,8 @@
         if pending is not None and norm_act_conv_available(pending[0], pending[2], conv):
             if pool and li == len(layers) - 1 and pending[0].dim() == 4 and pending[0].shape[-1] in (16, 32, 64):
                 if norm_act_conv_pool_available(pending[0], pending[2], conv, gn):
-                    return norm_act_conv_pool(pending[0], pending[1], pending[2], pending[3], conv, gn, relu)
+                    return norm_act_conv_pool(pending[0], pending[1], pending[2], pending[3], conv, gn, relu,
+                                              link if li == 2 else None)
                 y, stats, extremes = norm_act_conv(pending[0], pending[1], pending[2], pending[3], conv, gn,
                                                    pool=pending[0].shape[-1])
             else:
@@ -217,8 +222,8 @@
     return _shared_mlp_run(self, x, False)
 
 
-def _shared_mlp_forward_maxpool(self, x, first=None):
-    return _shared_mlp_run(self, x, True, first)
+def _shared_mlp_forward_maxpool(self, x, first=None, live=None):
+    return _shared_mlp_run(self, x, True, first, live)
 
 
 def _shared_mlp_first_layer(self):
diff --git a/ogc_amd/utils/pointnet2_util.py b/ogc_amd/utils/pointnet2_util.py
--- a/ogc_amd/utils/pointnet2_util.py
+++ b/ogc_amd/utils/pointnet2_util.py
@@ -24,7 +24,16 @@
         plan = self.plan_sampling(xyz, parent_ties)
         plan["idx"] = self.plan_neighbours(xyz, plan["new_xyz"])
         plan["rev"] = self.plan_reverse(plan["idx"], xyz.shape[1])
+        plan["live"] = self.plan_live(plan["idx"])
         return plan
+
+    def plan_live(self, idx):
+        from .. import fused as _fused
+
+        def chain(mlp):
+            head = mlp.first_layer() if len(mlp) == 3 else None
+            return head is not None and head[0].weight.shape[1] <= _fused.FIRST_PAIR_MAX_C0
+        return [_fused.live_steps(j) if (j is not None and chain(mlp)) else None for j, mlp in zip(idx, self.mlps)]
 
     def plan_reverse(self, idx, n):
         from .. import fused as _fused
@@ -68,6 +77,8 @@
             geometry = dict(geometry, idx=self.plan_neighbours(xyz, geometry["new_xyz"]))
         if geometry is not None and "rev" not in geometry:
             geometry = dict(geometry, rev=self.plan_reverse(geometry["idx"], xyz.shape[1]))
+        if geometry is not None and "live" not in geometry:
+            geometry = dict(geometry, live=self.plan_live(geometry["idx"]))
         new_xyz = geometry["new_xyz"] if geometry is not None else None
         new_inds = geometry["new_inds"] if geometry is not None else None
 
@@ -83,8 +94,9 @@
                                                                           act16=len(mlp) >= 2)))
                     continue
                 grouped = grouper(xyz, new_xyz, features, idx=nn_idx)[0]
-            else:
-                grouped = grouper(xyz, new_xyz, features)[0]
+                pooled.append(mlp.forward_maxpool(grouped, live=geometry["live"][i]))
+                continue
+            grouped = grouper(xyz, new_xyz, features)[0]
             pooled.append(mlp.forward_maxpool(grouped))
         new_features = torch.cat(pooled, dim=1) if len(pooled) != 1 else pooled[0]
         if return_inds:
```

Result: faster. 1776 point-clouds/s (median of 6 runs) (+7.4%).
